# jacobwilliams/lbfgsb

Hardware: NVIDIA B200
Metric: lbfgsb_iterations_per_s (higher is better)
Workload: dtype f64

## Files before the change

### include/lbfgsb_b200.h

```cpp
#ifndef LBFGSB_B200_H
#define LBFGSB_B200_H

#include <stdint.h>

#ifdef __cplusplus
extern "C" {
#endif

#define LBFGSB_B200_MMAX 20

typedef struct lbfgsb_dev lbfgsb_dev_t;

int lbfgsb_b200_version(void);
const char* lbfgsb_b200_last_error(void);

void lbfgsb_setulb_f64(const int32_t* n, const int32_t* m, double* x, const double* l, const double* u,
                       const int32_t* nbd, double* f, double* g, const double* factr, const double* pgtol,
                       double* wa, int32_t* iwa, char* task, const int32_t* iprint, char* csave,
                       int32_t* lsave, int32_t* isave, double* dsave, const char* itfile, int32_t itfile_len);
void lbfgsb_setulb_f32(const int32_t* n, const int32_t* m, float* x, const float* l, const float* u,
                       const int32_t* nbd, float* f, float* g, const float* factr, const float* pgtol,
                       float* wa, int32_t* iwa, char* task, const int32_t* iprint, char* csave,
                       int32_t* lsave, int32_t* isave, float* dsave, const char* itfile, int32_t itfile_len);
void lbfgsb_host_release(int32_t* isave);
// ... 5 lines not shown
lbfgsb_dev_t* lbfgsb_dev_create_sharded(int64_t n_local, int64_t offset, int64_t n_global, int32_t m,
                                        int32_t real_kind, void* cuda_stream, void* nccl_comm,
                                        int32_t rank, int32_t world);
void lbfgsb_dev_destroy(lbfgsb_dev_t* h);
void lbfgsb_dev_set_iteration_file(lbfgsb_dev_t* h, const char* name);
void lbfgsb_setulb_dev_f64(lbfgsb_dev_t* h, double* x_dev, const double* l_dev, const double* u_dev,
                           const int32_t* nbd_dev, double* f, double* g_dev, const double* factr,
                           const double* pgtol, char* task, const int32_t* iprint, char* csave,
                           int32_t* lsave, int32_t* isave, double* dsave);
void lbfgsb_setulb_dev_f32(lbfgsb_dev_t* h, float* x_dev, const float* l_dev, const float* u_dev,
                           const int32_t* nbd_dev, float* f, float* g_dev, const float* factr,
                           const float* pgtol, char* task, const int32_t* iprint, char* csave,
                           int32_t* lsave, int32_t* isave, float* dsave);

typedef int (*lbfgsb_fg_dev_f64)(void* user, int64_t n, const double* x_dev, double* g_dev, double* f_out, void* cuda_stream);
typedef int (*lbfgsb_fg_dev_f32)(void* user, int64_t n, const float* x_dev, float* g_dev, float* f_out, void* cuda_stream);
int lbfgsb_minimize_dev_f64(lbfgsb_dev_t* h, double* x_dev, const double* l_dev, const double* u_dev, const int32_t* nbd_dev,
                            lbfgsb_fg_dev_f64 fg, void* user, double factr, double pgtol, int32_t max_iter, int32_t max_fg,
                            int32_t iprint, double* f, double* g_dev, char* task, char* csave, int32_t* lsave, int32_t* isave,
                            double* dsave);
int lbfgsb_minimize_dev_f32(lbfgsb_dev_t* h, float* x_dev, const float* l_dev, const float* u_dev, const int32_t* nbd_dev,
                            lbfgsb_fg_dev_f32 fg, void* user, float factr, float pgtol, int32_t max_iter, int32_t max_fg,
                            int32_t iprint, float* f, float* g_dev, char* task, char* csave, int32_t* lsave, int32_t* isave,
                            float* dsave);

typedef int (*lbfgsb_fg_enqueue_f64)(void* user, int64_t n, const double* x_dev, double* g_dev, double* f_dev, void* cuda_stream);
typedef int (*lbfgsb_fg_enqueue_f32)(void* user, int64_t n, const float* x_dev, float* g_dev, float* f_dev, void* cuda_stream);
int lbfgsb_minimize_graph_dev_f64(lbfgsb_dev_t* h, double* x_dev, const double* l_dev, const double* u_dev, const int32_t* nbd_dev,
                                  lbfgsb_fg_enqueue_f64 fg, void* user, double factr, double pgtol, int32_t max_iter, int32_t max_fg,
                                  double* f, double* g_dev, char* task, char* csave, int32_t* lsave, int32_t* isave, double* dsave);
int lbfgsb_minimize_graph_dev_f32(lbfgsb_dev_t* h, float* x_dev, const float* l_dev, const float* u_dev, const int32_t* nbd_dev,
                                  lbfgsb_fg_enqueue_f32 fg, void* user, float factr, float pgtol, int32_t max_iter, int32_t max_fg,
                                  float* f, float* g_dev, char* task, char* csave, int32_t* lsave, int32_t* isave, float* dsave);
int lbfgsb_dev_graph_stats(lbfgsb_dev_t* h, int64_t* graph_steps, int64_t* launches_per_step);

int lbfgsb_dev_checkpoint_write(lbfgsb_dev_t* h, const char* path);
int lbfgsb_dev_checkpoint_read(lbfgsb_dev_t* h, const char* path);

int lbfgsb_dev_nccl_unique_id(void* id128);
void* lbfgsb_dev_nccl_init(const void* id128, int32_t rank, int32_t world);
void lbfgsb_dev_nccl_destroy(void* comm);

int lbfgsb_dev_active_set_hash(lbfgsb_dev_t* h, uint64_t* hash, int64_t* count);
void* lbfgsb_dev_vector(lbfgsb_dev_t* h, int32_t which);
int lbfgsb_dev_vector_copy(lbfgsb_dev_t* h, int32_t which, void* dst_dev, int64_t bytes);
int lbfgsb_dev_exchange_mode(lbfgsb_dev_t* h);
int lbfgsb_dev_counters(lbfgsb_dev_t* h, int64_t* launches, int64_t* syncs);
void lbfgsb_dev_profile(lbfgsb_dev_t* h, int32_t enable);
int lbfgsb_dev_profile_read(lbfgsb_dev_t* h, int32_t cap, char* names , double* ms, double* bytes,
                            int64_t* calls);
void lbfgsb_dev_profile_reset(lbfgsb_dev_t* h);
void lbfgsb_dev_set_tie_limit(lbfgsb_dev_t* h, int64_t max_breakpoints);
int lbfgsb_dev_tie_stats(lbfgsb_dev_t* h, int64_t* replays, int64_t* not_replayed);

int lbfgsb_problem_rosenbrock_f64(int64_t n, const double* x_dev, double* g_dev, double* f_out, void* cuda_stream,
                                  int32_t first, int32_t last, double xl, double xr, void* scratch_dev);
int lbfgsb_problem_rosenbrock_f32(int64_t n, const float* x_dev, float* g_dev, float* f_out, void* cuda_stream,
                                  int32_t first, int32_t last, float xl, float xr, void* scratch_dev);
int64_t lbfgsb_problem_scratch_bytes(void);
int lbfgsb_problem_rosenbrock_halo_f64(int64_t n, const double* x_dev, double* g_dev, double* f_part_dev, void* cuda_stream,
                                       int32_t first, int32_t last, const double* halo_dev, void* scratch_dev);
typedef struct {
    const void* d_dev;
    void* gd_part_dev;
    void* pg_part_dev;
    int64_t n;
    int32_t grid, block, unroll, real_kind;
    int32_t vec, reserved;
} lbfgsb_trial_sums_t;
int lbfgsb_dev_trial_sums(lbfgsb_dev_t* h, lbfgsb_trial_sums_t* out);
void lbfgsb_dev_trial_sums_commit(lbfgsb_dev_t* h);
int lbfgsb_problem_fused_f64(lbfgsb_dev_t* h, int32_t kind, const double* x_dev, double* g_dev, const double* l_dev,
                             const double* u_dev, const int32_t* nbd_dev, double* f_out, uint64_t seed);
int lbfgsb_problem_sharded_f64(lbfgsb_dev_t* h, int32_t kind, const double* x_dev, double* g_dev, const double* l_dev,
                               const double* u_dev, const int32_t* nbd_dev, double* f_out, uint64_t seed);
int lbfgsb_problem_quadratic_halo_f64(int64_t n, const double* x_dev, double* g_dev, double* f_part_dev, void* cuda_stream,
                                      int64_t index_offset, uint64_t seed, const double* halo_dev, void* scratch_dev);

int lbfgsb_problem_quadratic_f64(int64_t n, const double* x_dev, double* g_dev, double* f_out, void* cuda_stream,
                                 int64_t index_offset, uint64_t seed, double xl, double xr, void* scratch_dev);
int lbfgsb_problem_quadratic_f32(int64_t n, const float* x_dev, float* g_dev, float* f_out, void* cuda_stream,
                                 int64_t index_offset, uint64_t seed, float xl, float xr, void* scratch_dev);

typedef struct lbfgsb_batch lbfgsb_batch_t;
lbfgsb_batch_t* lbfgsb_batch_create(int32_t nprob, int64_t n, int32_t m, int32_t real_kind, void* cuda_stream);
void lbfgsb_batch_destroy(lbfgsb_batch_t* h);
void lbfgsb_batch_setulb_dev_f64(lbfgsb_batch_t* h, double* x_dev, const double* l_dev, const double* u_dev, const int32_t* nbd_dev,
                                 double* f_dev, double* g_dev, const double* factr, const double* pgtol, char* task, char* csave,
                                 int32_t* lsave, int32_t* isave, double* dsave);
void lbfgsb_batch_setulb_dev_f32(lbfgsb_batch_t* h, float* x_dev, const float* l_dev, const float* u_dev, const int32_t* nbd_dev,
                                 float* f_dev, float* g_dev, const float* factr, const float* pgtol, char* task, char* csave,
                                 int32_t* lsave, int32_t* isave, float* dsave);
int lbfgsb_batch_counts(lbfgsb_batch_t* h, int32_t* n_fg, int32_t* n_newx, int32_t* n_done);
void* lbfgsb_batch_stream(lbfgsb_batch_t* h);
void* lbfgsb_batch_fg_mask(lbfgsb_batch_t* h);
int lbfgsb_batch_get_iwhere(lbfgsb_batch_t* h, int32_t* iwhere_host);
int lbfgsb_problem_rosenbrock_batch_f64(int32_t nprob, int64_t n, const double* x_dev, double* g_dev, double* f_dev,
                                        const int32_t* mask_dev, void* cuda_stream);
int lbfgsb_problem_rosenbrock_batch_f32(int32_t nprob, int64_t n, const float* x_dev, float* g_dev, float* f_dev,
                                        const int32_t* mask_dev, void* cuda_stream);

int lbfgsb_test_projgr_f64(int64_t n, const double* l, const double* u, const int32_t* nbd, const double* x,
                           const double* g, double* sbgnrm_out);
int lbfgsb_test_sum_f64(int64_t n, const double* a, const double* b, double* out);
int lbfgsb_test_sum_f32(int64_t n, const float* a, const float* b, float* out);
int lbfgsb_test_sort_f64(int64_t n, const double* t_dev, int32_t* order_out_dev, double* sorted_out_dev);
// ... 16 lines not shown
```

### lbfgsb_b200/__init__.py

```python
import ctypes as C
import os
import subprocess

import numpy as np

_HERE = os.path.dirname(os.path.abspath(__file__))
_ROOT = os.path.dirname(_HERE)
SO_PATH = os.path.join(_HERE, "liblbfgsb_b200.so")
_SOURCES = ["engine.cu", "common.cuh", "kernels_stream.cuh", "kernels_dense.cuh", "cauchy_walk.cuh", "kernels_tma.cuh",
            "tma_pipe.cuh", "cauchy_walk_dist.cuh", "batch.cuh", "host_print.h"]
NVCC_FLAGS = ["-gencode", "arch=compute_100a,code=sm_100a", "-lineinfo", "-O3", "-std=c++17",
              "-fmad=false", "-Xcompiler", "-fPIC", "-shared"]

_LIB = None


class LbfgsbB200Error(RuntimeError):
    pass


def _stale():
    if not os.path.exists(SO_PATH):
        return True
    t = os.path.getmtime(SO_PATH)
    deps = [os.path.join(_HERE, "csrc", s) for s in _SOURCES]
    deps += [os.path.join(_ROOT, "include", h) for h in ("lbfgsb_b200.h", "lbfgsb_b200_shape.h")]
    return any(os.path.exists(p) and os.path.getmtime(p) > t for p in deps)


def build(force=False, verbose=False):
    if not (force or _stale()):
        return SO_PATH
    nvcc = os.environ.get("NVCC", "/usr/local/cuda/bin/nvcc")
    cmd = [nvcc] + NVCC_FLAGS + (["-Xptxas", "-v"] if verbose else []) + \
          ["-o", SO_PATH, os.path.join(_HERE, "csrc", "engine.cu"), "-ldl"]
    subprocess.check_call(cmd)
    return SO_PATH


_REAL = {np.dtype(np.float64): ("f64", C.c_double), np.dtype(np.float32): ("f32", C.c_float)}


def lib():
    global _LIB
    if _LIB is None:
        if not os.path.exists(SO_PATH):
            raise LbfgsbB200Error(
                "lbfgsb_b200: %s is missing -- run `python -c 'import __graft_entry__ as g; g.build()'` "
                "(there is no CPU path)" % SO_PATH)
        L = C.CDLL(SO_PATH)
        L.lbfgsb_b200_last_error.restype = C.c_char_p
        L.lbfgsb_dev_create.restype = C.c_void_p
        L.lbfgsb_dev_create.argtypes = [C.c_int64, C.c_int32, C.c_int32, C.c_void_p]
        L.lbfgsb_dev_create_sharded.restype = C.c_void_p
        L.lbfgsb_dev_create_sharded.argtypes = [C.c_int64, C.c_int64, C.c_int64, C.c_int32, C.c_int32,
                                                C.c_void_p, C.c_void_p, C.c_int32, C.c_int32]
        L.lbfgsb_dev_destroy.argtypes = [C.c_void_p]
        L.lbfgsb_dev_set_iteration_file.argtypes = [C.c_void_p, C.c_char_p]
        L.lbfgsb_dev_checkpoint_write.argtypes = [C.c_void_p, C.c_char_p]
        L.lbfgsb_dev_checkpoint_read.argtypes = [C.c_void_p, C.c_char_p]
        L.lbfgsb_host_engine.restype = C.c_void_p
        L.lbfgsb_host_engine.argtypes = [C.c_void_p]
        L.lbfgsb_dev_vector.restype = C.c_void_p
        L.lbfgsb_dev_vector.argtypes = [C.c_void_p, C.c_int32]
        L.lbfgsb_dev_vector_copy.argtypes = [C.c_void_p, C.c_int32, C.c_void_p, C.c_int64]
        L.lbfgsb_dev_active_set_hash.argtypes = [C.c_void_p, C.c_void_p, C.c_void_p]
        L.lbfgsb_dev_counters.argtypes = [C.c_void_p, C.c_void_p, C.c_void_p]
        L.lbfgsb_dev_graph_stats.argtypes = [C.c_void_p, C.c_void_p, C.c_void_p]
        L.lbfgsb_problem_rosenbrock_halo_f64.argtypes = [C.c_int64, C.c_void_p, C.c_void_p, C.c_void_p, C.c_void_p, C.c_int32, C.c_int32,
                                                         C.c_void_p, C.c_void_p]
        L.lbfgsb_problem_quadratic_halo_f64.argtypes = [C.c_int64, C.c_void_p, C.c_void_p, C.c_void_p, C.c_void_p, C.c_int64, C.c_uint64,
                                                        C.c_void_p, C.c_void_p]
        L.lbfgsb_dev_profile.argtypes = [C.c_void_p, C.c_int32]
        L.lbfgsb_dev_profile_reset.argtypes = [C.c_void_p]
        L.lbfgsb_dev_set_tie_limit.argtypes = [C.c_void_p, C.c_int64]
        L.lbfgsb_dev_set_tie_limit.restype = None
        L.lbfgsb_dev_tie_stats.argtypes = [C.c_void_p, C.c_void_p, C.c_void_p]
        L.lbfgsb_dev_profile_read.argtypes = [C.c_void_p, C.c_int32, C.c_void_p, C.c_void_p, C.c_void_p, C.c_void_p]
        L.lbfgsb_dev_nccl_init.restype = C.c_void_p
        L.lbfgsb_dev_nccl_init.argtypes = [C.c_void_p, C.c_int32, C.c_int32]
        L.lbfgsb_dev_nccl_destroy.argtypes = [C.c_void_p]
        L.lbfgsb_problem_scratch_bytes.restype = C.c_int64
        for sfx, cr in (("f64", C.c_double), ("f32", C.c_float)):
            getattr(L, "lbfgsb_setulb_" + sfx).restype = None
            getattr(L, "lbfgsb_setulb_dev_" + sfx).restype = None
            getattr(L, "lbfgsb_problem_rosenbrock_" + sfx).argtypes = [
                C.c_int64, C.c_void_p, C.c_void_p, C.c_void_p, C.c_void_p, C.c_int32, C.c_int32, cr, cr, C.c_void_p]
            getattr(L, "lbfgsb_problem_quadratic_" + sfx).argtypes = [
                C.c_int64, C.c_void_p, C.c_void_p, C.c_void_p, C.c_void_p, C.c_int64, C.c_uint64, cr, cr, C.c_void_p]
        L.lbfgsb_problem_rosenbrock_halo_f64.argtypes = [C.c_int64, C.c_void_p, C.c_void_p, C.c_void_p, C.c_void_p, C.c_int32,
                                                         C.c_int32, C.c_void_p, C.c_void_p]
        L.lbfgsb_problem_quadratic_halo_f64.argtypes = [C.c_int64, C.c_void_p, C.c_void_p, C.c_void_p, C.c_void_p, C.c_int64,
                                                        C.c_uint64, C.c_void_p, C.c_void_p]
        for nm in ("lbfgsb_problem_fused_f64", "lbfgsb_problem_sharded_f64"):
            getattr(L, nm).argtypes = [C.c_void_p, C.c_int32, C.c_void_p, C.c_void_p, C.c_void_p, C.c_void_p, C.c_void_p,
                                       C.c_void_p, C.c_uint64]
        L.lbfgsb_dev_exchange_mode.argtypes = [C.c_void_p]
        L.lbfgsb_batch_create.restype = C.c_void_p
        L.lbfgsb_batch_create.argtypes = [C.c_int32, C.c_int64, C.c_int32, C.c_int32, C.c_void_p]
        L.lbfgsb_batch_destroy.argtypes = [C.c_void_p]
        L.lbfgsb_batch_counts.argtypes = [C.c_void_p, C.c_void_p, C.c_void_p, C.c_void_p]
        L.lbfgsb_batch_stream.restype = C.c_void_p
        L.lbfgsb_batch_stream.argtypes = [C.c_void_p]
        L.lbfgsb_batch_get_iwhere.restype = C.c_int
        L.lbfgsb_batch_get_iwhere.argtypes = [C.c_void_p, C.c_void_p]
        L.lbfgsb_batch_fg_mask.restype = C.c_void_p
        L.lbfgsb_batch_fg_mask.argtypes = [C.c_void_p]
        for sfx in ("f64", "f32"):
            getattr(L, "lbfgsb_batch_setulb_dev_" + sfx).restype = None
            getattr(L, "lbfgsb_batch_setulb_dev_" + sfx).argtypes = [C.c_void_p] * 14
            getattr(L, "lbfgsb_problem_rosenbrock_batch_" + sfx).argtypes = [C.c_int32, C.c_int64, C.c_void_p, C.c_void_p, C.c_void_p,
                                                                             C.c_void_p, C.c_void_p]
        _LIB = L
    return _LIB


def last_error():
    return lib().lbfgsb_b200_last_error().decode()


def _p(a):
    return a.ctypes.data_as(C.c_void_p)


def _check_task(task):
    s = bytes(task[:60]).decode(errors="replace")
    if s.startswith(("ERROR: CUDA", "ERROR: NO CUDA", "ERROR: INVALID LBFGSB", "ERROR: DEVICE POINTERS", "ERROR: SETULB CALLED")):
        raise LbfgsbB200Error(s.rstrip() + " -- " + last_error())


# ... 150 lines not shown
        if lib().lbfgsb_dev_checkpoint_write(C.c_void_p(self.h), path.encode()) != 0:
            raise LbfgsbB200Error("checkpoint write failed: " + last_error())

    def checkpoint_read(self, path):
        if lib().lbfgsb_dev_checkpoint_read(C.c_void_p(self.h), path.encode()) != 0:
            raise LbfgsbB200Error("checkpoint read failed: " + last_error())

    def active_set_hash(self):
        h, c = C.c_uint64(0), C.c_int64(0)
        if lib().lbfgsb_dev_active_set_hash(C.c_void_p(self.h), C.byref(h), C.byref(c)) != 0:
            raise LbfgsbB200Error(last_error())
        return h.value, c.value

    @staticmethod
    def _opt(t):
        return C.c_void_p(t.data_ptr()) if t is not None else C.c_void_p(0)

    def fused_fg(self, kind, x, g, l=None, u=None, nbd=None, seed=0):
        out = C.c_double(0.0)
        rc = lib().lbfgsb_problem_fused_f64(C.c_void_p(self.h), C.c_int32(kind), C.c_void_p(x.data_ptr()),
                                            C.c_void_p(g.data_ptr()), self._opt(l), self._opt(u), self._opt(nbd),
                                            C.byref(out), C.c_uint64(int(seed)))
        if rc != 0:
            raise LbfgsbB200Error("objective kernel failed (rc %d): %s" % (rc, last_error()))
        return out.value

    def sharded_fg(self, kind, x, g, l=None, u=None, nbd=None, seed=0):
        out = C.c_double(0.0)
        rc = lib().lbfgsb_problem_sharded_f64(C.c_void_p(self.h), C.c_int32(kind), C.c_void_p(x.data_ptr()),
                                              C.c_void_p(g.data_ptr()), self._opt(l), self._opt(u), self._opt(nbd),
                                              C.byref(out), C.c_uint64(int(seed)))
        if rc == 2:
            return None
        if rc != 0:
            raise LbfgsbB200Error("sharded objective failed: " + last_error())
        return out.value

    def exchange_mode(self):
        return int(lib().lbfgsb_dev_exchange_mode(C.c_void_p(self.h)))

    def counters(self):
        a, b = C.c_int64(0), C.c_int64(0)
        lib().lbfgsb_dev_counters(C.c_void_p(self.h), C.byref(a), C.byref(b))
        return a.value, b.value

    def set_tie_limit(self, max_breakpoints):
        lib().lbfgsb_dev_set_tie_limit(C.c_void_p(self.h), C.c_int64(int(max_breakpoints)))

    def tie_stats(self):
        a, b = C.c_int64(0), C.c_int64(0)
        lib().lbfgsb_dev_tie_stats(C.c_void_p(self.h), C.byref(a), C.byref(b))
        return a.value, b.value

    def profile(self, on=True):
        lib().lbfgsb_dev_profile(C.c_void_p(self.h), 1 if on else 0)

    def profile_reset(self):
        lib().lbfgsb_dev_profile_reset(C.c_void_p(self.h))

    def profile_read(self):
        cap = 64
        names = C.create_string_buffer(32 * cap)
        ms = (C.c_double * cap)()
        by = (C.c_double * cap)()
        calls = (C.c_int64 * cap)()
        k = lib().lbfgsb_dev_profile_read(C.c_void_p(self.h), cap, names, ms, by, calls)
        out = {}
        for i in range(k):
            nm = names.raw[32 * i:32 * (i + 1)].split(b"\0")[0].decode()
            out[nm] = {"ms": ms[i], "bytes": by[i], "calls": calls[i]}
        return out

    def vector(self, which, count=None, dtype=None):
        torch = self.torch
        n = self.n if count is None else count
        tdt = {np.dtype(np.float64): torch.float64, np.dtype(np.float32): torch.float32}[self.dtype]
        if which == 7:
            tdt = torch.int32
        out = torch.empty(n, dtype=tdt, device="cuda")
        if lib().lbfgsb_dev_vector_copy(C.c_void_p(self.h), which, C.c_void_p(out.data_ptr()),
                                        C.c_int64(out.numel() * out.element_size())) != 0:
            raise LbfgsbB200Error("lbfgsb_dev_vector_copy failed")
        return out

    def close(self):
        if self.h:
            lib().lbfgsb_dev_destroy(C.c_void_p(self.h))
            self.h = None

    def __del__(self):
        try:
            self.close()
        except Exception:
            pass


class RosenbrockDevice:

    def __init__(self, dtype, stream=None):
        import torch
        self.dtype = np.dtype(dtype)
        self.scratch = torch.empty(int(lib().lbfgsb_problem_scratch_bytes()), dtype=torch.uint8, device="cuda")
        sfx, self._cr = _REAL[self.dtype]
        self._fn = getattr(lib(), "lbfgsb_problem_rosenbrock_" + sfx)
        self._f = np.zeros(1, dtype=self.dtype)
        self.stream = stream
# ... 140 lines not shown
```

### lbfgsb_b200/csrc/common.cuh

```cuda
#pragma once
#include <cuda_runtime.h>
#include <stdint.h>
#include <float.h>
#include <math.h>

#include "../../include/lbfgsb_b200_shape.h"

typedef long long i64;

#define LB_MMAX 20
#define LB_KMAX (6 * LB_MMAX + 8)
#define LB_IMAX 8

enum {
    TK_START = 0, TK_FG_START = 1, TK_FG_LNSRCH = 2, TK_NEW_X = 3, TK_CONV_PG = 4, TK_CONV_F = 5,
    TK_ABNORMAL = 6, TK_RESTART = 7, TK_STOP = 8,
    TK_ERR_N = 10, TK_ERR_M = 11, TK_ERR_FACTR = 12, TK_ERR_NBD = 13, TK_ERR_INFEAS = 14
};
enum { PAUSE_NONE = 0, PAUSE_CLASSIFY = 1, PAUSE_WALK = 2, PAUSE_GCP_FREEV = 3, PAUSE_DELTA = 4, PAUSE_BACKTRACK = 5, PAUSE_LSINIT = 6 };
enum {
    CS_START = 0, CS_FG = 1, CS_CONV = 2, CS_WARN_ROUND = 3, CS_WARN_XTOL = 4, CS_WARN_STPMAX = 5,
    CS_WARN_STPMIN = 6, CS_ERR_STP_LT_MIN = 10, CS_ERR_STP_GT_MAX = 11, CS_ERR_G_GE_0 = 12,
    CS_ERR_FTOL = 13, CS_ERR_GTOL = 14, CS_ERR_XTOL = 15, CS_ERR_STPMIN = 16, CS_ERR_STPMAX = 17,
    CS_BLANK = 99
};
__host__ __device__ inline bool cs_is_warn(int c) { return c >= CS_WARN_ROUND && c <= CS_WARN_STPMIN; }
__host__ __device__ inline bool cs_is_err(int c) { return c >= CS_ERR_STP_LT_MIN && c <= CS_ERR_STPMAX; }

enum {
    EV_ITER_BEGIN = 1,
    EV_SUBGNORM0 = 2,
    EV_CAUCHY_SINGULAR = 3,
    EV_FORMK_FAIL = 4,
    EV_SUBSM_SINGULAR = 5,
    EV_BACKTRACK = 6,
    EV_ASCENT = 7,
    EV_LNSRCH_RESTART = 8,
    EV_SKIP = 9,
    EV_FORMT_FAIL = 10
};
#define LB_EVMAX 24

template <typename T> struct Real;
template <> struct Real<double> {
    static constexpr int VEC = LBFGSB_VEC_F64;
    static constexpr int UNROLL = LBFGSB_UNROLL_F64;
    typedef double2 vec_t;
    typedef int2 ivec_t;
    typedef unsigned long long key_t;
    __host__ __device__ static double eps() { return DBL_EPSILON; }
};
template <> struct Real<float> {
    static constexpr int VEC = LBFGSB_VEC_F32;
    static constexpr int UNROLL = LBFGSB_UNROLL_F32;
    typedef float2 vec_t;
    typedef int2 ivec_t;
    typedef unsigned int key_t;
    __host__ __device__ static float eps() { return FLT_EPSILON; }
};

template <typename T>
struct DevState {
    int go;
    int pause;
    int in_body;
    int restart;
    int need_walk;
    int cauchy_mode;
    int do_subspace, do_formk, do_delta, do_backtrack, do_update, do_step, do_restore;
    int fuse_uc;
    int classify_done;
    int lsinit_done;
    int spec_step;
    int step_done;
    int do_unstep;
    int lazy_gcp;
    int fuse_gf;
    int lazy_z;
    int p2p_timeout;
    int z_in_x;
    int save_z;
    int task, csave, info;
    int col, head, itail, iupdat, iter, nfgv, nskip, ifun, iback, iword;
    int updatd, prjctd, cnstnd, boxed, wrk, bnded;
    int brackt, stage;
    int m;
    int gstage;
    i64 n, nintol, nseg, nfree, nact, nenter, nleave, nbreak, nfreec, nbdd, errk;
    i64 ibkmin;
    i64 ibd;
    i64 walk_J;
    i64 walk_done;
    i64 walk_base;
    i64 walk_rcount;
    i64 walk_lcount;
    i64 walk_rem;
    i64 walk_cstart;
    i64 walk_fixn;
    int walk_closed, pad1;
    int tie_redo;
    int tie_round;
    i64 tie_limit;
    i64 tie_events;
    unsigned long long tie_key;
    i64 snap_base;
    int ev_n, ev_code[LB_EVMAX];
    T ev_a[LB_EVMAX], ev_b[LB_EVMAX];
    i64 n_el;
    T theta, fold, tol, dnorm, epsmch, gd, gdold, stp, stpmx, sbgnrm, dtd, xstep, f, rr, dr, ddum;
    T pgtol, factr, sbg_spec;
    T ls[13];
    T f1, f2, f2_org, dtm, tsum, bkmin;
    T dd_p, alpha;
    T walk_f1, walk_f2, walk_tlast, walk_tprev2;
    T sy[LB_MMAX * LB_MMAX], ss[LB_MMAX * LB_MMAX], wt[LB_MMAX * LB_MMAX];
    T wn[4 * LB_MMAX * LB_MMAX], wn1[4 * LB_MMAX * LB_MMAX];
    T p[2 * LB_MMAX], c[2 * LB_MMAX], v[2 * LB_MMAX], wv[2 * LB_MMAX], a[2 * LB_MMAX];
    T p0[2 * LB_MMAX];
    T walkA[2 * LB_MMAX], walkB[2 * LB_MMAX];
    T snapA[2 * LB_MMAX], snapB[2 * LB_MMAX];
    T snap_f1, snap_f2, snap_tlast, snap_tprev2;
};

template <typename T> __device__ inline void ev_push(DevState<T>* s, int code, T a = (T)0, T b = (T)0) {
    const int k = s->ev_n;
    if (k < LB_EVMAX) { s->ev_code[k] = code; s->ev_a[k] = a; s->ev_b[k] = b; s->ev_n = k + 1; }
}

template <typename T> __device__ __forceinline__ T shfl_xor_t(T v, int off);
template <> __device__ __forceinline__ double shfl_xor_t<double>(double v, int off) {
    return __shfl_xor_sync(0xffffffffu, v, off);
}
template <> __device__ __forceinline__ float shfl_xor_t<float>(float v, int off) {
    return __shfl_xor_sync(0xffffffffu, v, off);
}
template <> __device__ __forceinline__ i64 shfl_xor_t<i64>(i64 v, int off) {
    return __shfl_xor_sync(0xffffffffu, v, off);
}
template <> __device__ __forceinline__ int shfl_xor_t<int>(int v, int off) {
    return __shfl_xor_sync(0xffffffffu, v, off);
}

template <typename T> __device__ __forceinline__ T warp_sum(T v) {
#pragma unroll
    for (int off = 16; off >= 1; off >>= 1) v = v + shfl_xor_t<T>(v, off);
    return v;
}
template <typename T> __device__ __forceinline__ T warp_max(T v) {
#pragma unroll
    for (int off = 16; off >= 1; off >>= 1) { T o = shfl_xor_t<T>(v, off); v = o > v ? o : v; }
    return v;
}
template <typename T> __device__ __forceinline__ T warp_min(T v) {
#pragma unroll
    for (int off = 16; off >= 1; off >>= 1) { T o = shfl_xor_t<T>(v, off); v = o < v ? o : v; }
    return v;
}

template <typename T, int K>
__device__ __forceinline__ void block_sum_store(const T (&acc)[K], int kcount, T* smem, T* part) {
    const int lane = threadIdx.x & 31, w = threadIdx.x >> 5;
    constexpr int NW = LBFGSB_BLOCK / 32;
#pragma unroll
    for (int k = 0; k < K; ++k) {
        if (k < kcount) {
            T v = warp_sum<T>(acc[k]);
            if (lane == 0 && w < NW) smem[k * NW + w] = v;
        }
    }
    __syncthreads();
    for (int k = threadIdx.x; k < kcount; k += LBFGSB_BLOCK) {
        T s = smem[k * NW];
#pragma unroll
        for (int q = 1; q < NW; ++q) s = s + smem[k * NW + q];
// ... 186 lines not shown
            unsigned int q = *reinterpret_cast<const unsigned int*>(p + base);
#pragma unroll
            for (int v = 0; v < VEC; ++v) out[v] = (q >> (8 * v)) & 0xff;
        }
    } else {
#pragma unroll
        for (int v = 0; v < VEC; ++v) out[v] = (base + v < n) ? p[base + v] : 0;
    }
}
template <typename T>
__device__ __forceinline__ void stv(T* __restrict__ p, i64 base, i64 n, const T (&in)[Real<T>::VEC]) {
    constexpr int VEC = Real<T>::VEC;
    if (base + VEC <= n) {
        typename Real<T>::vec_t q;
        T* e = reinterpret_cast<T*>(&q);
#pragma unroll
        for (int v = 0; v < VEC; ++v) e[v] = in[v];
        *reinterpret_cast<typename Real<T>::vec_t*>(p + base) = q;
    } else {
#pragma unroll
        for (int v = 0; v < VEC; ++v) if (base + v < n) p[base + v] = in[v];
    }
}
template <typename T>
__device__ __forceinline__ void stvi(int* __restrict__ p, i64 base, i64 n, const int (&in)[Real<T>::VEC]) {
    constexpr int VEC = Real<T>::VEC;
    if (base + VEC <= n) {
        typename Real<T>::ivec_t q;
        int* e = reinterpret_cast<int*>(&q);
#pragma unroll
        for (int v = 0; v < VEC; ++v) e[v] = in[v];
        *reinterpret_cast<typename Real<T>::ivec_t*>(p + base) = q;
    } else {
#pragma unroll
        for (int v = 0; v < VEC; ++v) if (base + v < n) p[base + v] = in[v];
    }
}
template <typename T>
__device__ __forceinline__ void stvb(unsigned char* __restrict__ p, i64 base, i64 n,
                                     const int (&in)[Real<T>::VEC]) {
    constexpr int VEC = Real<T>::VEC;
    if (base + VEC <= n) {
        if (VEC == 2) {
            *reinterpret_cast<unsigned short*>(p + base) = (unsigned short)((in[0] & 0xff) | ((in[1] & 0xff) << 8));
        } else {
            unsigned int q = 0;
#pragma unroll
            for (int v = 0; v < VEC; ++v) q |= (unsigned int)(in[v] & 0xff) << (8 * v);
            *reinterpret_cast<unsigned int*>(p + base) = q;
        }
    } else {
#pragma unroll
        for (int v = 0; v < VEC; ++v) if (base + v < n) p[base + v] = (unsigned char)in[v];
    }
}

#define LB_FOR_TILES(T, n, base)                                                               \
    for (i64 _tl = blockIdx.x, _nt = ((n) + (i64)LBFGSB_BLOCK * Real<T>::VEC * Real<T>::UNROLL - 1) / \
                                     ((i64)LBFGSB_BLOCK * Real<T>::VEC * Real<T>::UNROLL);       \
         _tl < _nt; _tl += LBFGSB_GRID)                                                        \
        _Pragma("unroll") for (int _k = 0; _k < Real<T>::UNROLL; ++_k)                           \
            for (i64 base = _tl * ((i64)LBFGSB_BLOCK * Real<T>::VEC * Real<T>::UNROLL) +         \
                            (i64)_k * (LBFGSB_BLOCK * Real<T>::VEC) + (i64)threadIdx.x * Real<T>::VEC, \
                     _once = 1;                                                                \
                 _once && base < (n); _once = 0)

#define LB_FOR_TILES_NU(T, n, base)                                                            \
    for (i64 _tl = blockIdx.x, _nt = ((n) + (i64)LBFGSB_BLOCK * Real<T>::VEC * Real<T>::UNROLL - 1) / \
                                     ((i64)LBFGSB_BLOCK * Real<T>::VEC * Real<T>::UNROLL);       \
         _tl < _nt; _tl += LBFGSB_GRID)                                                        \
        _Pragma("unroll 1") for (int _k = 0; _k < Real<T>::UNROLL; ++_k)                         \
            for (i64 base = _tl * ((i64)LBFGSB_BLOCK * Real<T>::VEC * Real<T>::UNROLL) +         \
                            (i64)_k * (LBFGSB_BLOCK * Real<T>::VEC) + (i64)threadIdx.x * Real<T>::VEC, \
                     _once = 1;                                                                \
                 _once && base < (n); _once = 0)

namespace dense {

template <typename T> __device__ inline T ddot(int n, const T* dx, const T* dy) {
    T s = (T)0;
    for (int i = 0; i < n; ++i) s = s + dx[i] * dy[i];
    return s;
}
template <typename T> __device__ inline void daxpy(int n, T da, const T* dx, T* dy) {
    if (n <= 0 || da == (T)0) return;
    for (int i = 0; i < n; ++i) dy[i] = dy[i] + da * dx[i];
}

template <typename T> __device__ inline int dpofa(T* a, int lda, int n) {
    for (int j = 0; j < n; ++j) {
        T s = (T)0;
        for (int k = 0; k < j; ++k) {
            T t = a[k + j * lda] - ddot<T>(k, a + k * lda, a + j * lda);
            t = t / a[k + k * lda];
            a[k + j * lda] = t;
            s = s + t * t;
        }
        s = a[j + j * lda] - s;
        if (s <= (T)0) return j + 1;
        a[j + j * lda] = sqrt(s);
    }
    return 0;
}

template <typename T> __device__ inline int dtrsl(const T* t, int ldt, int n, T* b, int job) {
    for (int k = 0; k < n; ++k)
// ... 322 lines not shown
```

### lbfgsb_b200/csrc/engine.cu

```cuda
#include <cuda_runtime.h>
#include <dlfcn.h>
#include <stdarg.h>
#include <stdio.h>
#include <stdlib.h>
#include <string.h>

#include <mutex>
#include <string>
#include <unordered_set>
#include <vector>

#include "../../include/lbfgsb_b200.h"
#include "cauchy_walk.cuh"
#include "kernels_tma.cuh"
#include "cauchy_walk_dist.cuh"
#include "batch.cuh"
#include "host_print.h"
#include <algorithm>

static thread_local std::string g_last_error;
static void set_error(const char* fmt, ...) {
    char buf[512];
    va_list ap;
    va_start(ap, fmt);
// ... 4 lines not shown
#define CK(call)                                                                             \
    do {                                                                                     \
        cudaError_t _e = (call);                                                             \
        if (_e != cudaSuccess) {                                                             \
            set_error("CUDA error %s at %s:%d (%s)", cudaGetErrorString(_e), __FILE__, __LINE__, #call); \
            return false;                                                                    \
        }                                                                                    \
    } while (0)

typedef struct ncclComm* ncclComm_t;
typedef struct { char internal[128]; } ncclUniqueId;
struct NcclApi {
    int (*GetUniqueId)(ncclUniqueId*);
    int (*CommInitRank)(ncclComm_t*, int, ncclUniqueId, int);
    int (*CommDestroy)(ncclComm_t);
    int (*AllGather)(const void*, void*, size_t, int, ncclComm_t, cudaStream_t);
    int (*Send)(const void*, size_t, int, int, ncclComm_t, cudaStream_t);
    int (*Recv)(void*, size_t, int, int, ncclComm_t, cudaStream_t);
    int (*GroupStart)();
    int (*GroupEnd)();
    const char* (*GetErrorString)(int);
    bool ok;
};
static NcclApi* nccl_api() {
    static NcclApi api;
    static bool tried = false;
    if (!tried) {
        tried = true;
        api.ok = false;
        void* h = dlopen("libnccl.so.2", RTLD_NOW | RTLD_GLOBAL);
        if (!h) h = dlopen("libnccl.so", RTLD_NOW | RTLD_GLOBAL);
        if (h) {
            api.GetUniqueId = (int (*)(ncclUniqueId*))dlsym(h, "ncclGetUniqueId");
            api.CommInitRank = (int (*)(ncclComm_t*, int, ncclUniqueId, int))dlsym(h, "ncclCommInitRank");
            api.CommDestroy = (int (*)(ncclComm_t))dlsym(h, "ncclCommDestroy");
            api.AllGather = (int (*)(const void*, void*, size_t, int, ncclComm_t, cudaStream_t))dlsym(h, "ncclAllGather");
            api.GetErrorString = (const char* (*)(int))dlsym(h, "ncclGetErrorString");
            api.Send = (int (*)(const void*, size_t, int, int, ncclComm_t, cudaStream_t))dlsym(h, "ncclSend");
            api.Recv = (int (*)(void*, size_t, int, int, ncclComm_t, cudaStream_t))dlsym(h, "ncclRecv");
            api.GroupStart = (int (*)())dlsym(h, "ncclGroupStart");
            api.GroupEnd = (int (*)())dlsym(h, "ncclGroupEnd");
            api.ok = api.GetUniqueId && api.CommInitRank && api.CommDestroy && api.AllGather && api.Send && api.Recv &&
                     api.GroupStart && api.GroupEnd;
        }
    }
    return &api;
}

#define LB_TIE_DEVICE_MAX 16384

enum Fam {
    F_ERRCLB, F_ACTIVE, F_PROJGR, F_CLASSIFY, F_GCP_FREEV, F_FORMK_GRAM, F_FORMK_DELTA, F_CMPRLB_WV,
    F_SUBSM_STEP, F_BACKTRACK, F_LS_INIT, F_LS_STEP, F_LS_TRIAL, F_UPDATE, F_RESTORE, F_WALK_COMPACT,
    F_WALK_SORT, F_WALK_SCAN, F_WALK_FIX, F_SCALAR, F_HASH, F_UPDATE_CLASSIFY, F_FORMK_CMPRLB, F_SUBSM_LSINIT, F_COUNT
};
static const char* fam_name[F_COUNT] = {
    "errclb", "active", "projgr", "cauchy_classify", "gcp_freev", "formk_gram", "formk_delta", "cmprlb_wv",
    "subsm_step", "backtrack", "ls_init", "ls_step", "ls_trial", "update", "restore", "walk_compact",
    "walk_sort", "walk_scan", "walk_fix", "scalar", "hash", "update_classify", "formk_cmprlb", "subsm_lsinit"};

__global__ void __launch_bounds__(256) k_publish(const unsigned* src, unsigned* dst_host, int words, volatile unsigned long long* flag_host,
                                                 unsigned long long seq) {
    for (int q = threadIdx.x; q < words; q += blockDim.x) dst_host[q] = src[q];
    __threadfence_system();
    __syncthreads();
    if (threadIdx.x == 0) *flag_host = seq;
}

__global__ void __launch_bounds__(256) k_publish_g(const unsigned* src, unsigned* dst_host, int words, volatile unsigned long long* flag_host,
                                                   unsigned long long* counter) {
    for (int q = threadIdx.x; q < words; q += blockDim.x) dst_host[q] = src[q];
    __threadfence_system();
    __syncthreads();
    if (threadIdx.x == 0) { const unsigned long long v = *counter + 1; *counter = v; *flag_host = v; }
}

struct EngineBase {
    virtual ~EngineBase() {}
    int real_kind;
    lbprint::Ctx pr;
};

template <typename T>
struct Engine : EngineBase {
    i64 n = 0, n_global = 0, offset = 0;
    int m = 0, mt = 0;
    bool fused = false;
    cudaStream_t stream = 0;
    bool own_stream = false;
    Wk<T> w;
    WalkBuf<T> wb;
    DevState<T>* s_dev = nullptr;
    DevState<T>* s_host = nullptr;
    size_t header_bytes = 0;
    int* tile_counts = nullptr; i64* tile_offsets = nullptr; i64 ntiles = 0;
    int* rs_counts = nullptr;
    SortCtl* ctl_el = nullptr;
    SortCtl* ctl_host = nullptr;
    T* tmpAB = nullptr; T* tmpF = nullptr; unsigned long long* jmin = nullptr;
    T* fd_parts = nullptr; T* delta = nullptr; T* delta_all = nullptr; T* delta_sum = nullptr;
    std::vector<void*> allocs;
    int R = 1, rank = 0;
    ncclComm_t comm = nullptr;
    Red<T>* rec_local = nullptr; Red<T>* rec_all = nullptr;
    unsigned long long* samp_local = nullptr; unsigned long long* samp_all = nullptr; unsigned long long* spl_dev = nullptr;
    DwCtl* dctl = nullptr; i64* pos_all = nullptr; SortCtl* ctl_d = nullptr;
    RoundRec* rr_local = nullptr; RoundRec* rr_all = nullptr;
    WalkCarry<T>* carry_local = nullptr; WalkCarry<T>* carry_all = nullptr;
    struct DynBuf { void* p = nullptr; size_t cap = 0; };
    DynBuf dw_send, dw_recv, dw_k0, dw_k1, dw_v0, dw_v1;
    i64 launches = 0, syncs = 0, tie_replays = 0;
    bool profile = false;
    bool debug_launch = (getenv("LBFGSB_B200_DEBUG_LAUNCH") != nullptr);
    struct Ev { int fam; cudaEvent_t a, b; };
    std::vector<Ev> pending;
    std::vector<cudaEvent_t> pool;
    double fam_ms[F_COUNT]; i64 fam_calls[F_COUNT];
    bool x_changed = false, g_changed = false;
    bool walked_prev = false, walked_now = false, body_ran = false, bp_hint_ok = true, walk_gf_ok = true;
    bool started = false;

    bool p2p = false;
    P2PBuf<T>* p2p_local = nullptr;
    Peers peers, peers_delta;
    std::vector<void*> ipc_opened;
    bool trial_ready = false;
    unsigned long long site_seq = 0, delta_seq = 0, fg_seq = 0;
    T* fg_scratch = nullptr; T* fg_out = nullptr; T* fg_host = nullptr;
    int cur_slot = 0;
    bool site_pending = false;
    Dist<T> dist() {
        Dist<T> d; d.R = R; d.all = rec_all;
        d.p2p = p2p ? p2p_local : nullptr; d.slot = cur_slot; d.seq = site_seq; d.dseq = delta_seq;
        d.wait = site_pending ? 1 : 0; site_pending = false;
        return d;
    }
    bool setup_p2p() {
        if (const char* e = getenv("LBFGSB_B200_P2P")) { if (e[0] == '0') return true; }
        struct Pack { cudaIpcMemHandle_t hb, hd; int ok; int pad[3]; };
        Pack mine; memset(&mine, 0, sizeof mine);
        mine.ok = 1;
        if (cudaMalloc((void**)&p2p_local, sizeof(P2PBuf<T>)) != cudaSuccess) { p2p_local = nullptr; mine.ok = 0; cudaGetLastError(); }
        if (mine.ok) {
            allocs.push_back(p2p_local);
            cudaMemset(p2p_local, 0, sizeof(P2PBuf<T>));
            if (cudaIpcGetMemHandle(&mine.hb, p2p_local) != cudaSuccess || cudaIpcGetMemHandle(&mine.hd, delta_all) != cudaSuccess) {
                mine.ok = 0; cudaGetLastError();
            }
        }
        Pack* dsend = nullptr; Pack* drecv = nullptr;
        if (!dalloc(&dsend, sizeof(Pack)) || !dalloc(&drecv, sizeof(Pack) * R)) return false;
        CK(cudaMemcpy(dsend, &mine, sizeof mine, cudaMemcpyHostToDevice));
        if (!allgather(dsend, drecv, sizeof(Pack))) return false;
        std::vector<Pack> all(R);
        CK(cudaMemcpyAsync(all.data(), drecv, sizeof(Pack) * R, cudaMemcpyDeviceToHost, stream));
        CK(cudaStreamSynchronize(stream));
        bool ok = true;
        for (int q = 0; q < R; ++q) ok = ok && all[q].ok;
        memset(&peers, 0, sizeof peers); memset(&peers_delta, 0, sizeof peers_delta);
        int myok = ok ? 1 : 0;
        if (ok) {
            for (int q = 0; q < R && myok; ++q) {
                if (q == rank) { peers.p[q] = p2p_local; peers_delta.p[q] = delta_all; continue; }
                void *pb = nullptr, *pd = nullptr;
                if (cudaIpcOpenMemHandle(&pb, all[q].hb, cudaIpcMemLazyEnablePeerAccess) != cudaSuccess) { myok = 0; cudaGetLastError(); break; }
                ipc_opened.push_back(pb);
                if (cudaIpcOpenMemHandle(&pd, all[q].hd, cudaIpcMemLazyEnablePeerAccess) != cudaSuccess) { myok = 0; cudaGetLastError(); break; }
                ipc_opened.push_back(pd);
                peers.p[q] = pb; peers_delta.p[q] = pd;
            }
        }
        int* dflag = nullptr; int* dflags = nullptr;
        if (!dalloc(&dflag, sizeof(int)) || !dalloc(&dflags, sizeof(int) * R)) return false;
        CK(cudaMemcpy(dflag, &myok, sizeof(int), cudaMemcpyHostToDevice));
        if (!allgather(dflag, dflags, sizeof(int))) return false;
        std::vector<int> oks(R);
        CK(cudaMemcpyAsync(oks.data(), dflags, sizeof(int) * R, cudaMemcpyDeviceToHost, stream));
        CK(cudaStreamSynchronize(stream));
        p2p = true;
        for (int q = 0; q < R; ++q) p2p = p2p && oks[q];
        return true;
    }

    template <typename P> bool dalloc(P** p, size_t bytes) {
        void* q = nullptr;
        if (bytes == 0) bytes = 16;
        cudaError_t e = cudaMalloc(&q, bytes);
        if (e != cudaSuccess) { set_error("cudaMalloc(%zu) failed: %s", bytes, cudaGetErrorString(e)); return false; }
        allocs.push_back(q);
        *p = (P*)q;
        return true;
    }

    bool init(i64 n_, i64 off_, i64 ng_, int m_, cudaStream_t st, ncclComm_t cm, int rank_, int world_) {
        n = n_; offset = off_; n_global = ng_; m = m_; R = world_; rank = rank_; comm = cm;
        real_kind = (int)sizeof(T);
        mt = (m <= 5) ? 5 : (m <= 10 ? 10 : 20);
        fused = (mt == 5 ? fused_passes_ok<T, 5>() : (mt == 10 ? fused_passes_ok<T, 10>() : fused_passes_ok<T, 20>()));
        if (const char* e = getenv("LBFGSB_B200_NO_FUSION")) { if (e[0] == '1') fused = false; }
        fast = fused;
        if (const char* e = getenv("LBFGSB_B200_NO_FAST")) { if (e[0] == '1') fast = false; }
        if (const char* e = getenv("LBFGSB_B200_NO_TIMERS")) { if (e[0] == '1') timers = false; }
        if (const char* e = getenv("LBFGSB_B200_NO_SMALL_ROUNDS")) { if (e[0] == '1') { small_rounds = false; small_sort = false; } }
        if (const char* e = getenv("LBFGSB_B200_NO_BP_HINT")) { if (e[0] == '1') { bp_hint_ok = false; walk_gf_ok = false; } }
        if (!(mt == 5 ? set_smem_attrs<5>() : (mt == 10 ? set_smem_attrs<10>() : set_smem_attrs<20>()))) return false;
        for (int q = 0; q < F_COUNT; ++q) { fam_ms[q] = 0; fam_calls[q] = 0; }
        if (st) stream = st;
        else { CK(cudaStreamCreateWithFlags(&stream, cudaStreamNonBlocking)); own_stream = true; }
        memset(&w, 0, sizeof w);
        w.n = n; w.m = m; w.off = offset;
        w.ldw = (n + 31) / 32 * 32;
        const size_t vb = (size_t)w.ldw * sizeof(T);
        if (!dalloc(&w.ws, vb * m) || !dalloc(&w.wy, vb * m)) return false;
        if (!dalloc(&w.z, vb) || !dalloc(&w.r, vb) || !dalloc(&w.d, vb) || !dalloc(&w.t, vb) || !dalloc(&w.xp, vb) || !dalloc(&w.gold, vb)) return false;
        if (!dalloc(&w.iwhere, (size_t)w.ldw * 4) || !dalloc(&w.state, (size_t)w.ldw)) return false;
        if (!dalloc(&w.part, sizeof(T) * LB_KMAX * LBFGSB_GRID) || !dalloc(&w.ipart, sizeof(i64) * LB_IMAX * LBFGSB_GRID)) return false;
        if (!dalloc(&w.part2, sizeof(T) * LB_KMAX * LBFGSB_GRID) || !dalloc(&w.ipart2, sizeof(i64) * LB_IMAX * LBFGSB_GRID)) return false;
        if (!dalloc(&s_dev, sizeof(DevState<T>))) return false;
        CK(cudaMemsetAsync(s_dev, 0, sizeof(DevState<T>), stream));
        {
            i64 lim = (i64)1 << 28;
            if (R > 1) lim = (i64)1 << 26;
            if (const char* e = getenv("LBFGSB_B200_TIE_LIMIT")) lim = atoll(e);
            CK(cudaMemcpyAsync(&s_dev->tie_limit, &lim, sizeof lim, cudaMemcpyHostToDevice, stream));
        }
        CK(cudaMemsetAsync(w.ws, 0, vb * m, stream));
        CK(cudaMemsetAsync(w.wy, 0, vb * m, stream));
        w.s = s_dev;
        CK(cudaHostAlloc((void**)&s_host, sizeof(DevState<T>) + 64, cudaHostAllocMapped));
        memset(s_host, 0, sizeof(DevState<T>) + 64);
        pub_flag = (volatile unsigned long long*)((char*)s_host + ((sizeof(DevState<T>) + 7) / 8) * 8);
        if (const char* e = getenv("LBFGSB_B200_SYNC")) { if (e[0] == 'm') publish = false; }
        CK(cudaMallocHost((void**)&ctl_host, sizeof(SortCtl)));
        header_bytes = offsetof(DevState<T>, sy);
        const i64 tile = (i64)LBFGSB_BLOCK * Real<T>::VEC * Real<T>::UNROLL;
        ntiles = (n + tile - 1) / tile;
        if (!dalloc(&tile_counts, sizeof(int) * (size_t)(ntiles + 1)) || !dalloc(&tile_offsets, sizeof(i64) * (size_t)(ntiles + 1))) return false;
        if (!dalloc(&rs_counts, sizeof(int) * 256 * LB_RS_GRID)) return false;
        typedef typename Real<T>::key_t K;
        memset(&wb, 0, sizeof wb);
        if (!dalloc(&wb.k0, sizeof(K) * (size_t)w.ldw) || !dalloc(&wb.k1, sizeof(K) * (size_t)w.ldw)) return false;
        if (!dalloc(&wb.v0, 4 * (size_t)w.ldw) || !dalloc(&wb.v1, 4 * (size_t)w.ldw)) return false;
        if (!dalloc(&wb.ctl, sizeof(SortCtl)) || !dalloc(&ctl_el, sizeof(SortCtl))) return false;
        i64 cap = n < (i64)(1 << 22) ? n : (i64)(1 << 22);
        cap = (cap + LB_WB - 1) / LB_WB * LB_WB;
        wb.cap = cap;
        const size_t cb = (size_t)cap * sizeof(T);
        if (!dalloc(&wb.wj, cb * 2 * m) || !dalloc(&wb.vj, cb * 2 * m)) return false;
        if (!dalloc(&wb.delta, cb) || !dalloc(&wb.zeta, cb) || !dalloc(&wb.omega, cb) || !dalloc(&wb.g2, cb) ||
            !dalloc(&wb.g1, cb) || !dalloc(&wb.f1a, cb) || !dalloc(&wb.f2a, cb)) return false;
        const i64 nblk = cap / LB_WB;
        if (!dalloc(&wb.blkA, sizeof(T) * (size_t)nblk * 2 * LB_MMAX) || !dalloc(&wb.blkB, sizeof(T) * (size_t)nblk * 2 * LB_MMAX)) return false;
        if (!dalloc(&wb.blk_a, sizeof(T) * (size_t)nblk) || !dalloc(&wb.blk_b, sizeof(T) * (size_t)nblk) || !dalloc(&wb.blkH, sizeof(T) * (size_t)nblk)) return false;
        if (!dalloc(&tmpAB, sizeof(T) * 4 * LB_MMAX) || !dalloc(&tmpF, sizeof(T) * 2) || !dalloc(&jmin, 8)) return false;
        if (!dalloc(&fd_parts, sizeof(T) * (size_t)LB_FD_GRID * 6 * LB_MMAX * LB_MMAX) || !dalloc(&delta, sizeof(T) * 6 * LB_MMAX * LB_MMAX)) return false;
        CK(cudaMemsetAsync(delta, 0, sizeof(T) * 6 * LB_MMAX * LB_MMAX, stream));
        if (!dalloc(&rr_local, sizeof(RoundRec)) || !dalloc(&rr_all, sizeof(RoundRec) * (R > 1 ? R : 1))) return false;
        if (R > 1) {
            if (R > LB_MAXR) { set_error("at most %d ranks", LB_MAXR); return false; }
            if (!dalloc(&rec_local, sizeof(Red<T>)) || !dalloc(&rec_all, sizeof(Red<T>) * R)) return false;
            const size_t sb = sizeof(unsigned long long) * (2 * LB_DW_SAMPLES + 1);
            if (!dalloc(&samp_local, sb) || !dalloc(&samp_all, sb * R) || !dalloc(&spl_dev, 16 * LB_MAXR)) return false;
            if (!dalloc(&dctl, sizeof(DwCtl)) || !dalloc(&pos_all, sizeof(i64) * (LB_MAXR + 1) * R) || !dalloc(&ctl_d, sizeof(SortCtl))) return false;
            if (!dalloc(&carry_local, sizeof(WalkCarry<T>)) || !dalloc(&carry_all, sizeof(WalkCarry<T>) * R)) return false;
            if (!dalloc(&delta_all, sizeof(T) * 6 * LB_MMAX * LB_MMAX * R) || !dalloc(&delta_sum, sizeof(T) * 6 * LB_MMAX * LB_MMAX)) return false;
        }
        CK(cudaStreamSynchronize(stream));
        if (R > 1 && !setup_p2p()) return false;
// ... 74 lines not shown
            launches++;
            unsigned spins = 0;
            while (*pub_flag != pub_seq) {
                if ((++spins & 0x3fff) == 0) {
                    cudaError_t q = cudaStreamQuery(stream);
                    if (q != cudaSuccess && q != cudaErrorNotReady) { set_error("CUDA error %s while waiting for the state block", cudaGetErrorString(q)); return false; }
                    if (q == cudaSuccess && *pub_flag != pub_seq) { set_error("the state block was not published (internal error)"); return false; }
                }
            }
        } else {
            CK(cudaMemcpyAsync(s_host, s_dev, header_bytes, cudaMemcpyDeviceToHost, stream));
            CK(cudaStreamSynchronize(stream));
        }
        syncs++;
        if (profile && resolve) resolve_events();
        if (s_host->p2p_timeout) { set_error("a peer rank's reduction record did not arrive (sharded run over peer memory)"); return false; }
        return true;
    }
    bool site(const SiteSpec& sp) {
        if (R <= 1) return true;
        site_pending = true;
        if (p2p) {
            site_seq++; cur_slot = (int)(site_seq & 1ULL);
            k_rank_finish_p2p<T><<<1, LB_SCALAR_THREADS, 0, stream>>>(w, sp, peers, R, rank, cur_slot, site_seq);
            launches++;
            return true;
        }
        k_rank_finish<T><<<1, LB_SCALAR_THREADS, 0, stream>>>(w, sp, rec_local);
        launches++;
        int rc = nccl_api()->AllGather(rec_local, rec_all, sizeof(Red<T>), 0 , comm, stream);
        if (rc != 0) { set_error("ncclAllGather failed: %d", rc); return false; }
        return true;
    }
    bool site_m(const MSite& ms) {
        if (R <= 1) return true;
        site_pending = true;
        if (p2p) { site_seq++; cur_slot = (int)(site_seq & 1ULL); }
        k_rank_finish_m<T><<<1, LB_SCALAR_THREADS, 0, stream>>>(w, ms, rec_local, peers, R, rank, cur_slot, site_seq, p2p ? 1 : 0);
        launches++;
        if (!p2p) {
            int rc = nccl_api()->AllGather(rec_local, rec_all, sizeof(Red<T>), 0 , comm, stream);
            if (rc != 0) { set_error("ncclAllGather failed: %d", rc); return false; }
        }
        return true;
    }
#define LG LBFGSB_GRID, LBFGSB_BLOCK, 0, stream
#define LS 1, LB_SCALAR_THREADS, 0, stream
#define MTCALL(kern, smemfn, ...)                                                                          \
    do {                                                                                                   \
        if (mt == 5) kern<T, 5><<<LBFGSB_GRID, LB_TMA_THREADS, smemfn<T, 5>(), stream>>>(__VA_ARGS__);        \
        else if (mt == 10) kern<T, 10><<<LBFGSB_GRID, LB_TMA_THREADS, smemfn<T, 10>(), stream>>>(__VA_ARGS__); \
        else kern<T, 20><<<LBFGSB_GRID, LB_TMA_THREADS, smemfn<T, 20>(), stream>>>(__VA_ARGS__);              \
    } while (0)

    template <int MT> void launch_update_classify() {
        if constexpr (fused_passes_ok<T, MT>()) k_update_classify<T, MT><<<LBFGSB_GRID, LB_TMA_THREADS, smem_update_classify<T, MT>(), stream>>>(w);
    }
    template <int MT> void launch_formk_cmprlb() {
        if constexpr (fused_passes_ok<T, MT>()) k_formk_cmprlb<T, MT, 0><<<LBFGSB_GRID, LB_TMA_THREADS, smem_formk_cmprlb<T, MT>(), stream>>>(w);
    }
    template <int MT> void launch_formk_cmprlb_gf() {
        if constexpr (fused_passes_ok<T, MT>()) k_formk_cmprlb<T, MT, 1><<<LBFGSB_GRID, LB_TMA_THREADS, smem_formk_cmprlb<T, MT>(), stream>>>(w);
    }
    template <int MT> void launch_formk_cmprlb_gf2() {
        if constexpr (fused_passes_ok<T, MT>()) k_formk_cmprlb<T, MT, 2><<<LBFGSB_GRID, LB_TMA_THREADS, smem_formk_cmprlb<T, MT>(), stream>>>(w);
    }
    template <int MT> void launch_subsm_lsinit() {
        if constexpr (fused_passes_ok<T, MT>()) k_subsm_lsinit<T, MT, 0><<<LBFGSB_GRID, LB_TMA_THREADS, smem_subsm<T, MT>(), stream>>>(w);
    }
    template <int MT> void launch_subsm_dir() {
        if constexpr (fused_passes_ok<T, MT>()) k_subsm_lsinit<T, MT, 1><<<LBFGSB_GRID, LB_TMA_THREADS, smem_subsm<T, MT>(), stream>>>(w);
    }
#define MTFUSED(fn) do { if (mt == 5) fn<5>(); else if (mt == 10) fn<10>(); else fn<20>(); } while (0)

    template <int MT> bool set_smem_attrs() {
        CK(cudaFuncSetAttribute(k_update<T, MT>, cudaFuncAttributeMaxDynamicSharedMemorySize, (int)smem_update<T, MT>()));
        CK(cudaFuncSetAttribute(k_cauchy_classify<T, MT>, cudaFuncAttributeMaxDynamicSharedMemorySize, (int)smem_classify<T, MT>()));
        CK(cudaFuncSetAttribute(k_formk_gram<T, MT>, cudaFuncAttributeMaxDynamicSharedMemorySize, (int)smem_formk<T, MT>()));
        CK(cudaFuncSetAttribute(k_cmprlb_wv<T, MT>, cudaFuncAttributeMaxDynamicSharedMemorySize, (int)smem_cmprlb<T, MT>()));
        CK(cudaFuncSetAttribute(k_subsm_step<T, MT>, cudaFuncAttributeMaxDynamicSharedMemorySize, (int)smem_subsm<T, MT>()));
        if constexpr (fused_passes_ok<T, MT>()) {
            CK(cudaFuncSetAttribute(k_update_classify<T, MT>, cudaFuncAttributeMaxDynamicSharedMemorySize, (int)smem_update_classify<T, MT>()));
            CK(cudaFuncSetAttribute(k_formk_cmprlb<T, MT, 0>, cudaFuncAttributeMaxDynamicSharedMemorySize, (int)smem_formk_cmprlb<T, MT>()));
            CK(cudaFuncSetAttribute(k_formk_cmprlb<T, MT, 1>, cudaFuncAttributeMaxDynamicSharedMemorySize, (int)smem_formk_cmprlb<T, MT>()));
            CK(cudaFuncSetAttribute(k_formk_cmprlb<T, MT, 2>, cudaFuncAttributeMaxDynamicSharedMemorySize, (int)smem_formk_cmprlb<T, MT>()));
            CK(cudaFuncSetAttribute(k_subsm_lsinit<T, MT, 0>, cudaFuncAttributeMaxDynamicSharedMemorySize, (int)smem_subsm<T, MT>()));
            CK(cudaFuncSetAttribute(k_subsm_lsinit<T, MT, 1>, cudaFuncAttributeMaxDynamicSharedMemorySize, (int)smem_subsm<T, MT>()));
        }
        return true;
    }

    static unsigned long long key_of(T t) {
        typename Real<T>::key_t k;
        memcpy(&k, &t, sizeof k);
        return (unsigned long long)k;
    }
    int run_round(const BpRange& rg, bool first = false) {
        begin(F_WALK_COMPACT);
        if (first) k_bp_count<T, true><<<LG>>>(w, rg, tile_counts);
        else k_bp_count<T, false><<<LG>>>(w, rg, tile_counts);
        k_walk_round_local<T><<<1, 1024, 0, stream>>>(w, tile_counts, tile_offsets, ntiles, wb.ctl, rr_local);
        end(F_WALK_COMPACT, 2);
        if (R > 1 && !allgather(rr_local, rr_all, sizeof(RoundRec))) return -1;
        k_walk_round_begin<T><<<1, 32, 0, stream>>>(w, R > 1 ? rr_all : rr_local, R, n_global); launches++;
        if (!sync_state()) return -1;
        if (s_host->walk_closed) return 1;
        if (s_host->walk_rcount > 0) {
            begin(F_WALK_COMPACT); k_bp_write<T><<<LG>>>(w, rg, tile_counts, tile_offsets, wb.k0, wb.v0); end(F_WALK_COMPACT);
            begin(F_WALK_SORT); enqueue_sort(wb.k0, wb.k1, wb.v0, wb.v1, wb.ctl, s_host->walk_lcount); end(F_WALK_SORT, 0);
            if (R > 1) { if (!round_scan_sharded()) return -1; }
            else if (!round_scan_single(s_host->walk_lcount)) return -1;
            if (!sync_state()) return -1;
            if (s_host->walk_closed) return 1;
            if (s_host->tie_redo) return 2;
        }
        return 0;
    }
    int tie_replay(const BpRange& rg) {
        if (R > 1) return tie_replay_sharded(rg);
        const unsigned long long tk = s_host->tie_key;
        k_tie_restore<T><<<1, 32, 0, stream>>>(w); launches++;
        if (tk > 0) {
            BpRange ra = rg; ra.hi = tk - 1;
            if (!(ra.lo_valid && ra.hi <= ra.lo)) {
                const int st = run_round(ra);
                if (st < 0) return -1;
                if (st != 0) { set_error("heap replay: the round below the tie group did not pass (internal error)"); return -1; }
            }
        }
        begin(F_WALK_COMPACT);
        k_flag_count<T, 2><<<LG>>>(w, tile_counts);
        k_tile_scan<T><<<1, 1024, 0, stream>>>(w, 2, tile_counts, tile_offsets, ntiles, wb.ctl);
        k_flag_write<T, 2><<<LG>>>(w, tile_counts, tile_offsets, wb.k0, wb.v0);
        end(F_WALK_COMPACT, 3);
        if (s_host->nbreak <= LB_TIE_DEVICE_MAX) {
            begin(F_WALK_SORT); k_heap_replay<T><<<1, 1024, 0, stream>>>(w, wb); end(F_WALK_SORT);
        } else if (!heap_replay_on_host(tk)) return -1;
        if (!sync_state()) return -1;
        tie_replays++;
        if (s_host->walk_lcount <= 0) { set_error("heap replay: empty tie group (internal error)"); return -1; }
// ... 300 lines not shown
        k_dw_pack<T><<<LBFGSB_GRID, 256, 0, stream>>>(w, wb, send, rs); launches++;
        nccl_api()->GroupStart();
        for (int q = 0; q < R; ++q) {
            const i64 sc = cnt(rank, q), rc = cnt(q, rank);
            if (q == rank) {
                if (sc > 0) CK(cudaMemcpyAsync(recv + hc.roff[q] * rs, send + hc.pos[q] * rs, sizeof(T) * (size_t)sc * rs, cudaMemcpyDeviceToDevice, stream));
                continue;
            }
            if (sc > 0) nccl_api()->Send(send + hc.pos[q] * rs, sizeof(T) * (size_t)sc * rs, 0, q, comm, stream);
            if (rc > 0) nccl_api()->Recv(recv + hc.roff[q] * rs, sizeof(T) * (size_t)rc * rs, 0, q, comm, stream);
        }
        int grc = nccl_api()->GroupEnd();
        if (grc != 0) { set_error("nccl send/recv group failed: %d", grc); return false; }
        WalkBuf<T> wd = wb;
        wd.k0 = (K*)dw_k0.p; wd.k1 = (K*)dw_k1.p; wd.v0 = (int*)dw_v0.p; wd.v1 = (int*)dw_v1.p; wd.ctl = ctl_d;
        k_dw_keys<T><<<LBFGSB_GRID, 256, 0, stream>>>(recv, rs, nrecv, wd.k0, wd.v0, ctl_d); launches++;
        enqueue_sort(wd.k0, wd.k1, wd.v0, wd.v1, ctl_d, nrecv);
        for (int turn = 0; turn < R; ++turn) {
            if (turn == rank) {
                for (i64 start = 0; start < nrecv; start += wd.cap) {
                    const i64 len = (nrecv - start < wd.cap) ? (nrecv - start) : wd.cap;
                    const i64 nblk = (len + LB_WB - 1) / LB_WB;
                    CK(cudaMemsetAsync(jmin, 0xff, 8, stream));
                    k_dw_gather<T><<<(unsigned)nblk, LB_WB, 0, stream>>>(w, wd, recv, rs, start, len);
                    k_walk_scan_vec<T><<<1, 1024, 0, stream>>>(w, wd, nblk, tmpAB);
                    k_walk_dots<T><<<(unsigned)nblk, LB_WB, 0, stream>>>(w, wd, start, len);
                    k_walk_scan_f2<T><<<1, 32, 0, stream>>>(w, wd, nblk, tmpF);
                    k_walk_f2<T><<<(unsigned)nblk, LB_WB, 0, stream>>>(w, wd, start, len);
                    k_walk_scan_f1<T><<<1, 32, 0, stream>>>(w, wd, nblk, tmpF);
                    k_walk_test<T><<<(unsigned)nblk, LB_WB, 0, stream>>>(w, wd, start, len, jmin);
                    k_walk_chunk_end<T><<<1, 32, 0, stream>>>(w, wd, start, len, tmpAB, tmpF, jmin);
                    launches += 8;
                }
                k_dw_fixcount<T><<<LBFGSB_GRID, 256, 0, stream>>>(w, wd, R, dctl); launches++;
            }
            k_dw_turn_end<T><<<1, LB_WB, 0, stream>>>(w, wd, dctl, wd.cap, turn == rank ? 1 : 0, R, carry_local); launches++;
            if (!allgather(carry_local, carry_all, sizeof(WalkCarry<T>))) return false;
            k_dw_adopt<T><<<1, 32, 0, stream>>>(w, carry_all, turn, R, rank, dctl, n_global); launches++;
        }
        end(F_WALK_SCAN, 0);
        begin(F_WALK_FIX);
        k_dw_fix<T><<<LBFGSB_GRID, 256, 0, stream>>>(w, wb, dctl);
        end(F_WALK_FIX);
        return true;
    }

    bool enqueue_body(int from = PAUSE_NONE) {
        body_ran = true;
        for (;;) {
            bool gf = false;
            bool gf2 = false;
            if (from <= PAUSE_CLASSIFY) {
                phase(PH_CAUCHY);
                begin(F_CLASSIFY); MTCALL(k_cauchy_classify, smem_classify, w); end(F_CLASSIFY);
                if (!site(site_cauchy(mt))) return false;
                begin(F_SCALAR); s_cauchy<T><<<LS>>>(w, dist(), mt, fused ? 1 : 0); end(F_SCALAR);
            }
            if (from <= PAUSE_WALK) {
                if (s_host->cnstnd) {
                    if (from != PAUSE_WALK && !sync_state()) return false;
                    if (s_host->go && s_host->in_body && s_host->need_walk) {
                        walked_now = true;
                        if (!enqueue_walk_rounds()) return false;
                        if (fused && walk_gf_ok) { begin(F_SCALAR); s_walk_gf<T><<<LS>>>(w, 1); end(F_SCALAR); gf2 = true; }
                    }
                    gf = fused && s_host->go && s_host->in_body && s_host->fuse_gf;
                }
            }
            if (from <= PAUSE_GCP_FREEV) {
                phase(PH_SUBSPACE);
                if (!gf) {
                    begin(F_GCP_FREEV); k_gcp_freev<T><<<LG>>>(w); end(F_GCP_FREEV);
                    if (!site(site_freev())) return false;
                }
                begin(F_SCALAR); s_freev<T><<<LS>>>(w, dist(), n_global, 0); end(F_SCALAR);
                if (fused) {
                    begin(F_FORMK_CMPRLB);
                    if (gf) MTFUSED(launch_formk_cmprlb_gf);
                    else { if (gf2) { MTFUSED(launch_formk_cmprlb_gf2); launches++; } MTFUSED(launch_formk_cmprlb); }
                    end(F_FORMK_CMPRLB);
                }
                else { begin(F_FORMK_GRAM); MTCALL(k_formk_gram, smem_formk, w); end(F_FORMK_GRAM); }
                if (gf || gf2) {
                    if (!site(site_freev())) return false;
                    begin(F_SCALAR); s_freev<T><<<LS>>>(w, dist(), n_global, 1); end(F_SCALAR);
                }
            }
            if (from <= PAUSE_DELTA) {
                if (from == PAUSE_DELTA) phase(PH_SUBSPACE);
                begin(F_FORMK_DELTA);
                k_el_count<T><<<LG>>>(w, tile_counts);
                k_tile_scan<T><<<1, 1024, 0, stream>>>(w, 1, tile_counts, tile_offsets, ntiles, ctl_el);
                k_flag_write<T, 1><<<LG>>>(w, tile_counts, tile_offsets, wb.k0, wb.v0);
                k_formk_delta<T><<<fd_grid<T>(), 256, 0, stream>>>(w, wb.v0, ctl_el, fd_parts);
                k_formk_delta_final<T><<<(6 * LB_MMAX * LB_MMAX + 255) / 256, 256, 0, stream>>>(w, fd_parts, fd_grid<T>(), delta);
                end(F_FORMK_DELTA, 5);
                if (!site(site_formk(mt))) return false;
                if (R > 1) {
                    if (p2p) { delta_seq++; k_delta_push<T><<<1, 256, 0, stream>>>(w, delta, peers_delta, peers, R, rank, delta_seq); launches++; }
                    else if (!allgather(delta, delta_all, sizeof(T) * 6 * LB_MMAX * LB_MMAX)) return false;
                }
                begin(F_SCALAR); s_formk_dense<T><<<LS>>>(w, dist(), mt, R > 1 ? delta_all : delta, delta_sum); end(F_SCALAR);
                if (!fused) { begin(F_CMPRLB_WV); MTCALL(k_cmprlb_wv, smem_cmprlb, w); end(F_CMPRLB_WV); }
                if (!site(site_wv(mt))) return false;
                begin(F_SCALAR); s_subsm_dense<T><<<LS>>>(w, dist(), mt, fused ? 1 : 0); end(F_SCALAR);
                if (fused) { begin(F_SUBSM_LSINIT); MTFUSED(launch_subsm_lsinit); end(F_SUBSM_LSINIT); }
                else { begin(F_SUBSM_STEP); MTCALL(k_subsm_step, smem_subsm, w); end(F_SUBSM_STEP); }
                if (!site(site_subsm())) return false;
                begin(F_SCALAR); s_subsm_post<T><<<LS>>>(w, dist(), fused ? 1 : 0); end(F_SCALAR);
            }
            if (from <= PAUSE_BACKTRACK) {
                if (from == PAUSE_BACKTRACK) phase(PH_SUBSPACE);
                begin(F_BACKTRACK);
                if (fused) { MTFUSED(launch_subsm_dir); launches++; }
                k_bt_alpha<T><<<LG>>>(w);
                if (!site(site_bt())) return false;
                s_bt<T><<<LS>>>(w, dist(), offset);
                k_bt_apply<T><<<LG>>>(w);
                end(F_BACKTRACK, 3);
            }
            phase(PH_LNSRCH);
            begin(F_LS_INIT); k_ls_init<T><<<LG>>>(w); end(F_LS_INIT);
            if (!site(site_lsinit())) return false;
            begin(F_SCALAR); s_ls_init<T><<<LS>>>(w, dist()); end(F_SCALAR);
            begin(F_LS_STEP); k_ls_step<T><<<LG>>>(w); end(F_LS_STEP);
            phase(PH_END);
            if (!sync_state()) return false;
            if (s_host->do_step) x_changed = true;
            if (!s_host->restart) break;
            begin(F_SCALAR); s_restart_body<T><<<1, 32, 0, stream>>>(w); end(F_SCALAR);
            from = PAUSE_NONE;
        }
        return true;
    }

    bool fast = false;
    bool fast_newx(T f) {
        begin(F_SCALAR); f_head<T><<<1, 32, 0, stream>>>(w, f, 1); end(F_SCALAR);
        phase(PH_CAUCHY);
        begin(F_UPDATE_CLASSIFY); MTFUSED(launch_update_classify); end(F_UPDATE_CLASSIFY);
        if (!site_m(msite_ucf(mt))) return false;
        begin(F_SCALAR); f_ucf<T><<<LS>>>(w, dist(), mt); end(F_SCALAR);
        const size_t ev_ucf = pending.size();
        phase(PH_SUBSPACE);
        begin(F_FORMK_CMPRLB); MTFUSED(launch_formk_cmprlb_gf); end(F_FORMK_CMPRLB);
        if (!site_m(msite_mid(mt))) return false;
        begin(F_SCALAR); f_mid<T><<<LS>>>(w, dist(), mt, n_global); end(F_SCALAR);
        const size_t ev_mid = pending.size();
        begin(F_SUBSM_LSINIT); MTFUSED(launch_subsm_lsinit); end(F_SUBSM_LSINIT);
        if (!site_m(msite_tail())) return false;
        phase(PH_LNSRCH);
        begin(F_SCALAR); f_tail<T><<<LS>>>(w, dist()); end(F_SCALAR);
        phase(PH_END);
        if (!sync_state(false)) return false;
        if (profile) {
            const int ps = s_host->pause;
            if (ps == PAUSE_CLASSIFY || ps == PAUSE_WALK || ps == PAUSE_GCP_FREEV) drop_events_from(ev_ucf);
            else if (ps == PAUSE_DELTA || ps == PAUSE_LSINIT) drop_events_from(ev_mid);
            resolve_events();
        }
// ... 82 lines not shown
        marks.clear();
        walked_now = false; body_ran = false;
        if (s_host->gstage == 2) {
            if (s_host->pause != PAUSE_NONE) {
                const int from = s_host->pause;
                fast_pauses++;
                s_resume<T><<<1, 32, 0, stream>>>(w); launches++;
                if (!enqueue_body(from)) return false;
            } else if (s_host->restart) {
                s_restart_body<T><<<1, 32, 0, stream>>>(w); launches++;
                if (!enqueue_body()) return false;
            }
        } else {
            if (s_host->do_restore) {
                k_restore<T><<<LG>>>(w); launches++;
                CK(cudaStreamSynchronize(stream));
            }
            if (s_host->restart) {
                s_restart_body<T><<<1, 32, 0, stream>>>(w); launches++;
                if (!enqueue_body()) return false;
            }
        }
        resolve_phases();
        return check_launch();
    }

    bool check_launch() {
        cudaError_t e = cudaGetLastError();
        if (e != cudaSuccess) { set_error("kernel launch failed: %s", cudaGetErrorString(e)); return false; }
        return true;
    }

    bool call(int entry, int aux, T* x, const T* l, const T* u, const int* nbd, T* f, T* g, T factr, T pgtol) {
        w.x = x; w.l = l; w.u = u; w.nbd = nbd; w.g = g;
        w.bp_hint = (entry == 3 && walked_prev && bp_hint_ok) ? 1 : 0;
        walked_now = false; body_ran = false;
        x_changed = false; g_changed = false;
        for (auto& mk : marks) pool.push_back(mk.e);
        marks.clear();
        const bool ts_ready = trial_ready;
        trial_ready = false;
        if (entry == 0) {
            started = true;
            ph_time[0] = ph_time[1] = ph_time[2] = 0;
            int host_err = 0;
            if (factr < (T)0) host_err = TK_ERR_FACTR;
            s_start<T><<<1, 32, 0, stream>>>(w, factr, pgtol, host_err); launches++;
            begin(F_ERRCLB); k_errclb<T><<<LG>>>(w); end(F_ERRCLB);
            if (!site(site_errclb())) return false;
            s_errclb<T><<<LS>>>(w, dist(), offset); launches++;
            begin(F_ACTIVE); k_active<T><<<LG>>>(w); end(F_ACTIVE);
            if (!site(site_active())) return false;
            s_active<T><<<LS>>>(w, dist()); launches++;
            if (!sync_state()) return false;
            x_changed = true;
            return check_launch();
        }
        if (entry == 4) {
            if (aux) {
                CK(cudaMemcpyAsync(x, w.t, sizeof(T) * n, cudaMemcpyDeviceToDevice, stream));
                CK(cudaMemcpyAsync(g, w.gold, sizeof(T) * n, cudaMemcpyDeviceToDevice, stream));
                CK(cudaStreamSynchronize(stream));
                *f = s_host->fold;
                s_host->f = s_host->fold;
                x_changed = true; g_changed = true;
            }
            s_host->task = TK_STOP;
            return true;
        }
        if (entry == 5) {
            s_host->task = TK_FG_START;
            return true;
        }
        if (entry == 1) {
            s_call_begin<T><<<1, 32, 0, stream>>>(w, *f, entry); launches++;
            begin(F_PROJGR); k_projgr<T><<<LG>>>(w); end(F_PROJGR);
            if (!site(site_projgr())) return false;
            begin(F_SCALAR); s_fg_start<T><<<LS>>>(w, dist()); end(F_SCALAR);
            if (!enqueue_body()) return false;
        } else if (entry == 2) {
            phase(PH_LNSRCH);
            if (!ts_ready) { begin(F_LS_TRIAL); k_ls_trial<T><<<LG>>>(w); end(F_LS_TRIAL); }
            if (!site(site_lstrial())) return false;
            begin(F_SCALAR); s_ls_trial<T><<<LS>>>(w, dist(), 1, *f); end(F_SCALAR);
            phase(PH_END);
            if (!sync_state()) return false;
            if (s_host->do_restore) {
                begin(F_RESTORE); k_restore<T><<<LG>>>(w); end(F_RESTORE);
                CK(cudaStreamSynchronize(stream));
                if (profile) resolve_events();
                x_changed = true; g_changed = true;
            }
            if (!finish_step()) return false;
            if (s_host->restart) {
                begin(F_SCALAR); s_restart_body<T><<<1, 32, 0, stream>>>(w); end(F_SCALAR);
                if (!enqueue_body()) return false;
            }
        } else if (fast && s_host->cnstnd) {
            if (!fast_newx(*f)) return false;
        } else {
            s_call_begin<T><<<1, 32, 0, stream>>>(w, *f, entry); launches++;
            begin(F_SCALAR); s_newx_tests<T><<<1, 32, 0, stream>>>(w, fused ? 1 : 0); end(F_SCALAR);
            if (fused) { begin(F_UPDATE_CLASSIFY); MTFUSED(launch_update_classify); end(F_UPDATE_CLASSIFY); }
            begin(F_UPDATE); MTCALL(k_update, smem_update, w); end(F_UPDATE);
            if (!site(site_update(mt))) return false;
            begin(F_SCALAR); s_update_dense<T><<<LS>>>(w, dist(), mt); end(F_SCALAR);
            if (!enqueue_body()) return false;
        }
        *f = s_host->f;
        if (body_ran) walked_prev = walked_now;
        resolve_phases();
        return check_launch();
    }

    struct CkHeader { char magic[8]; i64 n, ldw, n_global, offset; int m, real_kind, R, rank; i64 state_bytes; };
    bool checkpoint_io(const char* path, bool write) {
        CK(cudaStreamSynchronize(stream));
        const std::string tmp = std::string(path) + ".tmp";
        FILE* fp = fopen(write ? tmp.c_str() : path, write ? "wb" : "rb");
        if (!fp) { set_error("cannot open checkpoint file %s", write ? tmp.c_str() : path); return false; }
        CkHeader hd; memset(&hd, 0, sizeof hd);
        memcpy(hd.magic, "LBB2CKP2", 8);
        hd.n = n; hd.ldw = w.ldw; hd.n_global = n_global; hd.offset = offset; hd.m = m; hd.real_kind = (int)sizeof(T); hd.R = R; hd.rank = rank;
        hd.state_bytes = (i64)sizeof(DevState<T>);
        bool ok = true;
        if (write) ok = fwrite(&hd, sizeof hd, 1, fp) == 1;
        else {
            CkHeader in;
            ok = fread(&in, sizeof in, 1, fp) == 1 && memcmp(in.magic, hd.magic, 8) == 0 && in.n == hd.n && in.ldw == hd.ldw &&
                 in.n_global == hd.n_global && in.offset == hd.offset && in.m == hd.m && in.real_kind == hd.real_kind &&
                 in.R == hd.R && in.rank == hd.rank && in.state_bytes == hd.state_bytes;
            if (!ok) set_error("checkpoint %s does not match this workspace (n, m, real kind or shard differ)", path);
        }
        i64 my_tie_limit = 0;
        if (ok && !write) ok = cudaMemcpy(&my_tie_limit, &s_dev->tie_limit, sizeof my_tie_limit, cudaMemcpyDeviceToHost) == cudaSuccess;
        const size_t CH = (size_t)64 << 20;
        void* stage = nullptr;
        if (ok && cudaMallocHost(&stage, CH) != cudaSuccess) { set_error("cudaMallocHost failed"); ok = false; }
        auto xfer = [&](void* dptr, size_t bytes) {
            for (size_t o = 0; ok && o < bytes; o += CH) {
                const size_t c = bytes - o < CH ? bytes - o : CH;
                if (write) {
                    ok = cudaMemcpy(stage, (char*)dptr + o, c, cudaMemcpyDeviceToHost) == cudaSuccess && fwrite(stage, 1, c, fp) == c;
                } else {
                    ok = fread(stage, 1, c, fp) == c && cudaMemcpy((char*)dptr + o, stage, c, cudaMemcpyHostToDevice) == cudaSuccess;
                }
            }
        };
        const size_t vb = (size_t)w.ldw * sizeof(T);
        xfer(s_dev, sizeof(DevState<T>));
        xfer(w.ws, vb * m); xfer(w.wy, vb * m);
        xfer(w.z, vb); xfer(w.r, vb); xfer(w.d, vb); xfer(w.t, vb); xfer(w.xp, vb); xfer(w.gold, vb);
        xfer(w.iwhere, (size_t)w.ldw * 4); xfer(w.state, (size_t)w.ldw);
        if (stage) cudaFreeHost(stage);
        if (ok && !write) ok = cudaMemcpy(&s_dev->tie_limit, &my_tie_limit, sizeof my_tie_limit, cudaMemcpyHostToDevice) == cudaSuccess;
        if (ok && !write) ok = cudaMemcpy(s_host, s_dev, header_bytes, cudaMemcpyDeviceToHost) == cudaSuccess;
        if (ok && !write) started = true;
        if (write && ok) ok = fflush(fp) == 0;
        if (fclose(fp) != 0) ok = false;
        if (write) {
            if (ok) ok = rename(tmp.c_str(), path) == 0;
            else remove(tmp.c_str());
        }
        if (!ok && g_last_error.empty()) set_error("checkpoint %s failed on %s", write ? "write" : "read", path);
        return ok;
    }

    bool active_hash(uint64_t* hash, i64* count) {
        begin(F_HASH); k_active_hash<T><<<LG>>>(w, offset); end(F_HASH);
        std::vector<i64> hp(2 * LBFGSB_GRID);
        CK(cudaMemcpyAsync(hp.data(), w.ipart, sizeof(i64) * 2 * LBFGSB_GRID, cudaMemcpyDeviceToHost, stream));
        CK(cudaStreamSynchronize(stream));
        uint64_t h = 0; i64 c = 0;
        for (int b = 0; b < LBFGSB_GRID; ++b) { h += (uint64_t)hp[b]; c += hp[LBFGSB_GRID + b]; }
        *hash = h; *count = c;
        return true;
    }
};

static void put60(char* s, const char* lit) {
    size_t k = strlen(lit);
    if (k > 60) k = 60;
    memcpy(s, lit, k);
    for (size_t i = k; i < 60; ++i) s[i] = ' ';
}
static bool pre60(const char* s, const char* lit) { return memcmp(s, lit, strlen(lit)) == 0; }
static bool eq60(const char* s, const char* lit) {
    size_t k = strlen(lit);
    if (memcmp(s, lit, k) != 0) return false;
    for (size_t i = k; i < 60; ++i) if (s[i] != ' ') return false;
    return true;
}
static const char* task_text(int code) {
    switch (code) {
        case TK_FG_START: return "FG_START";
        case TK_FG_LNSRCH: return "FG_LNSRCH";
        case TK_NEW_X: return "NEW_X";
        case TK_CONV_PG: return "CONVERGENCE: NORM_OF_PROJECTED_GRADIENT_<=_PGTOL";
        case TK_CONV_F: return "CONVERGENCE: REL_REDUCTION_OF_F_<=_FACTR*EPSMCH";
        case TK_ABNORMAL: return "ABNORMAL_TERMINATION_IN_LNSRCH";
        case TK_RESTART: return "RESTART_FROM_LNSRCH";
        case TK_ERR_N: return "ERROR: N <= 0";
        case TK_ERR_M: return "ERROR: M <= 0";
        case TK_ERR_FACTR: return "ERROR: FACTR < 0";
        case TK_ERR_NBD: return "ERROR: INVALID NBD";
        case TK_ERR_INFEAS: return "ERROR: NO FEASIBLE SOLUTION";
        default: return "START";
    }
}
static const char* csave_text(int code) {
// ... 260 lines not shown
        isave[18] = 0;
        if (*n <= 0) { put60(task, "ERROR: N <= 0"); if (*m <= 0) put60(task, "ERROR: M <= 0"); if (*factr < (T)0) put60(task, "ERROR: FACTR < 0"); return; }
        if (*m <= 0) { put60(task, "ERROR: M <= 0"); if (*factr < (T)0) put60(task, "ERROR: FACTR < 0"); return; }
        if (*m > LB_MMAX) { put60(task, "ERROR: M > 20 IS NOT SUPPORTED BY LBFGSB_B200"); return; }
        int ndev = 0;
        if (cudaGetDeviceCount(&ndev) != cudaSuccess || ndev == 0) {
            put60(task, "ERROR: NO CUDA DEVICE (LBFGSB_B200 HAS NO CPU PATH)");
            set_error("no CUDA device");
            return;
        }
        Engine<T>* e = new Engine<T>();
        if (!e->init(*n, 0, *n, *m, nullptr, nullptr, 0, 1)) { delete e; put60(task, "ERROR: CUDA FAILURE (see lbfgsb_b200_last_error)"); return; }
        if (itfile && itfile_len > 0) e->pr.itname = std::string(itfile, (size_t)itfile_len);
        p = new HostProblem();
        p->eng = e; p->n = *n; p->kind = (int)sizeof(T);
        const size_t vb = (size_t)(*n) * sizeof(T);
        if (cudaMalloc(&p->x, vb) || cudaMalloc(&p->l, vb) || cudaMalloc(&p->u, vb) || cudaMalloc(&p->g, vb) ||
            cudaMalloc((void**)&p->nbd, (size_t)(*n) * 4)) {
            set_error("cudaMalloc failed for the host twin's staging vectors");
            put60(task, "ERROR: CUDA FAILURE (see lbfgsb_b200_last_error)");
            delete e; delete p; return;
        }
        cudaMemcpyAsync(p->x, x, vb, cudaMemcpyHostToDevice, e->stream);
        cudaMemcpyAsync(p->l, l, vb, cudaMemcpyHostToDevice, e->stream);
        cudaMemcpyAsync(p->u, u, vb, cudaMemcpyHostToDevice, e->stream);
        cudaMemcpyAsync(p->nbd, nbd, (size_t)(*n) * 4, cudaMemcpyHostToDevice, e->stream);
        {
            std::lock_guard<std::mutex> lk(g_reg_mu);
            g_registry.insert(p);
        }
        uint64_t v = (uint64_t)(uintptr_t)p;
        isave[16] = (int32_t)(uint32_t)(v & 0xffffffffu); isave[17] = (int32_t)(uint32_t)(v >> 32); isave[18] = LB_MAGIC;
    } else {
        p = hp_from_isave(isave);
        if (!p || p->kind != (int)sizeof(T)) { put60(task, "ERROR: SETULB CALLED WITHOUT A VALID START (ISAVE ALTERED?)"); return; }
    }
    Engine<T>* e = (Engine<T>*)p->eng;
    const size_t vb = (size_t)p->n * sizeof(T);
    if (pre60(task, "FG")) cudaMemcpyAsync(p->g, g, vb, cudaMemcpyHostToDevice, e->stream);
    setulb_dev_impl<T>((lbfgsb_dev_t*)e, (T*)p->x, (const T*)p->l, (const T*)p->u, p->nbd, f, (T*)p->g, factr, pgtol,
                       task, iprint, csave, lsave, isave, dsave);
    if (e->x_changed) cudaMemcpyAsync(x, p->x, vb, cudaMemcpyDeviceToHost, e->stream);
    if (e->g_changed) cudaMemcpyAsync(g, p->g, vb, cudaMemcpyDeviceToHost, e->stream);
    if (e->x_changed || e->g_changed) cudaStreamSynchronize(e->stream);
    if (pre60(task, "CONV") || pre60(task, "ABNO") || pre60(task, "ERROR") || pre60(task, "STOP")) {
        hp_free(p);
        isave[18] = 0;
    }
}

template <typename T>
struct TrialSums {
    const T* d; const T* l; const T* u; const int* nbd;
    T* gd_part; T* pg_part;
};
template <typename T>
__device__ __forceinline__ void trial_sums_store(const TrialSums<T>& ts, T agd, T pg, T* sm) {
    T a[1]; a[0] = agd;
    __syncthreads();
    block_sum_store<T, 1>(a, 1, sm, ts.gd_part);
    __syncthreads();
    T r = block_max<T>(pg, sm);
    if (threadIdx.x == 0) ts.pg_part[blockIdx.x] = r;
}

template <typename T>
__global__ void __launch_bounds__(LBFGSB_BLOCK) k_rosenbrock(i64 n, const T* __restrict__ x, T* __restrict__ g,
                                                            T* part, int first, int last, T xl, T xr, const T* halo,
                                                            TrialSums<T> ts) {
    constexpr int VEC = Real<T>::VEC;
    __shared__ T sm[LBFGSB_BLOCK / 32];
    if (halo) { xl = halo[0]; xr = halo[1]; }
    T agd = (T)0, pgm = (T)0;
    T acc[1]; acc[0] = (T)0;
    LB_FOR_TILES(T, n, base) {
        T xv[VEC], gv[VEC];
        ldv<T>(x, base, n, xv);
        T xm = (base > 0) ? x[base - 1] : xl;
        T xp = (base + VEC < n) ? x[base + VEC] : xr;
#pragma unroll
        for (int v = 0; v < VEC; ++v) {
            const i64 i = base + v;
            if (i < n) {
                const T xi = xv[v];
                const T xprev = (v == 0) ? xm : xv[v - 1];
                const T xnext = (v == VEC - 1 || i + 1 >= n) ? ((i + 1 < n) ? ((v == VEC - 1) ? xp : xv[v + 1]) : xr) : xv[v + 1];
                const bool is_first = first && i == 0, is_last = last && i == n - 1;
                T t2 = xi - xprev * xprev;
                T t1 = xnext - xi * xi;
                if (is_first) {
                    gv[v] = (T)2 * (xi - (T)1) - (T)16 * xi * t1;
                    acc[0] = acc[0] + (T)0.25 * (xi - (T)1) * (xi - (T)1);
                } else {
                    acc[0] = acc[0] + t2 * t2;
                    gv[v] = is_last ? (T)8 * t2 : ((T)8 * t2 - (T)16 * xi * t1);
                }
            } else gv[v] = (T)0;
        }
        stv<T>(g, base, n, gv);
        if (ts.d) {
            T d[VEC], l[VEC], u[VEC]; int nb[VEC];
            ldv<T>(ts.d, base, n, d); ldv<T>(ts.l, base, n, l); ldv<T>(ts.u, base, n, u); ldvi<T>(ts.nbd, base, n, nb);
#pragma unroll
            for (int v = 0; v < VEC; ++v)
                if (base + v < n) {
                    agd = agd + gv[v] * d[v];
                    pgm = dense::tmax(pgm, projg_one<T>(xv[v], gv[v], l[v], u[v], nb[v]));
                }
        }
    }
    block_sum_store<T, 1>(acc, 1, sm, part);
    if (ts.d) trial_sums_store<T>(ts, agd, pgm, sm);
}
template <typename T>
__global__ void k_rosenbrock_final(const T* part, T* out) {
    T s = final_sum_warp<T>(part);
    if (threadIdx.x == 0) out[0] = (T)4 * s;
}
template <typename T>
static int rosenbrock_impl(i64 n, const T* x, T* g, T* f_out, void* st, int first, int last, T xl, T xr, void* scratch) {
    cudaStream_t s = (cudaStream_t)st;
    T* part = (T*)scratch;
    T* out = part + LBFGSB_GRID;
    k_rosenbrock<T><<<LBFGSB_GRID, LBFGSB_BLOCK, 0, s>>>(n, x, g, part, first, last, xl, xr, nullptr, TrialSums<T>{});
    k_rosenbrock_final<T><<<1, 32, 0, s>>>(part, out);
    if (cudaMemcpyAsync(f_out, out, sizeof(T), cudaMemcpyDeviceToHost, s) != cudaSuccess) return 1;
    if (cudaStreamSynchronize(s) != cudaSuccess) { set_error("rosenbrock kernel failed: %s", cudaGetErrorString(cudaGetLastError())); return 1; }
    return 0;
}

__host__ __device__ inline unsigned long long lb_mix64(unsigned long long v) {
    v += 0x9E3779B97F4A7C15ULL;
    v = (v ^ (v >> 30)) * 0xBF58476D1CE4E5B9ULL;
    v = (v ^ (v >> 27)) * 0x94D049BB133111EBULL;
    return v ^ (v >> 31);
}
template <typename T>
__device__ __forceinline__ void quad_coeff(unsigned long long gi, unsigned long long seedp, T& diag, T& b) {
    const double u1 = (double)(lb_mix64(2ULL * gi + 2ULL * seedp) >> 32) * (1.0 / 4294967296.0);
    const double u2 = (double)(lb_mix64(2ULL * gi + 1ULL + 2ULL * seedp) >> 32) * (1.0 / 4294967296.0);
    diag = (T)(2.0 + (0.1 + u1));
    b = (T)(2.0 * u2 - 1.0);
}
template <typename T>
__global__ void __launch_bounds__(LBFGSB_BLOCK) k_quadratic(i64 n, const T* __restrict__ x, T* __restrict__ g, T* part,
                                                           i64 off, unsigned long long seedp, T xl, T xr, const T* halo,
                                                           TrialSums<T> ts) {
    constexpr int VEC = Real<T>::VEC;
    __shared__ T sm[LBFGSB_BLOCK / 32];
    if (halo) { xl = halo[0]; xr = halo[1]; }
    T agd = (T)0, pgm = (T)0;
    T acc[1]; acc[0] = (T)0;
    LB_FOR_TILES(T, n, base) {
        T xv[VEC], gv[VEC];
        ldv<T>(x, base, n, xv);
        const T xm = (base > 0) ? x[base - 1] : xl;
        const T xp = (base + VEC < n) ? x[base + VEC] : xr;
#pragma unroll
        for (int v = 0; v < VEC; ++v) {
            const i64 i = base + v;
            gv[v] = (T)0;
            if (i < n) {
                const T xi = xv[v];
                const T xprev = (v == 0) ? xm : xv[v - 1];
                const T xnext = (i + 1 >= n) ? xr : ((v == VEC - 1) ? xp : xv[v + 1]);
                T diag, b;
                quad_coeff<T>((unsigned long long)(i + off), seedp, diag, b);
                const T ax = diag * xi - xprev - xnext;
                gv[v] = ax - b;
                acc[0] = acc[0] + ((T)0.5 * ax - b) * xi;
            }
        }
        stv<T>(g, base, n, gv);
        if (ts.d) {
            T d[VEC], l[VEC], u[VEC]; int nb[VEC];
            ldv<T>(ts.d, base, n, d); ldv<T>(ts.l, base, n, l); ldv<T>(ts.u, base, n, u); ldvi<T>(ts.nbd, base, n, nb);
#pragma unroll
            for (int v = 0; v < VEC; ++v)
                if (base + v < n) {
                    agd = agd + gv[v] * d[v];
                    pgm = dense::tmax(pgm, projg_one<T>(xv[v], gv[v], l[v], u[v], nb[v]));
                }
        }
    }
    block_sum_store<T, 1>(acc, 1, sm, part);
    if (ts.d) trial_sums_store<T>(ts, agd, pgm, sm);
}
template <typename T>
__global__ void k_sum_final(const T* part, T* out) {
    T s = final_sum_warp<T>(part);
    if (threadIdx.x == 0) out[0] = s;
}
template <typename T>
static int quadratic_impl(i64 n, const T* x, T* g, T* f_out, void* st, i64 off, unsigned long long seed, T xl, T xr, void* scratch) {
    cudaStream_t s = (cudaStream_t)st;
    T* part = (T*)scratch;
    T* out = part + LBFGSB_GRID;
    const unsigned long long seedp = seed * 0x9E3779B97F4A7C15ULL;
    k_quadratic<T><<<LBFGSB_GRID, LBFGSB_BLOCK, 0, s>>>(n, x, g, part, off, seedp, xl, xr, nullptr, TrialSums<T>{});
    k_sum_final<T><<<1, 32, 0, s>>>(part, out);
    if (cudaMemcpyAsync(f_out, out, sizeof(T), cudaMemcpyDeviceToHost, s) != cudaSuccess) return 1;
    if (cudaStreamSynchronize(s) != cudaSuccess) { set_error("quadratic kernel failed: %s", cudaGetErrorString(cudaGetLastError())); return 1; }
    return 0;
}

template <typename T>
__global__ void k_fg_halo_push(const T* x, i64 n, Peers peers, int R, int rank, int slot, unsigned long long seq) {
    if (threadIdx.x != 0) return;
    P2PBuf<T>* left = rank > 0 ? (P2PBuf<T>*)peers.p[rank - 1] : nullptr;
    P2PBuf<T>* right = rank < R - 1 ? (P2PBuf<T>*)peers.p[rank + 1] : nullptr;
    if (left) left->halo[slot][1] = x[0];
    if (right) right->halo[slot][0] = x[n - 1];
    __threadfence_system();
    if (left) *(volatile unsigned long long*)&left->hflag[slot][1] = seq;
    if (right) *(volatile unsigned long long*)&right->hflag[slot][0] = seq;
}
template <typename T>
__global__ void k_fg_halo_wait(Wk<T> w, P2PBuf<T>* mine, int R, int rank, int slot, unsigned long long seq, T* halo_out) {
    if (threadIdx.x != 0) return;
    const long long t0 = clock64();
    for (int side = 0; side < 2; ++side) {
        const bool need = side == 0 ? rank > 0 : rank < R - 1;
        T v = (T)0;
        if (need) {
            volatile unsigned long long* f = &mine->hflag[slot][side];
            while (*f != seq) { if (clock64() - t0 > LB_P2P_SPIN_LIMIT) { w.s->p2p_timeout = 1; break; } }
            __threadfence_system();
            v = *(volatile T*)&mine->halo[slot][side];
        }
// ... 72 lines not shown
        else if (op == 11) r = wdense::dtrsl<double>(a, m, col, b, 1);
        else if (op == 12) r = wdense::dtrsl<double>(a, m, col, b, 11);
        else if (op == 13) r = wdense::bmv<double>(m, a, b, col, c, c + 2 * m);
        else r = wdense::formt<double>(m, c, a, b, col, theta);
        if (threadIdx.x == 0) *info = r;
        return;
    }
    if (op == 15) {
        if (threadIdx.x == 0) {
            st->m = m; st->col = col; st->theta = theta; st->do_formk = 1; st->updatd = 0; st->do_delta = 0; st->iupdat = m + 1;
            st->restart = 0; st->in_body = 1; st->ev_n = 0;
            for (int q = 0; q < m * m; ++q) st->sy[q] = b[q];
        }
        __syncwarp();
        Red<double>* red = nullptr;
        w_formk_dense<double>(st, *red, m <= 5 ? 5 : (m <= 10 ? 10 : 20), (const double*)nullptr, c, a);
        if (threadIdx.x == 0) *info = st->restart ? 1 : 0;
        return;
    }
    if (threadIdx.x != 0) return;
    if (op == 0) *info = dense::dpofa<double>(a, m, col);
    else if (op == 1) *info = dense::dtrsl<double>(a, m, col, b, 1);
    else if (op == 2) *info = dense::dtrsl<double>(a, m, col, b, 11);
    else if (op == 3) *info = dense::bmv<double>(m, a, b, col, c, c + 2 * m);
    else if (op == 4) *info = dense::formt<double>(m, c, a, b, col, theta);
}
__global__ void k_test_dcsrch(double f, double g, double* stp, double stpmax, int* task, int* isave2, double* dsave13) {
    if (threadIdx.x != 0 || blockIdx.x != 0) return;
    dense::dcsrch<double>(f, g, *stp, 1.0e-3, 0.9, 0.1, 0.0, stpmax, *task, isave2[0], isave2[1], dsave13);
}
template <typename K>
__global__ void k_test_iota(int* v, i64 n) {
    for (i64 i = (i64)blockIdx.x * blockDim.x + threadIdx.x; i < n; i += (i64)gridDim.x * blockDim.x) v[i] = (int)i;
}
__global__ void k_test_heap_order(unsigned long long* k, int* v, i64 n, int* order_out) {
    if (threadIdx.x != 0 || blockIdx.x != 0) return;
    heap_build<unsigned long long>(k - 1, v - 1, n);
    for (i64 nleft = n; nleft > 0; --nleft) {
        unsigned long long out; int var;
        heap_pop<unsigned long long>(k - 1, v - 1, nleft, out, var);
        order_out[n - nleft] = var;
    }
}
__global__ void k_test_setctl(SortCtl* c, i64 n) { if (threadIdx.x == 0) { c->count = n; c->cur = 0; c->skip = 0; } }

extern "C" int lbfgsb_dev_trial_sums(lbfgsb_dev_t* h, lbfgsb_trial_sums_t* out);
extern "C" void lbfgsb_dev_trial_sums_commit(lbfgsb_dev_t* h);
template <typename T>
static TrialSums<T> trial_sums_of(Engine<T>* e, const T* l, const T* u, const int32_t* nbd) {
    TrialSums<T> ts; memset(&ts, 0, sizeof ts);
    lbfgsb_trial_sums_t pub;
    if (l && u && nbd && lbfgsb_dev_trial_sums((lbfgsb_dev_t*)e, &pub) == 0) {
        ts.d = (const T*)pub.d_dev; ts.l = l; ts.u = u; ts.nbd = nbd;
        ts.gd_part = (T*)pub.gd_part_dev; ts.pg_part = (T*)pub.pg_part_dev;
        lbfgsb_dev_trial_sums_commit((lbfgsb_dev_t*)e);
    }
    return ts;
}

struct BatchBase {
    virtual ~BatchBase() {}
    int real_kind;
};
template <typename T>
struct BatchEngine : BatchBase {
    BatchWk<T> bw;
    cudaStream_t stream = 0;
    bool own_stream = false;
    std::vector<void*> allocs;
    int* entry_dev = nullptr; int* entry_host = nullptr;
    char* hdr_host = nullptr;
    size_t header_bytes = 0;
    std::vector<char> started;
    int n_fg = 0, n_newx = 0, n_done = 0;
    i64 launches = 0;
    template <typename P> bool dalloc(P** p, size_t bytes) {
        void* q = nullptr;
        if (bytes == 0) bytes = 16;
        cudaError_t e = cudaMalloc(&q, bytes);
        if (e != cudaSuccess) { set_error("cudaMalloc(%zu) failed: %s", bytes, cudaGetErrorString(e)); return false; }
        allocs.push_back(q);
        *p = (P*)q;
        return true;
    }
    template <int MT> bool set_attr() {
        CK(cudaFuncSetAttribute(k_batch_setulb<T, MT>, cudaFuncAttributeMaxDynamicSharedMemorySize, (int)sizeof(BatchSm<T>)));
        return true;
    }
    bool init(int nprob, i64 n, int m, cudaStream_t st) {
        real_kind = (int)sizeof(T);
        memset(&bw, 0, sizeof bw);
        bw.nprob = nprob; bw.n = n; bw.m = m; bw.mt = (m <= 5) ? 5 : (m <= 10 ? 10 : 20);
        bw.ldw = (n + 31) / 32 * 32;
        if (st) stream = st;
        else { CK(cudaStreamCreateWithFlags(&stream, cudaStreamNonBlocking)); own_stream = true; }
        const size_t P = (size_t)nprob, vb = (size_t)bw.ldw * sizeof(T);
        if (!dalloc(&bw.ws, P * vb * m) || !dalloc(&bw.wy, P * vb * m)) return false;
        if (!dalloc(&bw.z, P * vb) || !dalloc(&bw.r, P * vb) || !dalloc(&bw.d, P * vb) || !dalloc(&bw.t, P * vb) || !dalloc(&bw.xp, P * vb) ||
            !dalloc(&bw.gold, P * vb) || !dalloc(&bw.bpt, P * vb)) return false;
        if (!dalloc(&bw.iwhere, P * bw.ldw * 4) || !dalloc(&bw.bpo, P * bw.ldw * 4) || !dalloc(&bw.state, P * bw.ldw)) return false;
        if (!dalloc(&bw.delta, P * sizeof(T) * 6 * LB_MMAX * LB_MMAX) || !dalloc(&bw.s, P * sizeof(DevState<T>))) return false;
        if (!dalloc(&entry_dev, P * sizeof(int)) || !dalloc(&bw.fgmask, P * sizeof(int))) return false;
        CK(cudaMemsetAsync(bw.fgmask, 0, P * sizeof(int), stream));
        CK(cudaMemsetAsync(bw.s, 0, P * sizeof(DevState<T>), stream));
        CK(cudaMemsetAsync(bw.ws, 0, P * vb * m, stream));
        CK(cudaMemsetAsync(bw.wy, 0, P * vb * m, stream));
// ... 273 lines not shown
    if (!b) return nullptr;
#define VSEL(E)                                                                                          \
    switch (which) { case 0: return E->w.z; case 1: return E->w.r; case 2: return E->w.d; case 3: return E->w.t; \
                     case 4: return E->w.xp; case 5: return E->w.ws; case 6: return E->w.wy; case 7: return E->w.iwhere; case 8: return E->w.gold; default: return nullptr; }
    if (b->real_kind == 8) { Engine<double>* e = (Engine<double>*)b; VSEL(e) }
    else { Engine<float>* e = (Engine<float>*)b; VSEL(e) }
}
int lbfgsb_dev_vector_copy(lbfgsb_dev_t* h, int32_t which, void* dst_dev, int64_t bytes) {
    void* src = lbfgsb_dev_vector(h, which);
    if (!src || !dst_dev || bytes < 0) return 1;
    EngineBase* b = (EngineBase*)h;
    const i64 ldw = (b->real_kind == 8) ? ((Engine<double>*)b)->w.ldw : ((Engine<float>*)b)->w.ldw;
    const i64 m = (b->real_kind == 8) ? ((Engine<double>*)b)->w.m : ((Engine<float>*)b)->w.m;
    const i64 cap = (which == 7) ? ldw * 4 : ((which == 5 || which == 6) ? m : 1) * ldw * (i64)b->real_kind;
    if (bytes > cap) { set_error("lbfgsb_dev_vector_copy: %lld bytes requested, vector %d holds %lld", (long long)bytes, (int)which, (long long)cap); return 1; }
    if (cudaDeviceSynchronize() != cudaSuccess) return 1;
    return cudaMemcpy(dst_dev, src, (size_t)bytes, cudaMemcpyDeviceToDevice) != cudaSuccess;
}
int lbfgsb_dev_exchange_mode(lbfgsb_dev_t* h) {
    EngineBase* b = (EngineBase*)h;
    if (!b) return -1;
    if (b->real_kind == 8) { Engine<double>* e = (Engine<double>*)b; return e->R <= 1 ? 0 : (e->p2p ? 2 : 1); }
    Engine<float>* e = (Engine<float>*)b; return e->R <= 1 ? 0 : (e->p2p ? 2 : 1);
}
int lbfgsb_dev_counters(lbfgsb_dev_t* h, int64_t* launches, int64_t* syncs) {
    EngineBase* b = (EngineBase*)h;
    if (!b) return 1;
    if (b->real_kind == 8) { *launches = ((Engine<double>*)b)->launches; *syncs = ((Engine<double>*)b)->syncs; }
    else { *launches = ((Engine<float>*)b)->launches; *syncs = ((Engine<float>*)b)->syncs; }
    return 0;
}
void lbfgsb_dev_profile(lbfgsb_dev_t* h, int32_t enable) {
    EngineBase* b = (EngineBase*)h;
    if (!b) return;
    if (b->real_kind == 8) ((Engine<double>*)b)->profile = enable != 0; else ((Engine<float>*)b)->profile = enable != 0;
}
void lbfgsb_dev_set_tie_limit(lbfgsb_dev_t* h, int64_t max_breakpoints) {
    EngineBase* b = (EngineBase*)h;
    if (!b) return;
    i64 lim = max_breakpoints < 0 ? 0 : max_breakpoints;
    if (b->real_kind == 8) { Engine<double>* e = (Engine<double>*)b; cudaStreamSynchronize(e->stream); cudaMemcpy(&e->s_dev->tie_limit, &lim, sizeof lim, cudaMemcpyHostToDevice); }
    else { Engine<float>* e = (Engine<float>*)b; cudaStreamSynchronize(e->stream); cudaMemcpy(&e->s_dev->tie_limit, &lim, sizeof lim, cudaMemcpyHostToDevice); }
}
int lbfgsb_dev_tie_stats(lbfgsb_dev_t* h, int64_t* replays, int64_t* not_replayed) {
    EngineBase* b = (EngineBase*)h;
    if (!b) return 1;
    i64 ev = 0;
    cudaError_t e;
    if (b->real_kind == 8) { Engine<double>* g = (Engine<double>*)b; cudaStreamSynchronize(g->stream); e = cudaMemcpy(&ev, &g->s_dev->tie_events, sizeof ev, cudaMemcpyDeviceToHost); *replays = g->tie_replays; }
    else { Engine<float>* g = (Engine<float>*)b; cudaStreamSynchronize(g->stream); e = cudaMemcpy(&ev, &g->s_dev->tie_events, sizeof ev, cudaMemcpyDeviceToHost); *replays = g->tie_replays; }
    *not_replayed = ev;
    return e != cudaSuccess;
}
void lbfgsb_dev_profile_reset(lbfgsb_dev_t* h) {
    EngineBase* b = (EngineBase*)h;
    if (!b) return;
    for (int q = 0; q < F_COUNT; ++q) {
        if (b->real_kind == 8) { ((Engine<double>*)b)->fam_ms[q] = 0; ((Engine<double>*)b)->fam_calls[q] = 0; }
        else { ((Engine<float>*)b)->fam_ms[q] = 0; ((Engine<float>*)b)->fam_calls[q] = 0; }
    }
}
int lbfgsb_dev_profile_read(lbfgsb_dev_t* h, int32_t cap, char* names, double* ms, double* bytes, int64_t* calls) {
    EngineBase* b = (EngineBase*)h;
    if (!b) return 0;
    int k = 0;
    for (int q = 0; q < F_COUNT && k < cap; ++q, ++k) {
        snprintf(names + 32 * k, 32, "%s", fam_name[q]);
        if (b->real_kind == 8) { ms[k] = ((Engine<double>*)b)->fam_ms[q]; calls[k] = ((Engine<double>*)b)->fam_calls[q]; }
        else { ms[k] = ((Engine<float>*)b)->fam_ms[q]; calls[k] = ((Engine<float>*)b)->fam_calls[q]; }
        bytes[k] = 0;
    }
    return k;
}

int64_t lbfgsb_problem_scratch_bytes(void) { return (int64_t)sizeof(double) * (LBFGSB_GRID + 8); }
int lbfgsb_problem_rosenbrock_f64(int64_t n, const double* x, double* g, double* f_out, void* st, int32_t first, int32_t last,
                                  double xl, double xr, void* scratch) {
    return rosenbrock_impl<double>(n, x, g, f_out, st, first, last, xl, xr, scratch);
}
int lbfgsb_problem_rosenbrock_f32(int64_t n, const float* x, float* g, float* f_out, void* st, int32_t first, int32_t last,
                                  float xl, float xr, void* scratch) {
    return rosenbrock_impl<float>(n, x, g, f_out, st, first, last, xl, xr, scratch);
}

int lbfgsb_problem_rosenbrock_halo_f64(int64_t n, const double* x, double* g, double* f_part_dev, void* st, int32_t first,
                                       int32_t last, const double* halo_dev, void* scratch) {
    return rosenbrock_halo_impl<double>(n, x, g, f_part_dev, st, first, last, halo_dev, scratch);
}
int lbfgsb_problem_quadratic_halo_f64(int64_t n, const double* x, double* g, double* f_part_dev, void* st, int64_t off,
                                      uint64_t seed, const double* halo_dev, void* scratch) {
    return quadratic_halo_impl<double>(n, x, g, f_part_dev, st, off, seed, halo_dev, scratch);
}
int lbfgsb_dev_trial_sums(lbfgsb_dev_t* h, lbfgsb_trial_sums_t* out) {
    EngineBase* b = (EngineBase*)h;
    if (!b || !out) return 1;
    memset(out, 0, sizeof *out);
    if (b->real_kind == 8) {
        Engine<double>* e = (Engine<double>*)b;
        out->d_dev = e->w.d; out->gd_part_dev = LB_SLOT(e->w.part, 0); out->pg_part_dev = LB_SLOT(e->w.part, 1); out->n = e->n;
    } else {
        Engine<float>* e = (Engine<float>*)b;
        out->d_dev = e->w.d; out->gd_part_dev = LB_SLOT(e->w.part, 0); out->pg_part_dev = LB_SLOT(e->w.part, 1); out->n = e->n;
    }
    out->grid = LBFGSB_GRID; out->block = LBFGSB_BLOCK; out->unroll = LBFGSB_UNROLL(b->real_kind); out->real_kind = b->real_kind;
    out->vec = LBFGSB_VEC(b->real_kind);
    return 0;
}
void lbfgsb_dev_trial_sums_commit(lbfgsb_dev_t* h) {
    EngineBase* b = (EngineBase*)h;
    if (!b) return;
    if (b->real_kind == 8) ((Engine<double>*)b)->trial_ready = true;
    else ((Engine<float>*)b)->trial_ready = true;
}
int lbfgsb_problem_fused_f64(lbfgsb_dev_t* hh, int32_t kind, const double* x, double* g, const double* l, const double* u,
                             const int32_t* nbd, double* f_out, uint64_t seed) {
    EngineBase* b = (EngineBase*)hh;
    if (!b || b->real_kind != 8) return 2;
    Engine<double>* e = (Engine<double>*)b;
    if (e->R > 1) return 2;
    typedef double T;
    if (!e->fg_scratch) {
        if (!e->dalloc(&e->fg_scratch, sizeof(T) * (LBFGSB_GRID + 8)) || !e->dalloc(&e->fg_out, sizeof(T) * 8)) return 1;
        if (cudaMallocHost((void**)&e->fg_host, sizeof(T) * 8) != cudaSuccess) return 1;
    }
    cudaStream_t st = e->stream;
    const TrialSums<T> ts = trial_sums_of<T>(e, l, u, nbd);
    if (kind == 0) {
        k_rosenbrock<T><<<LBFGSB_GRID, LBFGSB_BLOCK, 0, st>>>(e->n, x, g, e->fg_scratch, 1, 1, (T)0, (T)0, nullptr, ts);
        k_rosenbrock_final<T><<<1, 32, 0, st>>>(e->fg_scratch, e->fg_out);
    } else {
        const unsigned long long seedp = seed * 0x9E3779B97F4A7C15ULL;
        k_quadratic<T><<<LBFGSB_GRID, LBFGSB_BLOCK, 0, st>>>(e->n, x, g, e->fg_scratch, 0, seedp, (T)0, (T)0, nullptr, ts);
        k_sum_final<T><<<1, 32, 0, st>>>(e->fg_scratch, e->fg_out);
    }
    if (cudaMemcpyAsync(e->fg_host, e->fg_out, sizeof(T), cudaMemcpyDeviceToHost, st) != cudaSuccess) return 1;
    if (cudaStreamSynchronize(st) != cudaSuccess) { set_error("objective kernel failed: %s", cudaGetErrorString(cudaGetLastError())); return 1; }
    *f_out = e->fg_host[0];
    return 0;
}
int lbfgsb_problem_sharded_f64(lbfgsb_dev_t* hh, int32_t kind, const double* x, double* g, const double* l, const double* u,
                               const int32_t* nbd, double* f_out, uint64_t seed) {
    EngineBase* b = (EngineBase*)hh;
    if (!b || b->real_kind != 8) return 2;
    Engine<double>* e = (Engine<double>*)b;
    if (e->R <= 1 || !e->p2p) return 2;
    typedef double T;
    const TrialSums<T> ts = trial_sums_of<T>(e, l, u, nbd);
    if (!e->fg_scratch) {
        if (!e->dalloc(&e->fg_scratch, sizeof(T) * (LBFGSB_GRID + 8)) || !e->dalloc(&e->fg_out, sizeof(T) * 8)) return 1;
        if (cudaMallocHost((void**)&e->fg_host, sizeof(T) * 8) != cudaSuccess) return 1;
    }
    cudaStream_t st = e->stream;
    const unsigned long long seq = ++e->fg_seq;
    const int slot = (int)(seq & 1ULL);
    T* halo = e->fg_out + 2;
    T* fpart = e->fg_out + 4;
    k_fg_halo_push<T><<<1, 32, 0, st>>>(x, e->n, e->peers, e->R, e->rank, slot, seq);
    k_fg_halo_wait<T><<<1, 32, 0, st>>>(e->w, e->p2p_local, e->R, e->rank, slot, seq, halo);
    if (kind == 0) {
        k_rosenbrock<T><<<LBFGSB_GRID, LBFGSB_BLOCK, 0, st>>>(e->n, x, g, e->fg_scratch, e->rank == 0 ? 1 : 0, e->rank == e->R - 1 ? 1 : 0, (T)0, (T)0, halo, ts);
        k_rosenbrock_final<T><<<1, 32, 0, st>>>(e->fg_scratch, fpart);
    } else {
        const unsigned long long seedp = seed * 0x9E3779B97F4A7C15ULL;
        k_quadratic<T><<<LBFGSB_GRID, LBFGSB_BLOCK, 0, st>>>(e->n, x, g, e->fg_scratch, e->offset, seedp, (T)0, (T)0, halo, ts);
        k_sum_final<T><<<1, 32, 0, st>>>(e->fg_scratch, fpart);
    }
    k_fg_fsum_push<T><<<1, 32, 0, st>>>(fpart, e->peers, e->R, e->rank, slot, seq);
    k_fg_fsum_wait<T><<<1, 32, 0, st>>>(e->w, e->p2p_local, e->R, slot, seq, e->fg_out);
    if (cudaMemcpyAsync(e->fg_host, e->fg_out, sizeof(T), cudaMemcpyDeviceToHost, st) != cudaSuccess) return 1;
    if (cudaStreamSynchronize(st) != cudaSuccess) { set_error("sharded objective failed: %s", cudaGetErrorString(cudaGetLastError())); return 1; }
    *f_out = e->fg_host[0];
    return 0;
}
int lbfgsb_problem_quadratic_f64(int64_t n, const double* x, double* g, double* f_out, void* st, int64_t off, uint64_t seed,
                                 double xl, double xr, void* scratch) {
    return quadratic_impl<double>(n, x, g, f_out, st, off, seed, xl, xr, scratch);
}
int lbfgsb_problem_quadratic_f32(int64_t n, const float* x, float* g, float* f_out, void* st, int64_t off, uint64_t seed,
                                 float xl, float xr, void* scratch) {
    return quadratic_impl<float>(n, x, g, f_out, st, off, seed, xl, xr, scratch);
}

int lbfgsb_test_projgr_f64(int64_t n, const double* l, const double* u, const int32_t* nbd, const double* x, const double* g,
                           double* out) {
    Wk<double> w; memset(&w, 0, sizeof w);
    DevState<double>* s = nullptr; double* part = nullptr;
    if (cudaMalloc(&s, sizeof(DevState<double>)) || cudaMalloc(&part, sizeof(double) * (LBFGSB_GRID + 1))) return 1;
    int one = 1;
    cudaMemcpy(&s->go, &one, sizeof(int), cudaMemcpyHostToDevice);
    w.n = n; w.l = l; w.u = u; w.nbd = nbd; w.x = (double*)x; w.g = (double*)g; w.part = part; w.s = s;
    k_projgr<double><<<LBFGSB_GRID, LBFGSB_BLOCK>>>(w);
    std::vector<double> hp(LBFGSB_GRID);
    cudaError_t e = cudaMemcpy(hp.data(), part, sizeof(double) * LBFGSB_GRID, cudaMemcpyDeviceToHost);
    double r = 0; for (double v : hp) r = v > r ? v : r;
    *out = r;
    cudaFree(s); cudaFree(part);
    return e != cudaSuccess;
}
int lbfgsb_test_sum_f64(int64_t n, const double* a, const double* b, double* out) { return test_sum_impl<double>(n, a, b, out); }
int lbfgsb_test_sum_f32(int64_t n, const float* a, const float* b, float* out) { return test_sum_impl<float>(n, a, b, out); }

int lbfgsb_test_sort_f64(int64_t n, const double* t, int32_t* order_out, double* sorted_out) {
    typedef unsigned long long K;
    K *k0, *k1; int *v0, *v1, *cnt; SortCtl* ctl;
    if (cudaMalloc(&k0, 8 * n) || cudaMalloc(&k1, 8 * n) || cudaMalloc(&v0, 4 * n) || cudaMalloc(&v1, 4 * n) ||
        cudaMalloc(&cnt, 4 * 256 * LB_RS_GRID) || cudaMalloc(&ctl, sizeof(SortCtl))) return 1;
    cudaMemcpy(k0, t, 8 * n, cudaMemcpyDeviceToDevice);
    k_test_iota<K><<<256, 256>>>(v0, n);
    k_test_setctl<<<1, 32>>>(ctl, n);
    for (int pass = 0; pass < 8; ++pass) {
        k_rs_hist<K><<<LB_RS_GRID, 256>>>(k0, k1, ctl, pass * 8, cnt);
        k_rs_scan<<<1, 1024>>>(cnt, ctl, LB_RS_GRID);
        k_rs_scatter<K><<<LB_RS_GRID, 256>>>(k0, k1, v0, v1, ctl, pass * 8, cnt);
        k_rs_flip<<<1, 32>>>(ctl);
    }
    SortCtl hc;
    cudaMemcpy(&hc, ctl, sizeof hc, cudaMemcpyDeviceToHost);
// ... 141 lines not shown
```

### lbfgsb_b200/csrc/kernels_stream.cuh

```cuda
#pragma once
#include "common.cuh"

template <typename T>
struct Wk {
    i64 n, ldw;
    i64 off;
    int m;
    T *ws, *wy;
    T *z, *r, *d, *t, *xp;
    T* gold;
    int* iwhere;
    unsigned char* state;
    T* part;
    i64* ipart;
    T* part2;
    i64* ipart2;
    DevState<T>* s;
    T* x; const T* l; const T* u; const int* nbd; T* g;
    int bp_hint;
};

#define LB_SLOT(part, k) ((part) + (i64)(k) * LBFGSB_GRID)
#define LB_INF(T) ((T)INFINITY)
#define LB_I64MAX 0x7fffffffffffffffLL

template <typename T>
__global__ void __launch_bounds__(LBFGSB_BLOCK) k_errclb(Wk<T> w) {
    constexpr int VEC = Real<T>::VEC;
    i64 k6 = -1, k7 = -1;
    LB_FOR_TILES(T, w.n, base) {
        T l[VEC], u[VEC]; int nb[VEC];
        ldv<T>(w.l, base, w.n, l); ldv<T>(w.u, base, w.n, u); ldvi<T>(w.nbd, base, w.n, nb);
#pragma unroll
        for (int v = 0; v < VEC; ++v) {
            i64 i = base + v;
            if (i < w.n) {
                if (nb[v] < 0 || nb[v] > 3) k6 = i;
                if (nb[v] == 2 && l[v] > u[v]) k7 = i;
            }
        }
    }
    i64 m6 = k6, m7 = k7;
#pragma unroll
    for (int off = 16; off >= 1; off >>= 1) {
        i64 o6 = shfl_xor_t<i64>(m6, off), o7 = shfl_xor_t<i64>(m7, off);
        m6 = o6 > m6 ? o6 : m6; m7 = o7 > m7 ? o7 : m7;
    }
    __shared__ i64 s6[LBFGSB_BLOCK / 32], s7[LBFGSB_BLOCK / 32];
    if ((threadIdx.x & 31) == 0) { s6[threadIdx.x >> 5] = m6; s7[threadIdx.x >> 5] = m7; }
    __syncthreads();
    if (threadIdx.x == 0) {
        for (int q = 1; q < LBFGSB_BLOCK / 32; ++q) { m6 = s6[q] > m6 ? s6[q] : m6; m7 = s7[q] > m7 ? s7[q] : m7; }
        LB_SLOT(w.ipart, 0)[blockIdx.x] = m6;
        LB_SLOT(w.ipart, 1)[blockIdx.x] = m7;
    }
}

template <typename T>
__global__ void __launch_bounds__(LBFGSB_BLOCK) k_active(Wk<T> w) {
    constexpr int VEC = Real<T>::VEC;
    if (!w.s->go) return;
    __shared__ i64 smi[LBFGSB_BLOCK / 32];
    i64 nbdd = 0, prj = 0, cns = 0, nbx = 0;
    LB_FOR_TILES(T, w.n, base) {
        T x[VEC], l[VEC], u[VEC]; int nb[VEC], iw[VEC], st[VEC];
        ldv<T>(w.x, base, w.n, x); ldv<T>(w.l, base, w.n, l); ldv<T>(w.u, base, w.n, u);
        ldvi<T>(w.nbd, base, w.n, nb);
#pragma unroll
        for (int v = 0; v < VEC; ++v) {
            iw[v] = 0; st[v] = 3;
            if (base + v < w.n) {
                if (nb[v] > 0) {
                    if (nb[v] <= 2 && x[v] <= l[v]) {
                        if (x[v] < l[v]) { prj = 1; x[v] = l[v]; }
                        nbdd++;
                    } else if (nb[v] >= 2 && x[v] >= u[v]) {
                        if (x[v] > u[v]) { prj = 1; x[v] = u[v]; }
                        nbdd++;
                    }
                }
                if (nb[v] != 2) nbx = 1;
                if (nb[v] == 0) iw[v] = -1;
                else {
                    cns = 1;
                    iw[v] = (nb[v] == 2 && u[v] - l[v] <= (T)0) ? 3 : 0;
                }
            }
        }
        stv<T>(w.x, base, w.n, x);
        stvi<T>(w.iwhere, base, w.n, iw);
        stvb<T>(w.state, base, w.n, st);
    }
    i64 r0 = block_isum(nbdd, smi), r1 = block_isum(prj, smi), r2 = block_isum(cns, smi), r3 = block_isum(nbx, smi);
    if (threadIdx.x == 0) {
        LB_SLOT(w.ipart, 0)[blockIdx.x] = r0; LB_SLOT(w.ipart, 1)[blockIdx.x] = r1;
        LB_SLOT(w.ipart, 2)[blockIdx.x] = r2; LB_SLOT(w.ipart, 3)[blockIdx.x] = r3;
    }
}

template <typename T>
__device__ __forceinline__ T projg_one(T x, T g, T l, T u, int nb) {
    T gi = g;
    if (nb != 0) {
        if (gi < (T)0) { if (nb >= 2) gi = dense::tmax(x - u, gi); }
        else           { if (nb <= 2) gi = dense::tmin(x - l, gi); }
    }
    return fabs(gi);
}

template <typename T>
__global__ void __launch_bounds__(LBFGSB_BLOCK) k_projgr(Wk<T> w) {
    constexpr int VEC = Real<T>::VEC;
    if (!w.s->go) return;
    __shared__ T sm[LBFGSB_BLOCK / 32];
    T acc = (T)0;
    LB_FOR_TILES(T, w.n, base) {
        T x[VEC], l[VEC], u[VEC], g[VEC]; int nb[VEC];
        ldv<T>(w.x, base, w.n, x); ldv<T>(w.g, base, w.n, g); ldv<T>(w.l, base, w.n, l);
        ldv<T>(w.u, base, w.n, u); ldvi<T>(w.nbd, base, w.n, nb);
#pragma unroll
        for (int v = 0; v < VEC; ++v)
            if (base + v < w.n) acc = dense::tmax(acc, projg_one<T>(x[v], g[v], l[v], u[v], nb[v]));
    }
    T r = block_max<T>(acc, sm);
    if (threadIdx.x == 0) LB_SLOT(w.part, 0)[blockIdx.x] = r;
}

template <typename T>
__device__ __forceinline__ T cauchy_dir(int iw, T g) { return (iw == 0 || iw == -1) ? -g : (T)0; }

template <typename T>
__global__ void __launch_bounds__(LBFGSB_BLOCK) k_gcp_freev(Wk<T> w) {
    constexpr int VEC = Real<T>::VEC;
    const DevState<T>* s = w.s;
    if (!s->go || !s->in_body || s->cauchy_mode == 1 || s->fuse_gf) return;
    const i64 n = w.n;
    const T tsum = s->tsum;
    const bool axpy = (s->cauchy_mode == 0) && (tsum != (T)0);
    const bool lazy = (s->cauchy_mode == 0) && s->lazy_gcp;
    const bool cnt = (s->iter > 0 && s->cnstnd);
    __shared__ i64 smi[LBFGSB_BLOCK / 32];
    i64 nfr = 0, nen = 0, nle = 0;
    LB_FOR_TILES(T, n, base) {
        int iw[VEC], st[VEC];
        ldvi<T>(w.iwhere, base, n, iw); ldvb<T>(w.state, base, n, st);
        if (lazy) {
            T z[VEC];
            ldv<T>(w.x, base, n, z);
            if (axpy) {
                T g[VEC];
                ldv<T>(w.g, base, n, g);
#pragma unroll
// ... 232 lines not shown
```

### lbfgsb_b200/csrc/kernels_tma.cuh

```cuda
#pragma once
#include "kernels_stream.cuh"
#include "tma_pipe.cuh"

template <typename T, int MT> struct SubT { static constexpr int v = (sizeof(T) * MT <= 80) ? 256 : 128; };

template <typename T> struct SpecializeFullHistory { static constexpr bool value = sizeof(T) == 4; };
template <bool B> struct BoolC { static constexpr bool value = B; };

#define LB_DYN_STAGES(dyn) (dyn)

template <typename T>
__device__ __forceinline__ void pipe_add_w(PipeSrc* ps, const Wk<T>& w, int head0, int count, unsigned slot) {
    int pj = head0;
    for (int j = 0; j < count; ++j) {
        pipe_add(ps, w.wy + (i64)pj * w.ldw, (int)sizeof(T), slot);
        pipe_add(ps, w.ws + (i64)pj * w.ldw, (int)sizeof(T), slot);
        pj = (pj + 1 == w.m) ? 0 : pj + 1;
    }
}

template <typename T, int MT>
__global__ void __launch_bounds__(LB_TMA_THREADS, 1) k_update(Wk<T> w) {
    constexpr int VEC = Real<T>::VEC;
    constexpr int SUBT = SubT<T, MT>::v;
    typedef PipeGeom<T, SUBT> G;
    extern __shared__ __align__(128) char dyn[];
    __shared__ unsigned long long full[2 * LB_PIPE_STAGES];
    __shared__ PipeSrc ps;
    __shared__ T sm[(2 * MT + 1) * (LBFGSB_BLOCK / 32)];
    const DevState<T>* s = w.s;
    if (!s->go || !s->do_update || s->fuse_uc) return;
    const i64 n = w.n;
    const int col = s->col, m = s->m, head0 = s->head - 1, itail0 = s->itail - 1;
    const T stp = s->stp;
    if (threadIdx.x == 0) {
        pipe_begin(&ps);
        pipe_add(&ps, w.g, sizeof(T), G::REAL_SLOT);
        pipe_add(&ps, w.gold, sizeof(T), G::REAL_SLOT);
        pipe_add(&ps, w.d, sizeof(T), G::REAL_SLOT);
        pipe_add_w<T>(&ps, w, head0, col - 1, G::REAL_SLOT);
        pipe_end(&ps);
    }
    T acc[2 * MT + 1];
#pragma unroll
    for (int k = 0; k < 2 * MT + 1; ++k) acc[k] = (T)0;
    T* wsn = w.ws + (i64)itail0 * w.ldw;
    T* wyn = w.wy + (i64)itail0 * w.ldw;
    (void)m;
    tma_pass<T, SUBT>(n, &ps, LB_DYN_STAGES(dyn), full, [&](i64 base, const char* sb, int lt) {
        T g[VEC], r[VEC], d[VEC];
        lds_real<T>(sb, 0 * G::REAL_SLOT, lt, g);
        lds_real<T>(sb, 1 * G::REAL_SLOT, lt, r);
        lds_real<T>(sb, 2 * G::REAL_SLOT, lt, d);
#pragma unroll
        for (int v = 0; v < VEC; ++v) {
            r[v] = g[v] - r[v];
            if (stp != (T)1) d[v] = stp * d[v];
            if (base + v < n) acc[0] = acc[0] + r[v] * r[v];
        }
#pragma unroll
        for (int j = 0; j < MT; ++j) {
            if (j < col - 1) {
// ... 17 lines not shown

template <typename T>
struct CauchyScan {
    T bk; i64 ibk, nbr, nfc, bnd;
    __device__ __forceinline__ void init() { bk = LB_INF(T); ibk = LB_I64MAX; nbr = 0; nfc = 0; bnd = 1; }
};
template <typename T>
__device__ __forceinline__ void cauchy_classify_one(T x, T l, T u, T g, int nb, int& iw, T& d, bool& mv, T& d2acc,
                                                    CauchyScan<T>& cs, i64 gidx, T& tbp) {
    tbp = (T)-1;
    const T neggi = -g;
    T tl = (T)0, tu = (T)0;
    if (iw != 3 && iw != -1) {
        if (nb <= 2) tl = x - l;
        if (nb >= 2) tu = u - x;
        const bool xlower = nb <= 2 && tl <= (T)0;
        const bool xupper = nb >= 2 && tu <= (T)0;
        iw = 0;
        if (xlower) { if (neggi <= (T)0) iw = 1; }
        else if (xupper) { if (neggi >= (T)0) iw = 2; }
        else { if (fabs(neggi) <= (T)0) iw = -3; }
    }
    if (iw == 0 || iw == -1) {
        mv = true;
        d = neggi;
        d2acc = d2acc + neggi * neggi;
        T tb; bool hasb = false;
        if (nb <= 2 && nb != 0 && neggi < (T)0) { tb = tl / (-neggi); hasb = true; }
        else if (nb >= 2 && neggi > (T)0) { tb = tu / neggi; hasb = true; }
        if (hasb) {
            tbp = tb;
            cs.nbr++;
            if (tb < cs.bk) { cs.bk = tb; cs.ibk = gidx; }
        } else {
            cs.nfc++;
            if (fabs(neggi) > (T)0) cs.bnd = 0;
        }
    }
}
template <typename T, int MT>
__device__ __forceinline__ void cauchy_scan_store(const Wk<T>& w, CauchyScan<T>& cs, T* smv, i64* smi) {
    block_argmin<T>(cs.bk, cs.ibk, smv, smi);
    i64 r1 = block_isum(cs.nbr, smi), r2 = block_isum(cs.nfc, smi);
    i64 r3 = -block_isum(cs.bnd ? 0 : 1, smi);
    if (threadIdx.x == 0) {
        LB_SLOT(w.part2, 2 * MT + 1)[blockIdx.x] = cs.bk;
        LB_SLOT(w.ipart2, 0)[blockIdx.x] = cs.ibk;
        LB_SLOT(w.ipart2, 1)[blockIdx.x] = r1;
        LB_SLOT(w.ipart2, 2)[blockIdx.x] = r2;
        LB_SLOT(w.ipart2, 3)[blockIdx.x] = (r3 < 0) ? 0 : 1;
    }
}

template <typename T, int MT>
__global__ void __launch_bounds__(LB_TMA_THREADS, 1) k_cauchy_classify(Wk<T> w) {
    constexpr int VEC = Real<T>::VEC;
    constexpr int SUBT = SubT<T, MT>::v;
    typedef PipeGeom<T, SUBT> G;
    extern __shared__ __align__(128) char dyn[];
    __shared__ unsigned long long full[2 * LB_PIPE_STAGES];
    __shared__ PipeSrc ps;
    __shared__ T sm[(2 * MT + 1) * (LBFGSB_BLOCK / 32)];
    __shared__ T smv[LBFGSB_BLOCK / 32];
    __shared__ i64 smi[LBFGSB_BLOCK / 32];
    const DevState<T>* s = w.s;
    if (!s->go || !s->in_body || s->classify_done) return;
    const int mode = s->cauchy_mode;
    const i64 n = w.n;
    if (mode != 0) {
        if (threadIdx.x >= LBFGSB_BLOCK) return;
        LB_FOR_TILES(T, n, base) {
            T x[VEC];
            ldv<T>(w.x, base, n, x);
            stv<T>(w.z, base, n, x);
        }
        return;
    }
    const int col = s->col, head0 = s->head - 1;
    constexpr unsigned OX = 0, OG = G::REAL_SLOT, OL = 2 * G::REAL_SLOT, OU = 3 * G::REAL_SLOT, ONB = 4 * G::REAL_SLOT,
                       OIW = ONB + G::INT_SLOT, OW = OIW + G::INT_SLOT;
    if (threadIdx.x == 0) {
        pipe_begin(&ps);
        pipe_add(&ps, w.x, sizeof(T), G::REAL_SLOT);
        pipe_add(&ps, w.g, sizeof(T), G::REAL_SLOT);
        pipe_add(&ps, w.l, sizeof(T), G::REAL_SLOT);
        pipe_add(&ps, w.u, sizeof(T), G::REAL_SLOT);
        pipe_add(&ps, w.nbd, 4, G::INT_SLOT);
        pipe_add(&ps, w.iwhere, 4, G::INT_SLOT);
        pipe_add_w<T>(&ps, w, head0, col, G::REAL_SLOT);
        pipe_end(&ps);
    }
    T acc[2 * MT + 1];
#pragma unroll
    for (int k = 0; k < 2 * MT + 1; ++k) acc[k] = (T)0;
    CauchyScan<T> cs; cs.init();
    tma_pass<T, SUBT>(n, &ps, LB_DYN_STAGES(dyn), full, [&](i64 base, const char* sb, int lt) {
        T x[VEC], l[VEC], u[VEC], g[VEC], d[VEC];
        int nb[VEC], iw[VEC];
        lds_real<T>(sb, OX, lt, x); lds_real<T>(sb, OG, lt, g); lds_real<T>(sb, OL, lt, l); lds_real<T>(sb, OU, lt, u);
        lds_int<T>(sb, ONB, lt, nb); lds_int<T>(sb, OIW, lt, iw);
        bool mv[VEC]; T tk[VEC];
#pragma unroll
        for (int v = 0; v < VEC; ++v) {
            mv[v] = false; d[v] = (T)0; tk[v] = (T)-1;
            if (base + v < n) cauchy_classify_one<T>(x[v], l[v], u[v], g[v], nb[v], iw[v], d[v], mv[v], acc[2 * MT], cs, base + v + w.off, tk[v]);
        }
        if (w.bp_hint) { stv<T>(w.r, base, n, tk); stv<T>(w.z, base, n, x); }
        stvi<T>(w.iwhere, base, n, iw);
#pragma unroll
        for (int j = 0; j < MT; ++j) {
            if (j < col) {
                T wy[VEC], wsv[VEC];
                lds_real<T>(sb, OW + (2 * j) * G::REAL_SLOT, lt, wy);
                lds_real<T>(sb, OW + (2 * j + 1) * G::REAL_SLOT, lt, wsv);
#pragma unroll
                for (int v = 0; v < VEC; ++v)
                    if (mv[v]) {
                        acc[j] = acc[j] + wy[v] * d[v];
                        acc[MT + j] = acc[MT + j] + wsv[v] * d[v];
                    }
            }
        }
    });
    block_sum_store<T, 2 * MT + 1>(acc, 2 * MT + 1, sm, w.part2);
    cauchy_scan_store<T, MT>(w, cs, smv, smi);
}
template <typename T, int MT> constexpr unsigned smem_classify() { return pipe_smem_bytes<T, SubT<T, MT>::v>(4 + 2 * MT, 2, 0); }

template <typename T, int MT>
__global__ void __launch_bounds__(LB_TMA_THREADS, 1) k_formk_gram(Wk<T> w) {
    constexpr int VEC = Real<T>::VEC;
    constexpr int SUBT = SubT<T, MT>::v;
    typedef PipeGeom<T, SUBT> G;
    extern __shared__ __align__(128) char dyn[];
    __shared__ unsigned long long full[2 * LB_PIPE_STAGES];
    __shared__ PipeSrc ps;
    __shared__ T sm[4 * MT * (LBFGSB_BLOCK / 32)];
    const DevState<T>* s = w.s;
    if (!s->go || !s->in_body || !s->do_formk || !s->updatd) return;
    const i64 n = w.n;
    const int col = s->col, head0 = s->head - 1;
    if (threadIdx.x == 0) {
        pipe_begin(&ps);
        pipe_add_w<T>(&ps, w, head0, col, G::REAL_SLOT);
        pipe_add(&ps, w.state, 1, G::BYTE_SLOT);
        pipe_end(&ps);
    }
    const unsigned ost = 2u * (unsigned)col * G::REAL_SLOT;
    const unsigned olast = 2u * (unsigned)(col - 1) * G::REAL_SLOT;
    T acc[4 * MT];
#pragma unroll
    for (int k = 0; k < 4 * MT; ++k) acc[k] = (T)0;
    tma_pass<T, SUBT>(n, &ps, LB_DYN_STAGES(dyn), full, [&](i64 base, const char* sb, int lt) {
        int st[VEC];
        lds_byte<T>(sb, ost, lt, st);
        T wyl[VEC], wsl[VEC];
        lds_real<T>(sb, olast, lt, wyl);
        lds_real<T>(sb, olast + G::REAL_SLOT, lt, wsl);
#pragma unroll
        for (int j = 0; j < MT; ++j) {
            if (j < col) {
                T wy[VEC], wsv[VEC];
                lds_real<T>(sb, (2 * j) * G::REAL_SLOT, lt, wy);
                lds_real<T>(sb, (2 * j + 1) * G::REAL_SLOT, lt, wsv);
#pragma unroll
                for (int v = 0; v < VEC; ++v) {
                    if (base + v < n) {
                        if (st[v] & 1) {
                            acc[j] = acc[j] + wyl[v] * wy[v];
                            acc[3 * MT + j] = acc[3 * MT + j] + wsv[v] * wyl[v];
                        } else {
                            acc[MT + j] = acc[MT + j] + wsl[v] * wsv[v];
                            acc[2 * MT + j] = acc[2 * MT + j] + wsl[v] * wy[v];
                        }
                    }
                }
            }
        }
    });
    block_sum_store<T, 4 * MT>(acc, 4 * MT, sm, w.part);
// ... 26 lines not shown
        pipe_end(&ps);
    }
    const unsigned ost = OW + 2u * (unsigned)col * G::REAL_SLOT;
    T a1[MT], a2[MT], acc[2 * MT];
#pragma unroll
    for (int j = 0; j < MT; ++j) {
        a1[j] = (j < col) ? s->a[j] : (T)0;
        a2[j] = (j < col) ? theta * s->a[col + j] : (T)0;
        acc[j] = (T)0; acc[MT + j] = (T)0;
    }
    tma_pass<T, SUBT>(n, &ps, LB_DYN_STAGES(dyn), full, [&](i64 base, const char* sb, int lt) {
        int st[VEC];
        lds_byte<T>(sb, ost, lt, st);
        bool fr[VEC]; bool any = false;
#pragma unroll
        for (int v = 0; v < VEC; ++v) { fr[v] = (base + v < n) && (st[v] & 1); any |= fr[v]; }
        if (!any) return;
        T z[VEC], x[VEC], g[VEC], r[VEC];
        lds_real<T>(sb, OG, lt, g); lds_real<T>(sb, OZ, lt, z); lds_real<T>(sb, OX, lt, x);
#pragma unroll
        for (int v = 0; v < VEC; ++v) r[v] = uc ? -g[v] : (-theta * (z[v] - x[v]) - g[v]);
        if (!uc) {
#pragma unroll
            for (int j = 0; j < MT; ++j) {
                if (j < col) {
                    T wy[VEC], wsv[VEC];
                    lds_real<T>(sb, OW + (2 * j) * G::REAL_SLOT, lt, wy);
                    lds_real<T>(sb, OW + (2 * j + 1) * G::REAL_SLOT, lt, wsv);
#pragma unroll
                    for (int v = 0; v < VEC; ++v) r[v] = r[v] + wy[v] * a1[j] + wsv[v] * a2[j];
                }
            }
        }
#pragma unroll
        for (int j = 0; j < MT; ++j) {
            if (j < col) {
                T wy[VEC], wsv[VEC];
                lds_real<T>(sb, OW + (2 * j) * G::REAL_SLOT, lt, wy);
                lds_real<T>(sb, OW + (2 * j + 1) * G::REAL_SLOT, lt, wsv);
#pragma unroll
                for (int v = 0; v < VEC; ++v)
                    if (fr[v]) {
                        acc[j] = acc[j] + wy[v] * r[v];
                        acc[MT + j] = acc[MT + j] + wsv[v] * r[v];
                    }
            }
        }
        stv<T>(w.r, base, n, r);
    });
    block_sum_store<T, 2 * MT>(acc, 2 * MT, sm, w.part2);
}
template <typename T, int MT> constexpr unsigned smem_cmprlb() { return pipe_smem_bytes<T, SubT<T, MT>::v>(3 + 2 * MT, 0, 1); }

template <typename T, int MT>
__global__ void __launch_bounds__(LB_TMA_THREADS, 1) k_subsm_step(Wk<T> w) {
    constexpr int VEC = Real<T>::VEC;
    constexpr int SUBT = SubT<T, MT>::v;
    typedef PipeGeom<T, SUBT> G;
    extern __shared__ __align__(128) char dyn[];
    __shared__ unsigned long long full[2 * LB_PIPE_STAGES];
    __shared__ PipeSrc ps;
    __shared__ T sm[LBFGSB_BLOCK / 32];
    __shared__ i64 smi[LBFGSB_BLOCK / 32];
    const DevState<T>* s = w.s;
    if (!s->go || !s->in_body || !s->do_subspace) return;
    const i64 n = w.n;
    const int col = s->col, head0 = s->head - 1;
    const T theta = s->theta, rtheta = (T)1 / theta;
    constexpr unsigned OZ = 0, OX = G::REAL_SLOT, OG = 2 * G::REAL_SLOT, OR = 3 * G::REAL_SLOT, OL = 4 * G::REAL_SLOT,
                       OU = 5 * G::REAL_SLOT, OW = 6 * G::REAL_SLOT;
    if (threadIdx.x == 0) {
        pipe_begin(&ps);
        pipe_add(&ps, w.z, sizeof(T), G::REAL_SLOT);
        pipe_add(&ps, w.x, sizeof(T), G::REAL_SLOT);
        pipe_add(&ps, w.g, sizeof(T), G::REAL_SLOT);
        pipe_add(&ps, w.r, sizeof(T), G::REAL_SLOT);
        pipe_add(&ps, w.l, sizeof(T), G::REAL_SLOT);
        pipe_add(&ps, w.u, sizeof(T), G::REAL_SLOT);
        pipe_add_w<T>(&ps, w, head0, col, G::REAL_SLOT);
        pipe_add(&ps, w.nbd, 4, G::INT_SLOT);
        pipe_add(&ps, w.state, 1, G::BYTE_SLOT);
        pipe_end(&ps);
    }
    const unsigned onb = OW + 2u * (unsigned)col * G::REAL_SLOT, ost = onb + G::INT_SLOT;
    T wv1[MT], wv2[MT];
#pragma unroll
    for (int j = 0; j < MT; ++j) { wv1[j] = (j < col) ? s->wv[j] : (T)0; wv2[j] = (j < col) ? s->wv[col + j] : (T)0; }
    T acc[1]; acc[0] = (T)0;
    i64 iwd = 0;
    tma_pass<T, SUBT>(n, &ps, LB_DYN_STAGES(dyn), full, [&](i64 base, const char* sb, int lt) {
        int st[VEC];
        lds_byte<T>(sb, ost, lt, st);
        bool fr[VEC]; bool any = false;
#pragma unroll
        for (int v = 0; v < VEC; ++v) { fr[v] = (base + v < n) && (st[v] & 1); any |= fr[v]; }
        T z[VEC], x[VEC], g[VEC];
        lds_real<T>(sb, OZ, lt, z); lds_real<T>(sb, OX, lt, x); lds_real<T>(sb, OG, lt, g);
        stv<T>(w.xp, base, n, z);
        if (any) {
            T dk[VEC], l[VEC], u[VEC]; int nb[VEC];
            lds_real<T>(sb, OR, lt, dk); lds_real<T>(sb, OL, lt, l); lds_real<T>(sb, OU, lt, u);
            lds_int<T>(sb, onb, lt, nb);
#pragma unroll
            for (int j = 0; j < MT; ++j) {
                if (j < col) {
                    T wy[VEC], wsv[VEC];
                    lds_real<T>(sb, OW + (2 * j) * G::REAL_SLOT, lt, wy);
                    lds_real<T>(sb, OW + (2 * j + 1) * G::REAL_SLOT, lt, wsv);
#pragma unroll
                    for (int v = 0; v < VEC; ++v) dk[v] = dk[v] + wy[v] * wv1[j] / theta + wsv[v] * wv2[j];
                }
            }
#pragma unroll
            for (int v = 0; v < VEC; ++v) {
                dk[v] = rtheta * dk[v];
                if (fr[v]) {
                    T xk = z[v];
                    if (nb[v] != 0) {
                        if (nb[v] == 1) { z[v] = dense::tmax(l[v], xk + dk[v]); if (z[v] == l[v]) iwd = 1; }
                        else if (nb[v] == 2) {
                            xk = dense::tmax(l[v], xk + dk[v]);
                            z[v] = dense::tmin(u[v], xk);
                            if (z[v] == l[v] || z[v] == u[v]) iwd = 1;
                        } else if (nb[v] == 3) { z[v] = dense::tmin(u[v], xk + dk[v]); if (z[v] == u[v]) iwd = 1; }
                    } else z[v] = xk + dk[v];
                }
            }
            stv<T>(w.r, base, n, dk);
            stv<T>(w.z, base, n, z);
        }
#pragma unroll
        for (int v = 0; v < VEC; ++v)
            if (base + v < n) acc[0] = acc[0] + (z[v] - x[v]) * g[v];
    });
    block_sum_store<T, 1>(acc, 1, sm, w.part);
    i64 r0 = block_isum(iwd, smi);
    if (threadIdx.x == 0) LB_SLOT(w.ipart, 0)[blockIdx.x] = r0;
}
template <typename T, int MT> constexpr unsigned smem_subsm() { return pipe_smem_bytes<T, SubT<T, MT>::v>(6 + 2 * MT, 1, 1); }

template <typename T, int MT> constexpr bool fused_passes_ok() { return sizeof(T) * MT <= 80; }

template <typename T, int MT>
__global__ void __launch_bounds__(LB_TMA_THREADS, 1) k_update_classify(Wk<T> w) {
    constexpr int VEC = Real<T>::VEC;
    constexpr int SUBT = SubT<T, MT>::v;
    typedef PipeGeom<T, SUBT> G;
    extern __shared__ __align__(128) char dyn[];
    __shared__ unsigned long long full[2 * LB_PIPE_STAGES];
    __shared__ PipeSrc ps;
    __shared__ T sm[(2 * MT + 1) * (LBFGSB_BLOCK / 32)];
    __shared__ T smv[LBFGSB_BLOCK / 32];
    __shared__ i64 smi[LBFGSB_BLOCK / 32];
    const DevState<T>* s = w.s;
    if (!s->go || !s->do_update || !s->fuse_uc) return;
    const i64 n = w.n;
    const int col = s->col, head0 = s->head - 1, itail0 = s->itail - 1;
    const T stp = s->stp;
    constexpr unsigned OG = 0, OR = G::REAL_SLOT, OD = 2 * G::REAL_SLOT, OX = 3 * G::REAL_SLOT, OL = 4 * G::REAL_SLOT,
                       OU = 5 * G::REAL_SLOT, ONB = 6 * G::REAL_SLOT, OIW = ONB + G::INT_SLOT, OW = OIW + G::INT_SLOT;
    if (threadIdx.x == 0) {
        pipe_begin(&ps);
        pipe_add(&ps, w.g, sizeof(T), G::REAL_SLOT);
        pipe_add(&ps, w.gold, sizeof(T), G::REAL_SLOT);
        pipe_add(&ps, w.d, sizeof(T), G::REAL_SLOT);
        pipe_add(&ps, w.x, sizeof(T), G::REAL_SLOT);
        pipe_add(&ps, w.l, sizeof(T), G::REAL_SLOT);
        pipe_add(&ps, w.u, sizeof(T), G::REAL_SLOT);
        pipe_add(&ps, w.nbd, 4, G::INT_SLOT);
        pipe_add(&ps, w.iwhere, 4, G::INT_SLOT);
        pipe_add_w<T>(&ps, w, head0, col - 1, G::REAL_SLOT);
        pipe_end(&ps);
    }
    T au[2 * MT + 1], ac[2 * MT + 1];
#pragma unroll
    for (int k = 0; k < 2 * MT + 1; ++k) { au[k] = (T)0; ac[k] = (T)0; }
    CauchyScan<T> cs; cs.init();
    T* wsn = w.ws + (i64)itail0 * w.ldw;
    T* wyn = w.wy + (i64)itail0 * w.ldw;
    auto pass = [&](auto full_c) {
    constexpr bool FULLC = decltype(full_c)::value;
    tma_pass<T, SUBT>(n, &ps, LB_DYN_STAGES(dyn), full, [&](i64 base, const char* sb, int lt) {
        T g[VEC], y[VEC], sn[VEC];
        lds_real<T>(sb, OG, lt, g);
        lds_real<T>(sb, OR, lt, y);
        lds_real<T>(sb, OD, lt, sn);
#pragma unroll
        for (int v = 0; v < VEC; ++v) {
            y[v] = g[v] - y[v];
            if (stp != (T)1) sn[v] = stp * sn[v];
            if (base + v < n) au[0] = au[0] + y[v] * y[v];
        }
        stv<T>(wsn, base, n, sn);
        stv<T>(wyn, base, n, y);
        T x[VEC], l[VEC], u[VEC], dc[VEC];
        int nb[VEC], iw[VEC];
        lds_real<T>(sb, OX, lt, x); lds_real<T>(sb, OL, lt, l); lds_real<T>(sb, OU, lt, u);
        lds_int<T>(sb, ONB, lt, nb); lds_int<T>(sb, OIW, lt, iw);
        bool mv[VEC]; T tk[VEC];
#pragma unroll
        for (int v = 0; v < VEC; ++v) {
            mv[v] = false; dc[v] = (T)0; tk[v] = (T)-1;
            if (base + v < n) cauchy_classify_one<T>(x[v], l[v], u[v], g[v], nb[v], iw[v], dc[v], mv[v], ac[2 * MT], cs, base + v + w.off, tk[v]);
        }
        if (w.bp_hint) { stv<T>(w.r, base, n, tk); stv<T>(w.z, base, n, x); }
        stvi<T>(w.iwhere, base, n, iw);
#pragma unroll
        for (int j = 0; j < MT; ++j) {
            if (FULLC ? (j < MT - 1) : (j < col - 1)) {
                T wy[VEC], wsv[VEC];
                lds_real<T>(sb, OW + (2 * j) * G::REAL_SLOT, lt, wy);
                lds_real<T>(sb, OW + (2 * j + 1) * G::REAL_SLOT, lt, wsv);
#pragma unroll
                for (int v = 0; v < VEC; ++v) {
                    if (base + v < n) {
                        au[1 + j] = au[1 + j] + sn[v] * wy[v];
                        au[1 + MT + j] = au[1 + MT + j] + wsv[v] * sn[v];
                    }
                    if (mv[v]) {
                        ac[j] = ac[j] + wy[v] * dc[v];
                        ac[MT + j] = ac[MT + j] + wsv[v] * dc[v];
                    }
                }
            } else if (FULLC ? (j == MT - 1) : (j == col - 1)) {
#pragma unroll
                for (int v = 0; v < VEC; ++v)
                    if (mv[v]) {
                        ac[j] = ac[j] + y[v] * dc[v];
                        ac[MT + j] = ac[MT + j] + sn[v] * dc[v];
                    }
            }
        }
    });
    };
    if constexpr (SpecializeFullHistory<T>::value) { if (col == MT) pass(BoolC<true>{}); else pass(BoolC<false>{}); }
    else pass(BoolC<false>{});
    block_sum_store<T, 2 * MT + 1>(au, 2 * MT + 1, sm, w.part);
    block_sum_store<T, 2 * MT + 1>(ac, 2 * MT + 1, sm, w.part2);
    cauchy_scan_store<T, MT>(w, cs, smv, smi);
}
template <typename T, int MT> constexpr unsigned smem_update_classify() { return pipe_smem_bytes<T, SubT<T, MT>::v>(6 + 2 * (MT - 1), 2, 0); }

template <typename T, int MT, int GF>
__global__ void __launch_bounds__(LB_TMA_THREADS, 1) k_formk_cmprlb(Wk<T> w) {
    constexpr int VEC = Real<T>::VEC;
    constexpr int SUBT = SubT<T, MT>::v;
    typedef PipeGeom<T, SUBT> G;
    extern __shared__ __align__(128) char dyn[];
    __shared__ unsigned long long full[2 * LB_PIPE_STAGES];
    __shared__ PipeSrc ps;
    __shared__ T sm[4 * MT * (LBFGSB_BLOCK / 32)];
    __shared__ T coef[2 * MT];
    __shared__ i64 smi[LBFGSB_BLOCK / 32];
    const DevState<T>* s = w.s;
    if (!s->go || s->pause || !s->in_body || !s->do_subspace) return;
    constexpr bool gf = GF != 0;
    if (s->fuse_gf != GF) return;
    const bool gram = s->do_formk && s->updatd;
    const i64 n = w.n;
    const int col = s->col, head0 = s->head - 1;
    const T theta = s->theta;
    const bool uc = (!s->cnstnd && col > 0);
    const T tsum = s->tsum;
    const bool axpy = tsum != (T)0;
    const bool cnt = (s->iter > 0 && s->cnstnd);
    constexpr unsigned OG = 0, OX = G::REAL_SLOT, OZ = 2 * G::REAL_SLOT;
    constexpr unsigned OW = (GF == 1 ? 2u : 3u) * G::REAL_SLOT;
    if (threadIdx.x == 0) {
        pipe_begin(&ps);
        pipe_add(&ps, w.g, sizeof(T), G::REAL_SLOT);
        pipe_add(&ps, w.x, sizeof(T), G::REAL_SLOT);
        if (GF != 1) pipe_add(&ps, w.z, sizeof(T), G::REAL_SLOT);
        pipe_add_w<T>(&ps, w, head0, col, G::REAL_SLOT);
        pipe_add(&ps, w.state, 1, G::BYTE_SLOT);
        if (gf) pipe_add(&ps, w.iwhere, 4, G::INT_SLOT);
        pipe_end(&ps);
    }
    if (threadIdx.x < 2 * MT) {
        const int j = threadIdx.x % MT;
        coef[threadIdx.x] = (j < col) ? ((threadIdx.x < MT) ? s->a[j] : theta * s->a[col + j]) : (T)0;
    }
    T af[4 * MT], aw[2 * MT];
#pragma unroll
    for (int k = 0; k < 4 * MT; ++k) af[k] = (T)0;
#pragma unroll
    for (int k = 0; k < 2 * MT; ++k) aw[k] = (T)0;
    int nfr = 0, nen = 0, nle = 0;
    auto pass = [&](auto full_c) {
    constexpr bool FULLC = decltype(full_c)::value;
    const int colv = FULLC ? MT : col;
    const bool gramv = FULLC ? true : gram, ucv = FULLC ? false : uc;
    const unsigned ost = OW + 2u * (unsigned)colv * G::REAL_SLOT;
    const unsigned oiw = ost + G::BYTE_SLOT;
    const unsigned olast = OW + 2u * (unsigned)(colv - 1) * G::REAL_SLOT;
// ... 74 lines not shown
                            else { af[2 * MT + j] = af[2 * MT + j] + py; af[MT + j] = af[MT + j] + psv; }
                        }
                    }
                    if (!ucv) {
#pragma unroll
                        for (int v = 0; v < VEC; ++v) r[v] = r[v] + wy[v] * a1 + wsv[v] * a2;
                    }
                }
            }
        }
        if (!any) return;
        {
            T wyn[VEC], wsn[VEC];
            if (PREF) { lds_real_v<T>(sb, OW, lt, wyn); lds_real_v<T>(sb, OW + G::REAL_SLOT, lt, wsn); }
#pragma unroll
            for (int j = 0; j < MT; ++j) {
                if (j < col) {
                    T wy[VEC], wsv[VEC];
                    if (PREF) {
#pragma unroll
                        for (int v = 0; v < VEC; ++v) { wy[v] = wyn[v]; wsv[v] = wsn[v]; }
                        if (j + 1 < MT) {
                            lds_real_v<T>(sb, OW + (2 * j + 2) * G::REAL_SLOT, lt, wyn);
                            lds_real_v<T>(sb, OW + (2 * j + 3) * G::REAL_SLOT, lt, wsn);
                        }
                    } else {
                        lds_real<T>(sb, OW + (2 * j) * G::REAL_SLOT, lt, wy);
                        lds_real<T>(sb, OW + (2 * j + 1) * G::REAL_SLOT, lt, wsv);
                    }
#pragma unroll
                    for (int v = 0; v < VEC; ++v) {
                        const T py = wy[v] * r[v], psv = wsv[v] * r[v];
                        if (fr[v]) { aw[j] = aw[j] + py; aw[MT + j] = aw[MT + j] + psv; }
                    }
                }
            }
        }
        stv<T>(w.r, base, n, r);
    });
    };
    pass(BoolC<false>{});
    if (gram) block_sum_store<T, 4 * MT>(af, 4 * MT, sm, w.part);
    block_sum_store<T, 2 * MT>(aw, 2 * MT, sm, w.part2);
    if (gf) {
        i64 r0 = block_isum((i64)nfr, smi), r1 = block_isum((i64)nen, smi), r2 = block_isum((i64)nle, smi);
        if (threadIdx.x == 0) {
            LB_SLOT(w.ipart, 0)[blockIdx.x] = r0; LB_SLOT(w.ipart, 1)[blockIdx.x] = r1;
            LB_SLOT(w.ipart, 2)[blockIdx.x] = r2;
        }
    }
}
template <typename T, int MT> constexpr unsigned smem_formk_cmprlb() { return pipe_smem_bytes<T, SubT<T, MT>::v>(3 + 2 * MT, 1, 1); }

template <typename T, int MT, int PASS>
__global__ void __launch_bounds__(LB_TMA_THREADS, 1) k_subsm_lsinit(Wk<T> w) {
    constexpr int VEC = Real<T>::VEC;
    constexpr int SUBT = SubT<T, MT>::v;
    typedef PipeGeom<T, SUBT> G;
    extern __shared__ __align__(128) char dyn[];
    __shared__ unsigned long long full[2 * LB_PIPE_STAGES];
    __shared__ PipeSrc ps;
    __shared__ T sm[2 * (LBFGSB_BLOCK / 32)];
    __shared__ T smm[LBFGSB_BLOCK / 32];
    __shared__ i64 smi[LBFGSB_BLOCK / 32];
    const DevState<T>* s = w.s;
    if (!s->go || s->pause || !s->in_body || !s->do_subspace) return;
    const bool spec = s->spec_step != 0;
    if (PASS == 1 && !(spec && s->do_backtrack)) return;
    const i64 n = w.n;
    const int col = s->col, head0 = s->head - 1;
    const T theta = s->theta, rtheta = (T)1 / theta;
    const bool bounds = (s->cnstnd && s->iter != 0);
    const bool lz = s->lazy_z != 0;
    const T tsum = s->tsum;
    const bool axpy = tsum != (T)0;
    constexpr unsigned OX = 0, OG = G::REAL_SLOT, OL = 2 * G::REAL_SLOT, OU = 3 * G::REAL_SLOT, OR = 4 * G::REAL_SLOT,
                       OZ = 5 * G::REAL_SLOT;
    const unsigned OW = (lz ? 5u : 6u) * G::REAL_SLOT;
    if (threadIdx.x == 0) {
        pipe_begin(&ps);
        pipe_add(&ps, PASS == 1 ? w.t : w.x, sizeof(T), G::REAL_SLOT);
        pipe_add(&ps, w.g, sizeof(T), G::REAL_SLOT);
        pipe_add(&ps, w.l, sizeof(T), G::REAL_SLOT);
        pipe_add(&ps, w.u, sizeof(T), G::REAL_SLOT);
        pipe_add(&ps, w.r, sizeof(T), G::REAL_SLOT);
        if (!lz) pipe_add(&ps, w.z, sizeof(T), G::REAL_SLOT);
        pipe_add_w<T>(&ps, w, head0, col, G::REAL_SLOT);
        pipe_add(&ps, w.nbd, 4, G::INT_SLOT);
        pipe_add(&ps, w.state, 1, G::BYTE_SLOT);
        pipe_end(&ps);
    }
    T wv1[MT], wv2[MT];
#pragma unroll
    for (int j = 0; j < MT; ++j) { wv1[j] = (j < col) ? s->wv[j] : (T)0; wv2[j] = (j < col) ? s->wv[col + j] : (T)0; }
    T acc[2]; acc[0] = (T)0; acc[1] = (T)0;
    T smx = LB_INF(T);
    i64 iwd = 0;
    auto pass = [&](auto full_c) {
    constexpr bool FULLC = decltype(full_c)::value;
    const unsigned onb = OW + 2u * (unsigned)(FULLC ? MT : col) * G::REAL_SLOT, ost = onb + G::INT_SLOT;
    tma_pass<T, SUBT>(n, &ps, LB_DYN_STAGES(dyn), full, [&](i64 base, const char* sb, int lt) {
        int st[VEC];
        lds_byte<T>(sb, ost, lt, st);
        bool fr[VEC]; bool any = false;
#pragma unroll
        for (int v = 0; v < VEC; ++v) { fr[v] = (base + v < n) && (st[v] & 1); any |= fr[v]; }
        if (PASS == 1 && !any && !lz) return;
        T z[VEC], x[VEC], g[VEC];
        lds_real<T>(sb, OX, lt, x); lds_real<T>(sb, OG, lt, g);
        if (lz) {
#pragma unroll
            for (int v = 0; v < VEC; ++v) z[v] = axpy ? (x[v] + tsum * ((st[v] & 4) ? -g[v] : (T)0)) : x[v];
        } else lds_real<T>(sb, OZ, lt, z);
        T dk[VEC];
        if (any) {
            lds_real<T>(sb, OR, lt, dk);
#pragma unroll
            for (int j = 0; j < MT; ++j) {
                if (FULLC || j < col) {
                    T wy[VEC], wsv[VEC];
                    lds_real<T>(sb, OW + (2 * j) * G::REAL_SLOT, lt, wy);
                    lds_real<T>(sb, OW + (2 * j + 1) * G::REAL_SLOT, lt, wsv);
#pragma unroll
                    for (int v = 0; v < VEC; ++v) dk[v] = dk[v] + wy[v] * wv1[j] / theta + wsv[v] * wv2[j];
                }
            }
#pragma unroll
            for (int v = 0; v < VEC; ++v) dk[v] = rtheta * dk[v];
        }
        if (PASS == 1) {
            if (any) stv<T>(w.r, base, n, dk);
            if (lz) stv<T>(w.z, base, n, z);
            return;
        }
        T l[VEC], u[VEC]; int nb[VEC];
        lds_real<T>(sb, OL, lt, l); lds_real<T>(sb, OU, lt, u);
        lds_int<T>(sb, onb, lt, nb);
        if (!spec) stv<T>(w.xp, base, n, z);
        if (any) {
#pragma unroll
            for (int v = 0; v < VEC; ++v) {
                if (fr[v]) {
                    T xk = z[v];
                    if (nb[v] != 0) {
                        if (nb[v] == 1) { z[v] = dense::tmax(l[v], xk + dk[v]); if (z[v] == l[v]) iwd = 1; }
                        else if (nb[v] == 2) {
                            xk = dense::tmax(l[v], xk + dk[v]);
                            z[v] = dense::tmin(u[v], xk);
                            if (z[v] == l[v] || z[v] == u[v]) iwd = 1;
                        } else if (nb[v] == 3) { z[v] = dense::tmin(u[v], xk + dk[v]); if (z[v] == u[v]) iwd = 1; }
                    } else z[v] = xk + dk[v];
                }
            }
            if (!spec) {
                stv<T>(w.r, base, n, dk);
                stv<T>(w.z, base, n, z);
            }
        } else if (!spec && lz) stv<T>(w.z, base, n, z);
        T d[VEC];
#pragma unroll
        for (int v = 0; v < VEC; ++v) {
            d[v] = z[v] - x[v];
            if (base + v < n) { acc[0] = acc[0] + d[v] * d[v]; acc[1] = acc[1] + d[v] * g[v]; }
        }
        stv<T>(w.d, base, n, d); stv<T>(w.t, base, n, x); stv<T>(w.gold, base, n, g);
        if (spec) stv<T>(w.x, base, n, z);
        if (bounds) {
#pragma unroll
            for (int v = 0; v < VEC; ++v) {
                if (base + v < n && nb[v] != 0) {
                    const T a1 = d[v];
                    if (a1 < (T)0 && nb[v] <= 2) {
                        const T a2 = l[v] - x[v];
                        const T cand = (a2 >= (T)0) ? (T)0 : a2 / a1;
                        smx = dense::tmin(smx, cand);
                    } else if (a1 > (T)0 && nb[v] >= 2) {
                        const T a2 = u[v] - x[v];
                        const T cand = (a2 <= (T)0) ? (T)0 : a2 / a1;
                        smx = dense::tmin(smx, cand);
                    }
                }
            }
        }
    });
    };
    if constexpr (SpecializeFullHistory<T>::value && PASS == 0) { if (col == MT) pass(BoolC<true>{}); else pass(BoolC<false>{}); }
    else pass(BoolC<false>{});
    if (PASS == 1) return;
    T ddp[1]; ddp[0] = acc[1];
    block_sum_store<T, 1>(ddp, 1, sm, w.part);
// ... 7 lines not shown
```

Before: 93.93.

## Compress per-variable bounds into byte class indices with a shared lookup table

Adds a pass after the active-set setup that finds the distinct (l, u, nbd) combinations and, if there are no more than 64, writes a one-byte class index per variable plus a small table in device state. The classify, subspace step, update-classify and lsinit kernels, and the Rosenbrock trial sums, get compact variants that stream the byte index instead of two f64 bound arrays and an int32 nbd array. This is meant to cut per-iteration memory traffic in these bandwidth-bound passes. In exchange it adds three setup kernels, doubles the template instantiations, and changes the checkpoint format.

```diff
diff --git a/include/lbfgsb_b200.h b/include/lbfgsb_b200.h
--- a/include/lbfgsb_b200.h
+++ b/include/lbfgsb_b200.h
@@ -81,6 +81,7 @@
 void lbfgsb_dev_profile_reset(lbfgsb_dev_t* h);
 void lbfgsb_dev_set_tie_limit(lbfgsb_dev_t* h, int64_t max_breakpoints);
 int lbfgsb_dev_tie_stats(lbfgsb_dev_t* h, int64_t* replays, int64_t* not_replayed);
+int lbfgsb_dev_bound_classes(lbfgsb_dev_t* h, int32_t* count);
 
 int lbfgsb_problem_rosenbrock_f64(int64_t n, const double* x_dev, double* g_dev, double* f_out, void* cuda_stream,
                                   int32_t first, int32_t last, double xl, double xr, void* scratch_dev);
diff --git a/lbfgsb_b200/__init__.py b/lbfgsb_b200/__init__.py
--- a/lbfgsb_b200/__init__.py
+++ b/lbfgsb_b200/__init__.py
@@ -76,6 +76,7 @@
         L.lbfgsb_dev_set_tie_limit.argtypes = [C.c_void_p, C.c_int64]
         L.lbfgsb_dev_set_tie_limit.restype = None
         L.lbfgsb_dev_tie_stats.argtypes = [C.c_void_p, C.c_void_p, C.c_void_p]
+        L.lbfgsb_dev_bound_classes.argtypes = [C.c_void_p, C.c_void_p]
         L.lbfgsb_dev_profile_read.argtypes = [C.c_void_p, C.c_int32, C.c_void_p, C.c_void_p, C.c_void_p, C.c_void_p]
         L.lbfgsb_dev_nccl_init.restype = C.c_void_p
         L.lbfgsb_dev_nccl_init.argtypes = [C.c_void_p, C.c_int32, C.c_int32]
@@ -332,6 +333,12 @@
         lib().lbfgsb_dev_tie_stats(C.c_void_p(self.h), C.byref(a), C.byref(b))
         return a.value, b.value
 
+    def bound_classes(self):
+        c = C.c_int32(0)
+        if lib().lbfgsb_dev_bound_classes(C.c_void_p(self.h), C.byref(c)) != 0:
+            raise RuntimeError(last_error())
+        return c.value
+
     def profile(self, on=True):
         lib().lbfgsb_dev_profile(C.c_void_p(self.h), 1 if on else 0)
 
diff --git a/lbfgsb_b200/csrc/common.cuh b/lbfgsb_b200/csrc/common.cuh
--- a/lbfgsb_b200/csrc/common.cuh
+++ b/lbfgsb_b200/csrc/common.cuh
@@ -9,6 +9,7 @@
 typedef long long i64;
 
 #define LB_MMAX 20
+#define LB_NCLS 64
 #define LB_KMAX (6 * LB_MMAX + 8)
 #define LB_IMAX 8
 
@@ -81,6 +82,7 @@
     int z_in_x;
     int save_z;
     int task, csave, info;
+    int nbcls;
     int col, head, itail, iupdat, iter, nfgv, nskip, ifun, iback, iword;
     int updatd, prjctd, cnstnd, boxed, wrk, bnded;
     int brackt, stage;
@@ -120,6 +122,7 @@
     T walkA[2 * LB_MMAX], walkB[2 * LB_MMAX];
     T snapA[2 * LB_MMAX], snapB[2 * LB_MMAX];
     T snap_f1, snap_f2, snap_tlast, snap_tprev2;
+    typename Real<T>::vec_t bcls_tab[LB_NCLS];
 };
 
 template <typename T> __device__ inline void ev_push(DevState<T>* s, int code, T a = (T)0, T b = (T)0) {
@@ -412,6 +415,32 @@
     } else {
 #pragma unroll
         for (int v = 0; v < VEC; ++v) if (base + v < n) p[base + v] = (unsigned char)in[v];
+    }
+}
+
+template <typename T>
+__host__ __device__ __forceinline__ void bound_key(T l, T u, int nb, typename Real<T>::key_t& kl, typename Real<T>::key_t& ku) {
+    typename Real<T>::key_t bl, bu;
+    memcpy(&bl, &l, sizeof bl); memcpy(&bu, &u, sizeof bu);
+    kl = (nb == 1 || nb == 2) ? bl : 0;
+    ku = (nb == 2 || nb == 3) ? bu : 0;
+}
+template <typename T>
+__device__ __forceinline__ void class_bounds(int c, const typename Real<T>::vec_t* tab, T& l, T& u, int& nb) {
+    const typename Real<T>::vec_t q = tab[c & (LB_NCLS - 1)];
+    l = q.x; u = q.y; nb = c >> 6;
+}
+template <typename T>
+__device__ __forceinline__ void ld_bounds(const T* l, const T* u, const int* nbd, const unsigned char* cls,
+                                          const typename Real<T>::vec_t* tab, i64 base, i64 n, T (&lo)[Real<T>::VEC],
+                                          T (&hi)[Real<T>::VEC], int (&nb)[Real<T>::VEC]) {
+    if (cls) {
+        int c[Real<T>::VEC];
+        ldvb<T>(cls, base, n, c);
+#pragma unroll
+        for (int v = 0; v < Real<T>::VEC; ++v) class_bounds<T>(c[v], tab, lo[v], hi[v], nb[v]);
+    } else {
+        ldv<T>(l, base, n, lo); ldv<T>(u, base, n, hi); ldvi<T>(nbd, base, n, nb);
     }
 }
 
diff --git a/lbfgsb_b200/csrc/engine.cu b/lbfgsb_b200/csrc/engine.cu
--- a/lbfgsb_b200/csrc/engine.cu
+++ b/lbfgsb_b200/csrc/engine.cu
@@ -80,12 +80,12 @@
 enum Fam {
     F_ERRCLB, F_ACTIVE, F_PROJGR, F_CLASSIFY, F_GCP_FREEV, F_FORMK_GRAM, F_FORMK_DELTA, F_CMPRLB_WV,
     F_SUBSM_STEP, F_BACKTRACK, F_LS_INIT, F_LS_STEP, F_LS_TRIAL, F_UPDATE, F_RESTORE, F_WALK_COMPACT,
-    F_WALK_SORT, F_WALK_SCAN, F_WALK_FIX, F_SCALAR, F_HASH, F_UPDATE_CLASSIFY, F_FORMK_CMPRLB, F_SUBSM_LSINIT, F_COUNT
+    F_WALK_SORT, F_WALK_SCAN, F_WALK_FIX, F_SCALAR, F_HASH, F_UPDATE_CLASSIFY, F_FORMK_CMPRLB, F_SUBSM_LSINIT, F_BCLS, F_COUNT
 };
 static const char* fam_name[F_COUNT] = {
     "errclb", "active", "projgr", "cauchy_classify", "gcp_freev", "formk_gram", "formk_delta", "cmprlb_wv",
     "subsm_step", "backtrack", "ls_init", "ls_step", "ls_trial", "update", "restore", "walk_compact",
-    "walk_sort", "walk_scan", "walk_fix", "scalar", "hash", "update_classify", "formk_cmprlb", "subsm_lsinit"};
+    "walk_sort", "walk_scan", "walk_fix", "scalar", "hash", "update_classify", "formk_cmprlb", "subsm_lsinit", "bound_classes"};
 
 __global__ void __launch_bounds__(256) k_publish(const unsigned* src, unsigned* dst_host, int words, volatile unsigned long long* flag_host,
                                                  unsigned long long seq) {
@@ -147,6 +147,8 @@
     bool x_changed = false, g_changed = false;
     bool walked_prev = false, walked_now = false, body_ran = false, bp_hint_ok = true, walk_gf_ok = true;
     bool started = false;
+    bool classes_ok = true, compact = false;
+    typename Real<T>::key_t* bcls_blk = nullptr; int* bcls_blkn = nullptr;
 
     bool p2p = false;
     P2PBuf<T>* p2p_local = nullptr;
@@ -231,6 +233,7 @@
         if (const char* e = getenv("LBFGSB_B200_NO_TIMERS")) { if (e[0] == '1') timers = false; }
         if (const char* e = getenv("LBFGSB_B200_NO_SMALL_ROUNDS")) { if (e[0] == '1') { small_rounds = false; small_sort = false; } }
         if (const char* e = getenv("LBFGSB_B200_NO_BP_HINT")) { if (e[0] == '1') { bp_hint_ok = false; walk_gf_ok = false; } }
+        if (const char* e = getenv("LBFGSB_B200_NO_BOUND_CLASSES")) { if (e[0] == '1') classes_ok = false; }
         if (!(mt == 5 ? set_smem_attrs<5>() : (mt == 10 ? set_smem_attrs<10>() : set_smem_attrs<20>()))) return false;
         for (int q = 0; q < F_COUNT; ++q) { fam_ms[q] = 0; fam_calls[q] = 0; }
         if (st) stream = st;
@@ -241,7 +244,8 @@
         const size_t vb = (size_t)w.ldw * sizeof(T);
         if (!dalloc(&w.ws, vb * m) || !dalloc(&w.wy, vb * m)) return false;
         if (!dalloc(&w.z, vb) || !dalloc(&w.r, vb) || !dalloc(&w.d, vb) || !dalloc(&w.t, vb) || !dalloc(&w.xp, vb) || !dalloc(&w.gold, vb)) return false;
-        if (!dalloc(&w.iwhere, (size_t)w.ldw * 4) || !dalloc(&w.state, (size_t)w.ldw)) return false;
+        if (!dalloc(&w.iwhere, (size_t)w.ldw * 4) || !dalloc(&w.state, (size_t)w.ldw) || !dalloc(&w.bcls, (size_t)w.ldw)) return false;
+        if (!dalloc(&bcls_blk, sizeof(*bcls_blk) * 2 * LB_NCLS * LBFGSB_GRID) || !dalloc(&bcls_blkn, sizeof(int) * LBFGSB_GRID)) return false;
         if (!dalloc(&w.part, sizeof(T) * LB_KMAX * LBFGSB_GRID) || !dalloc(&w.ipart, sizeof(i64) * LB_IMAX * LBFGSB_GRID)) return false;
         if (!dalloc(&w.part2, sizeof(T) * LB_KMAX * LBFGSB_GRID) || !dalloc(&w.ipart2, sizeof(i64) * LB_IMAX * LBFGSB_GRID)) return false;
         if (!dalloc(&s_dev, sizeof(DevState<T>))) return false;
@@ -422,9 +426,20 @@
         else if (mt == 10) kern<T, 10><<<LBFGSB_GRID, LB_TMA_THREADS, smemfn<T, 10>(), stream>>>(__VA_ARGS__); \
         else kern<T, 20><<<LBFGSB_GRID, LB_TMA_THREADS, smemfn<T, 20>(), stream>>>(__VA_ARGS__);              \
     } while (0)
+    template <int MT> void launch_classify() {
+        if (compact) k_cauchy_classify<T, MT, true><<<LBFGSB_GRID, LB_TMA_THREADS, smem_classify<T, MT, true>(), stream>>>(w);
+        else k_cauchy_classify<T, MT, false><<<LBFGSB_GRID, LB_TMA_THREADS, smem_classify<T, MT, false>(), stream>>>(w);
+    }
+    template <int MT> void launch_subsm_step() {
+        if (compact) k_subsm_step<T, MT, true><<<LBFGSB_GRID, LB_TMA_THREADS, smem_subsm<T, MT, true>(), stream>>>(w);
+        else k_subsm_step<T, MT, false><<<LBFGSB_GRID, LB_TMA_THREADS, smem_subsm<T, MT, false>(), stream>>>(w);
+    }
 
     template <int MT> void launch_update_classify() {
-        if constexpr (fused_passes_ok<T, MT>()) k_update_classify<T, MT><<<LBFGSB_GRID, LB_TMA_THREADS, smem_update_classify<T, MT>(), stream>>>(w);
+        if constexpr (fused_passes_ok<T, MT>()) {
+            if (compact) k_update_classify<T, MT, true><<<LBFGSB_GRID, LB_TMA_THREADS, smem_update_classify<T, MT, true>(), stream>>>(w);
+            else k_update_classify<T, MT, false><<<LBFGSB_GRID, LB_TMA_THREADS, smem_update_classify<T, MT, false>(), stream>>>(w);
+        }
     }
     template <int MT> void launch_formk_cmprlb() {
         if constexpr (fused_passes_ok<T, MT>()) k_formk_cmprlb<T, MT, 0><<<LBFGSB_GRID, LB_TMA_THREADS, smem_formk_cmprlb<T, MT>(), stream>>>(w);
@@ -435,27 +450,32 @@
     template <int MT> void launch_formk_cmprlb_gf2() {
         if constexpr (fused_passes_ok<T, MT>()) k_formk_cmprlb<T, MT, 2><<<LBFGSB_GRID, LB_TMA_THREADS, smem_formk_cmprlb<T, MT>(), stream>>>(w);
     }
-    template <int MT> void launch_subsm_lsinit() {
-        if constexpr (fused_passes_ok<T, MT>()) k_subsm_lsinit<T, MT, 0><<<LBFGSB_GRID, LB_TMA_THREADS, smem_subsm<T, MT>(), stream>>>(w);
-    }
-    template <int MT> void launch_subsm_dir() {
-        if constexpr (fused_passes_ok<T, MT>()) k_subsm_lsinit<T, MT, 1><<<LBFGSB_GRID, LB_TMA_THREADS, smem_subsm<T, MT>(), stream>>>(w);
-    }
+    template <int MT, int PASS> void launch_subsm_pass() {
+        if constexpr (fused_passes_ok<T, MT>()) {
+            if (compact) k_subsm_lsinit<T, MT, PASS, true><<<LBFGSB_GRID, LB_TMA_THREADS, smem_subsm<T, MT, true>(), stream>>>(w);
+            else k_subsm_lsinit<T, MT, PASS, false><<<LBFGSB_GRID, LB_TMA_THREADS, smem_subsm<T, MT, false>(), stream>>>(w);
+        }
+    }
+    template <int MT> void launch_subsm_lsinit() { launch_subsm_pass<MT, 0>(); }
+    template <int MT> void launch_subsm_dir() { launch_subsm_pass<MT, 1>(); }
 #define MTFUSED(fn) do { if (mt == 5) fn<5>(); else if (mt == 10) fn<10>(); else fn<20>(); } while (0)
 
     template <int MT> bool set_smem_attrs() {
         CK(cudaFuncSetAttribute(k_update<T, MT>, cudaFuncAttributeMaxDynamicSharedMemorySize, (int)smem_update<T, MT>()));
-        CK(cudaFuncSetAttribute(k_cauchy_classify<T, MT>, cudaFuncAttributeMaxDynamicSharedMemorySize, (int)smem_classify<T, MT>()));
         CK(cudaFuncSetAttribute(k_formk_gram<T, MT>, cudaFuncAttributeMaxDynamicSharedMemorySize, (int)smem_formk<T, MT>()));
         CK(cudaFuncSetAttribute(k_cmprlb_wv<T, MT>, cudaFuncAttributeMaxDynamicSharedMemorySize, (int)smem_cmprlb<T, MT>()));
-        CK(cudaFuncSetAttribute(k_subsm_step<T, MT>, cudaFuncAttributeMaxDynamicSharedMemorySize, (int)smem_subsm<T, MT>()));
+        return set_smem_attrs_cb<MT, false>() && set_smem_attrs_cb<MT, true>();
+    }
+    template <int MT, bool CB> bool set_smem_attrs_cb() {
+        CK(cudaFuncSetAttribute(k_cauchy_classify<T, MT, CB>, cudaFuncAttributeMaxDynamicSharedMemorySize, (int)smem_classify<T, MT, CB>()));
+        CK(cudaFuncSetAttribute(k_subsm_step<T, MT, CB>, cudaFuncAttributeMaxDynamicSharedMemorySize, (int)smem_subsm<T, MT, CB>()));
         if constexpr (fused_passes_ok<T, MT>()) {
-            CK(cudaFuncSetAttribute(k_update_classify<T, MT>, cudaFuncAttributeMaxDynamicSharedMemorySize, (int)smem_update_classify<T, MT>()));
+            CK(cudaFuncSetAttribute(k_update_classify<T, MT, CB>, cudaFuncAttributeMaxDynamicSharedMemorySize, (int)smem_update_classify<T, MT, CB>()));
             CK(cudaFuncSetAttribute(k_formk_cmprlb<T, MT, 0>, cudaFuncAttributeMaxDynamicSharedMemorySize, (int)smem_formk_cmprlb<T, MT>()));
             CK(cudaFuncSetAttribute(k_formk_cmprlb<T, MT, 1>, cudaFuncAttributeMaxDynamicSharedMemorySize, (int)smem_formk_cmprlb<T, MT>()));
             CK(cudaFuncSetAttribute(k_formk_cmprlb<T, MT, 2>, cudaFuncAttributeMaxDynamicSharedMemorySize, (int)smem_formk_cmprlb<T, MT>()));
-            CK(cudaFuncSetAttribute(k_subsm_lsinit<T, MT, 0>, cudaFuncAttributeMaxDynamicSharedMemorySize, (int)smem_subsm<T, MT>()));
-            CK(cudaFuncSetAttribute(k_subsm_lsinit<T, MT, 1>, cudaFuncAttributeMaxDynamicSharedMemorySize, (int)smem_subsm<T, MT>()));
+            CK(cudaFuncSetAttribute(k_subsm_lsinit<T, MT, 0, CB>, cudaFuncAttributeMaxDynamicSharedMemorySize, (int)smem_subsm<T, MT, CB>()));
+            CK(cudaFuncSetAttribute(k_subsm_lsinit<T, MT, 1, CB>, cudaFuncAttributeMaxDynamicSharedMemorySize, (int)smem_subsm<T, MT, CB>()));
         }
         return true;
     }
@@ -862,7 +882,7 @@
             bool gf2 = false;
             if (from <= PAUSE_CLASSIFY) {
                 phase(PH_CAUCHY);
-                begin(F_CLASSIFY); MTCALL(k_cauchy_classify, smem_classify, w); end(F_CLASSIFY);
+                begin(F_CLASSIFY); MTFUSED(launch_classify); end(F_CLASSIFY);
                 if (!site(site_cauchy(mt))) return false;
                 begin(F_SCALAR); s_cauchy<T><<<LS>>>(w, dist(), mt, fused ? 1 : 0); end(F_SCALAR);
             }
@@ -915,7 +935,7 @@
                 if (!site(site_wv(mt))) return false;
                 begin(F_SCALAR); s_subsm_dense<T><<<LS>>>(w, dist(), mt, fused ? 1 : 0); end(F_SCALAR);
                 if (fused) { begin(F_SUBSM_LSINIT); MTFUSED(launch_subsm_lsinit); end(F_SUBSM_LSINIT); }
-                else { begin(F_SUBSM_STEP); MTCALL(k_subsm_step, smem_subsm, w); end(F_SUBSM_STEP); }
+                else { begin(F_SUBSM_STEP); MTFUSED(launch_subsm_step); end(F_SUBSM_STEP); }
                 if (!site(site_subsm())) return false;
                 begin(F_SCALAR); s_subsm_post<T><<<LS>>>(w, dist(), fused ? 1 : 0); end(F_SCALAR);
             }
@@ -1104,7 +1124,15 @@
             begin(F_ACTIVE); k_active<T><<<LG>>>(w); end(F_ACTIVE);
             if (!site(site_active())) return false;
             s_active<T><<<LS>>>(w, dist()); launches++;
+            if (classes_ok) {
+                begin(F_BCLS);
+                k_bcls_collect<T><<<LG>>>(w, bcls_blk, bcls_blkn);
+                k_bcls_merge<T><<<1, 32, 0, stream>>>(w, bcls_blk, bcls_blkn);
+                k_bcls_write<T><<<LG>>>(w);
+                end(F_BCLS, 3);
+            }
             if (!sync_state()) return false;
+            compact = classes_ok && s_host->nbcls > 0;
             x_changed = true;
             return check_launch();
         }
@@ -1172,7 +1200,7 @@
         FILE* fp = fopen(write ? tmp.c_str() : path, write ? "wb" : "rb");
         if (!fp) { set_error("cannot open checkpoint file %s", write ? tmp.c_str() : path); return false; }
         CkHeader hd; memset(&hd, 0, sizeof hd);
-        memcpy(hd.magic, "LBB2CKP2", 8);
+        memcpy(hd.magic, "LBB2CKP3", 8);
         hd.n = n; hd.ldw = w.ldw; hd.n_global = n_global; hd.offset = offset; hd.m = m; hd.real_kind = (int)sizeof(T); hd.R = R; hd.rank = rank;
         hd.state_bytes = (i64)sizeof(DevState<T>);
         bool ok = true;
@@ -1203,11 +1231,11 @@
         xfer(s_dev, sizeof(DevState<T>));
         xfer(w.ws, vb * m); xfer(w.wy, vb * m);
         xfer(w.z, vb); xfer(w.r, vb); xfer(w.d, vb); xfer(w.t, vb); xfer(w.xp, vb); xfer(w.gold, vb);
-        xfer(w.iwhere, (size_t)w.ldw * 4); xfer(w.state, (size_t)w.ldw);
+        xfer(w.iwhere, (size_t)w.ldw * 4); xfer(w.state, (size_t)w.ldw); xfer(w.bcls, (size_t)w.ldw);
         if (stage) cudaFreeHost(stage);
         if (ok && !write) ok = cudaMemcpy(&s_dev->tie_limit, &my_tie_limit, sizeof my_tie_limit, cudaMemcpyHostToDevice) == cudaSuccess;
         if (ok && !write) ok = cudaMemcpy(s_host, s_dev, header_bytes, cudaMemcpyDeviceToHost) == cudaSuccess;
-        if (ok && !write) started = true;
+        if (ok && !write) { started = true; compact = classes_ok && s_host->nbcls > 0; }
         if (write && ok) ok = fflush(fp) == 0;
         if (fclose(fp) != 0) ok = false;
         if (write) {
@@ -1574,6 +1602,7 @@
 template <typename T>
 struct TrialSums {
     const T* d; const T* l; const T* u; const int* nbd;
+    const unsigned char* bcls; const typename Real<T>::vec_t* btab;
     T* gd_part; T* pg_part;
 };
 template <typename T>
@@ -1586,7 +1615,7 @@
     if (threadIdx.x == 0) ts.pg_part[blockIdx.x] = r;
 }
 
-template <typename T>
+template <typename T, bool CB = false>
 __global__ void __launch_bounds__(LBFGSB_BLOCK) k_rosenbrock(i64 n, const T* __restrict__ x, T* __restrict__ g,
                                                             T* part, int first, int last, T xl, T xr, const T* halo,
                                                             TrialSums<T> ts) {
@@ -1622,7 +1651,7 @@
         stv<T>(g, base, n, gv);
         if (ts.d) {
             T d[VEC], l[VEC], u[VEC]; int nb[VEC];
-            ldv<T>(ts.d, base, n, d); ldv<T>(ts.l, base, n, l); ldv<T>(ts.u, base, n, u); ldvi<T>(ts.nbd, base, n, nb);
+            ldv<T>(ts.d, base, n, d); ld_bounds<T>(ts.l, ts.u, ts.nbd, CB ? ts.bcls : nullptr, ts.btab, base, n, l, u, nb);
 #pragma unroll
             for (int v = 0; v < VEC; ++v)
                 if (base + v < n) {
@@ -1664,7 +1693,7 @@
     diag = (T)(2.0 + (0.1 + u1));
     b = (T)(2.0 * u2 - 1.0);
 }
-template <typename T>
+template <typename T, bool CB = false>
 __global__ void __launch_bounds__(LBFGSB_BLOCK) k_quadratic(i64 n, const T* __restrict__ x, T* __restrict__ g, T* part,
                                                            i64 off, unsigned long long seedp, T xl, T xr, const T* halo,
                                                            TrialSums<T> ts) {
@@ -1696,7 +1725,7 @@
         stv<T>(g, base, n, gv);
         if (ts.d) {
             T d[VEC], l[VEC], u[VEC]; int nb[VEC];
-            ldv<T>(ts.d, base, n, d); ldv<T>(ts.l, base, n, l); ldv<T>(ts.u, base, n, u); ldvi<T>(ts.nbd, base, n, nb);
+            ldv<T>(ts.d, base, n, d); ld_bounds<T>(ts.l, ts.u, ts.nbd, CB ? ts.bcls : nullptr, ts.btab, base, n, l, u, nb);
 #pragma unroll
             for (int v = 0; v < VEC; ++v)
                 if (base + v < n) {
@@ -1875,6 +1904,7 @@
     lbfgsb_trial_sums_t pub;
     if (l && u && nbd && lbfgsb_dev_trial_sums((lbfgsb_dev_t*)e, &pub) == 0) {
         ts.d = (const T*)pub.d_dev; ts.l = l; ts.u = u; ts.nbd = nbd;
+        if (e->compact) { ts.bcls = e->w.bcls; ts.btab = e->s_dev->bcls_tab; }
         ts.gd_part = (T*)pub.gd_part_dev; ts.pg_part = (T*)pub.pg_part_dev;
         lbfgsb_dev_trial_sums_commit((lbfgsb_dev_t*)e);
     }
@@ -2254,6 +2284,13 @@
     *not_replayed = ev;
     return e != cudaSuccess;
 }
+int lbfgsb_dev_bound_classes(lbfgsb_dev_t* h, int32_t* count) {
+    EngineBase* b = (EngineBase*)h;
+    if (!b || !count) return 1;
+    if (b->real_kind == 8) { Engine<double>* e = (Engine<double>*)b; *count = e->compact ? e->s_host->nbcls : -1; }
+    else { Engine<float>* e = (Engine<float>*)b; *count = e->compact ? e->s_host->nbcls : -1; }
+    return 0;
+}
 void lbfgsb_dev_profile_reset(lbfgsb_dev_t* h) {
     EngineBase* b = (EngineBase*)h;
     if (!b) return;
@@ -2328,11 +2365,13 @@
     cudaStream_t st = e->stream;
     const TrialSums<T> ts = trial_sums_of<T>(e, l, u, nbd);
     if (kind == 0) {
-        k_rosenbrock<T><<<LBFGSB_GRID, LBFGSB_BLOCK, 0, st>>>(e->n, x, g, e->fg_scratch, 1, 1, (T)0, (T)0, nullptr, ts);
+        if (ts.bcls) k_rosenbrock<T, true><<<LBFGSB_GRID, LBFGSB_BLOCK, 0, st>>>(e->n, x, g, e->fg_scratch, 1, 1, (T)0, (T)0, nullptr, ts);
+        else k_rosenbrock<T><<<LBFGSB_GRID, LBFGSB_BLOCK, 0, st>>>(e->n, x, g, e->fg_scratch, 1, 1, (T)0, (T)0, nullptr, ts);
         k_rosenbrock_final<T><<<1, 32, 0, st>>>(e->fg_scratch, e->fg_out);
     } else {
         const unsigned long long seedp = seed * 0x9E3779B97F4A7C15ULL;
-        k_quadratic<T><<<LBFGSB_GRID, LBFGSB_BLOCK, 0, st>>>(e->n, x, g, e->fg_scratch, 0, seedp, (T)0, (T)0, nullptr, ts);
+        if (ts.bcls) k_quadratic<T, true><<<LBFGSB_GRID, LBFGSB_BLOCK, 0, st>>>(e->n, x, g, e->fg_scratch, 0, seedp, (T)0, (T)0, nullptr, ts);
+        else k_quadratic<T><<<LBFGSB_GRID, LBFGSB_BLOCK, 0, st>>>(e->n, x, g, e->fg_scratch, 0, seedp, (T)0, (T)0, nullptr, ts);
         k_sum_final<T><<<1, 32, 0, st>>>(e->fg_scratch, e->fg_out);
     }
     if (cudaMemcpyAsync(e->fg_host, e->fg_out, sizeof(T), cudaMemcpyDeviceToHost, st) != cudaSuccess) return 1;
@@ -2360,11 +2399,14 @@
     k_fg_halo_push<T><<<1, 32, 0, st>>>(x, e->n, e->peers, e->R, e->rank, slot, seq);
     k_fg_halo_wait<T><<<1, 32, 0, st>>>(e->w, e->p2p_local, e->R, e->rank, slot, seq, halo);
     if (kind == 0) {
-        k_rosenbrock<T><<<LBFGSB_GRID, LBFGSB_BLOCK, 0, st>>>(e->n, x, g, e->fg_scratch, e->rank == 0 ? 1 : 0, e->rank == e->R - 1 ? 1 : 0, (T)0, (T)0, halo, ts);
+        const int first = e->rank == 0 ? 1 : 0, last = e->rank == e->R - 1 ? 1 : 0;
+        if (ts.bcls) k_rosenbrock<T, true><<<LBFGSB_GRID, LBFGSB_BLOCK, 0, st>>>(e->n, x, g, e->fg_scratch, first, last, (T)0, (T)0, halo, ts);
+        else k_rosenbrock<T><<<LBFGSB_GRID, LBFGSB_BLOCK, 0, st>>>(e->n, x, g, e->fg_scratch, first, last, (T)0, (T)0, halo, ts);
         k_rosenbrock_final<T><<<1, 32, 0, st>>>(e->fg_scratch, fpart);
     } else {
         const unsigned long long seedp = seed * 0x9E3779B97F4A7C15ULL;
-        k_quadratic<T><<<LBFGSB_GRID, LBFGSB_BLOCK, 0, st>>>(e->n, x, g, e->fg_scratch, e->offset, seedp, (T)0, (T)0, halo, ts);
+        if (ts.bcls) k_quadratic<T, true><<<LBFGSB_GRID, LBFGSB_BLOCK, 0, st>>>(e->n, x, g, e->fg_scratch, e->offset, seedp, (T)0, (T)0, halo, ts);
+        else k_quadratic<T><<<LBFGSB_GRID, LBFGSB_BLOCK, 0, st>>>(e->n, x, g, e->fg_scratch, e->offset, seedp, (T)0, (T)0, halo, ts);
         k_sum_final<T><<<1, 32, 0, st>>>(e->fg_scratch, fpart);
     }
     k_fg_fsum_push<T><<<1, 32, 0, st>>>(fpart, e->peers, e->R, e->rank, slot, seq);
diff --git a/lbfgsb_b200/csrc/kernels_stream.cuh b/lbfgsb_b200/csrc/kernels_stream.cuh
--- a/lbfgsb_b200/csrc/kernels_stream.cuh
+++ b/lbfgsb_b200/csrc/kernels_stream.cuh
@@ -10,6 +10,7 @@
     T *z, *r, *d, *t, *xp;
     T* gold;
     int* iwhere;
+    unsigned char* bcls;
     unsigned char* state;
     T* part;
     i64* ipart;
@@ -98,6 +99,137 @@
     }
 }
 
+#define LB_BC_PER 4
+template <typename T>
+__global__ void __launch_bounds__(LBFGSB_BLOCK) k_bcls_collect(Wk<T> w, typename Real<T>::key_t* blk_tab, int* blk_n) {
+    typedef typename Real<T>::key_t K;
+    constexpr int STEP = LBFGSB_BLOCK * LB_BC_PER;
+    if (w.s->task != TK_FG_START) return;
+    __shared__ K tl[LB_NCLS], tu[LB_NCLS], cl[STEP], cu[STEP];
+    __shared__ unsigned miss[STEP / 32];
+    __shared__ int cnt, ovf;
+    const int tid = threadIdx.x, lane = tid & 31;
+    const i64 n = w.n;
+    const i64 chunk = ((n + LBFGSB_GRID - 1) / LBFGSB_GRID + STEP - 1) / STEP * STEP;
+    const i64 lo = (i64)blockIdx.x * chunk, hi = (lo + chunk < n) ? lo + chunk : n;
+    if (tid == 0) { cnt = 0; ovf = 0; }
+    __syncthreads();
+    int hint = 0;
+    for (i64 s0 = lo; s0 < hi; s0 += STEP) {
+        const int c = cnt;
+#pragma unroll
+        for (int p = 0; p < LB_BC_PER; ++p) {
+            const i64 i = s0 + p * LBFGSB_BLOCK + tid;
+            bool mis = false;
+            if (i < hi) {
+                K kl, ku;
+                bound_key<T>(w.l[i], w.u[i], w.nbd[i], kl, ku);
+                bool found = hint < c && tl[hint] == kl && tu[hint] == ku;
+                for (int k = 0; k < c && !found; ++k)
+                    if (tl[k] == kl && tu[k] == ku) { found = true; hint = k; }
+                cl[p * LBFGSB_BLOCK + tid] = kl; cu[p * LBFGSB_BLOCK + tid] = ku;
+                mis = !found;
+            }
+            const unsigned b = __ballot_sync(0xffffffffu, mis);
+            if (lane == 0) miss[(p * LBFGSB_BLOCK + tid) / 32] = b;
+        }
+        __syncthreads();
+        if (tid < 32) {
+            for (int q = 0; q < STEP / 32 && !ovf; ++q) {
+                unsigned b = miss[q];
+                while (b && !ovf) {
+                    const int e = q * 32 + __ffs(b) - 1;
+                    b &= b - 1;
+                    const K kl = cl[e], ku = cu[e];
+                    const int cc = cnt;
+                    const bool hit = (lane < cc && tl[lane] == kl && tu[lane] == ku) ||
+                                     (lane + 32 < cc && tl[lane + 32] == kl && tu[lane + 32] == ku);
+                    if (__ballot_sync(0xffffffffu, hit) == 0u && lane == 0) {
+                        if (cc == LB_NCLS) ovf = 1;
+                        else { tl[cc] = kl; tu[cc] = ku; cnt = cc + 1; }
+                    }
+                    __syncwarp();
+                }
+            }
+        }
+        __syncthreads();
+        if (ovf) break;
+    }
+    const int c = cnt;
+    for (int k = tid; k < c; k += LBFGSB_BLOCK) {
+        blk_tab[((i64)blockIdx.x * LB_NCLS + k) * 2] = tl[k];
+        blk_tab[((i64)blockIdx.x * LB_NCLS + k) * 2 + 1] = tu[k];
+    }
+    if (tid == 0) blk_n[blockIdx.x] = ovf ? -1 : c;
+}
+template <typename T>
+__global__ void k_bcls_merge(Wk<T> w, const typename Real<T>::key_t* blk_tab, const int* blk_n) {
+    typedef typename Real<T>::key_t K;
+    DevState<T>* s = w.s;
+    __shared__ K tl[LB_NCLS], tu[LB_NCLS];
+    const int lane = threadIdx.x;
+    if (s->task != TK_FG_START) { if (lane == 0) s->nbcls = 0; return; }
+    int cnt = 0;
+    bool ovf = false;
+    for (int b = 0; b < LBFGSB_GRID && !ovf; ++b) {
+        const int nb = blk_n[b];
+        if (nb < 0) { ovf = true; break; }
+        for (int k0 = 0; k0 < nb && !ovf; k0 += 32) {
+            const int k = k0 + lane;
+            K kl = 0, ku = 0;
+            bool miss = false;
+            if (k < nb) {
+                kl = blk_tab[((i64)b * LB_NCLS + k) * 2]; ku = blk_tab[((i64)b * LB_NCLS + k) * 2 + 1];
+                miss = true;
+                for (int j = 0; j < cnt; ++j) if (tl[j] == kl && tu[j] == ku) { miss = false; break; }
+            }
+            unsigned bal = __ballot_sync(0xffffffffu, miss);
+            const int add = __popc(bal);
+            if (cnt + add > LB_NCLS) { ovf = true; break; }
+            if (miss) { const int at = cnt + __popc(bal & ((1u << lane) - 1u)); tl[at] = kl; tu[at] = ku; }
+            cnt += add;
+            __syncwarp();
+        }
+    }
+    if (lane == 0) s->nbcls = ovf ? 0 : cnt;
+    if (!ovf)
+        for (int k = lane; k < cnt; k += 32) {
+            T l, u;
+            memcpy(&l, &tl[k], sizeof l); memcpy(&u, &tu[k], sizeof u);
+            s->bcls_tab[k].x = l; s->bcls_tab[k].y = u;
+        }
+}
+template <typename T>
+__global__ void __launch_bounds__(LBFGSB_BLOCK) k_bcls_write(Wk<T> w) {
+    typedef typename Real<T>::key_t K;
+    constexpr int VEC = Real<T>::VEC;
+    const DevState<T>* s = w.s;
+    const int c = s->nbcls;
+    if (s->task != TK_FG_START || c <= 0) return;
+    __shared__ K tl[LB_NCLS], tu[LB_NCLS];
+    for (int k = threadIdx.x; k < c; k += LBFGSB_BLOCK) {
+        memcpy(&tl[k], &s->bcls_tab[k].x, sizeof(K)); memcpy(&tu[k], &s->bcls_tab[k].y, sizeof(K));
+    }
+    __syncthreads();
+    int hint = 0;
+    LB_FOR_TILES(T, w.n, base) {
+        T l[VEC], u[VEC]; int nb[VEC], b[VEC];
+        ldv<T>(w.l, base, w.n, l); ldv<T>(w.u, base, w.n, u); ldvi<T>(w.nbd, base, w.n, nb);
+#pragma unroll
+        for (int v = 0; v < VEC; ++v) {
+            b[v] = 0;
+            if (base + v < w.n) {
+                K kl, ku;
+                bound_key<T>(l[v], u[v], nb[v], kl, ku);
+                if (!(tl[hint] == kl && tu[hint] == ku))
+                    for (int k = 0; k < c; ++k) if (tl[k] == kl && tu[k] == ku) { hint = k; break; }
+                b[v] = (nb[v] << 6) | hint;
+            }
+        }
+        stvb<T>(w.bcls, base, w.n, b);
+    }
+}
+
 template <typename T>
 __device__ __forceinline__ T projg_one(T x, T g, T l, T u, int nb) {
     T gi = g;
diff --git a/lbfgsb_b200/csrc/kernels_tma.cuh b/lbfgsb_b200/csrc/kernels_tma.cuh
--- a/lbfgsb_b200/csrc/kernels_tma.cuh
+++ b/lbfgsb_b200/csrc/kernels_tma.cuh
@@ -8,6 +8,26 @@
 template <bool B> struct BoolC { static constexpr bool value = B; };
 
 #define LB_DYN_STAGES(dyn) (dyn)
+
+template <typename T, bool CB>
+__device__ __forceinline__ void lds_bounds(const char* sb, unsigned ol, unsigned ou, unsigned onb, int lt,
+                                           const typename Real<T>::vec_t* btab, T (&l)[Real<T>::VEC], T (&u)[Real<T>::VEC],
+                                           int (&nb)[Real<T>::VEC]) {
+    if constexpr (CB) {
+        int c[Real<T>::VEC];
+        lds_byte<T>(sb, onb, lt, c);
+#pragma unroll
+        for (int v = 0; v < Real<T>::VEC; ++v) class_bounds<T>(c[v], btab, l[v], u[v], nb[v]);
+    } else {
+        lds_real<T>(sb, ol, lt, l); lds_real<T>(sb, ou, lt, u); lds_int<T>(sb, onb, lt, nb);
+    }
+}
+template <typename T, bool CB>
+__device__ __forceinline__ void btab_load(typename Real<T>::vec_t* btab, const DevState<T>* s) {
+    if constexpr (CB)
+        for (int k = threadIdx.x; k < s->nbcls; k += blockDim.x) btab[k] = s->bcls_tab[k];
+}
+#define LB_BTAB(T, CB) __shared__ typename Real<T>::vec_t btab[(CB) ? LB_NCLS : 1]
 
 template <typename T>
 __device__ __forceinline__ void pipe_add_w(PipeSrc* ps, const Wk<T>& w, int head0, int count, unsigned slot) {
@@ -131,7 +151,7 @@
     }
 }
 
-template <typename T, int MT>
+template <typename T, int MT, bool CB>
 __global__ void __launch_bounds__(LB_TMA_THREADS, 1) k_cauchy_classify(Wk<T> w) {
     constexpr int VEC = Real<T>::VEC;
     constexpr int SUBT = SubT<T, MT>::v;
@@ -156,15 +176,20 @@
         return;
     }
     const int col = s->col, head0 = s->head - 1;
-    constexpr unsigned OX = 0, OG = G::REAL_SLOT, OL = 2 * G::REAL_SLOT, OU = 3 * G::REAL_SLOT, ONB = 4 * G::REAL_SLOT,
-                       OIW = ONB + G::INT_SLOT, OW = OIW + G::INT_SLOT;
+    LB_BTAB(T, CB);
+    btab_load<T, CB>(btab, s);
+    constexpr unsigned OX = 0, OG = G::REAL_SLOT, OL = 2 * G::REAL_SLOT, OU = 3 * G::REAL_SLOT,
+                       ONB = (CB ? 2 : 4) * G::REAL_SLOT, OIW = ONB + (CB ? G::BYTE_SLOT : G::INT_SLOT), OW = OIW + G::INT_SLOT;
     if (threadIdx.x == 0) {
         pipe_begin(&ps);
         pipe_add(&ps, w.x, sizeof(T), G::REAL_SLOT);
         pipe_add(&ps, w.g, sizeof(T), G::REAL_SLOT);
-        pipe_add(&ps, w.l, sizeof(T), G::REAL_SLOT);
-        pipe_add(&ps, w.u, sizeof(T), G::REAL_SLOT);
-        pipe_add(&ps, w.nbd, 4, G::INT_SLOT);
+        if (CB) pipe_add(&ps, w.bcls, 1, G::BYTE_SLOT);
+        else {
+            pipe_add(&ps, w.l, sizeof(T), G::REAL_SLOT);
+            pipe_add(&ps, w.u, sizeof(T), G::REAL_SLOT);
+            pipe_add(&ps, w.nbd, 4, G::INT_SLOT);
+        }
         pipe_add(&ps, w.iwhere, 4, G::INT_SLOT);
         pipe_add_w<T>(&ps, w, head0, col, G::REAL_SLOT);
         pipe_end(&ps);
@@ -176,8 +201,8 @@
     tma_pass<T, SUBT>(n, &ps, LB_DYN_STAGES(dyn), full, [&](i64 base, const char* sb, int lt) {
         T x[VEC], l[VEC], u[VEC], g[VEC], d[VEC];
         int nb[VEC], iw[VEC];
-        lds_real<T>(sb, OX, lt, x); lds_real<T>(sb, OG, lt, g); lds_real<T>(sb, OL, lt, l); lds_real<T>(sb, OU, lt, u);
-        lds_int<T>(sb, ONB, lt, nb); lds_int<T>(sb, OIW, lt, iw);
+        lds_real<T>(sb, OX, lt, x); lds_real<T>(sb, OG, lt, g);
+        lds_bounds<T, CB>(sb, OL, OU, ONB, lt, btab, l, u, nb); lds_int<T>(sb, OIW, lt, iw);
         bool mv[VEC]; T tk[VEC];
 #pragma unroll
         for (int v = 0; v < VEC; ++v) {
@@ -204,7 +229,9 @@
     block_sum_store<T, 2 * MT + 1>(acc, 2 * MT + 1, sm, w.part2);
     cauchy_scan_store<T, MT>(w, cs, smv, smi);
 }
-template <typename T, int MT> constexpr unsigned smem_classify() { return pipe_smem_bytes<T, SubT<T, MT>::v>(4 + 2 * MT, 2, 0); }
+template <typename T, int MT, bool CB> constexpr unsigned smem_classify() {
+    return CB ? pipe_smem_bytes<T, SubT<T, MT>::v>(2 + 2 * MT, 1, 1) : pipe_smem_bytes<T, SubT<T, MT>::v>(4 + 2 * MT, 2, 0);
+}
 
 template <typename T, int MT>
 __global__ void __launch_bounds__(LB_TMA_THREADS, 1) k_formk_gram(Wk<T> w) {
@@ -337,7 +364,7 @@
 }
 template <typename T, int MT> constexpr unsigned smem_cmprlb() { return pipe_smem_bytes<T, SubT<T, MT>::v>(3 + 2 * MT, 0, 1); }
 
-template <typename T, int MT>
+template <typename T, int MT, bool CB>
 __global__ void __launch_bounds__(LB_TMA_THREADS, 1) k_subsm_step(Wk<T> w) {
     constexpr int VEC = Real<T>::VEC;
     constexpr int SUBT = SubT<T, MT>::v;
@@ -352,22 +379,27 @@
     const i64 n = w.n;
     const int col = s->col, head0 = s->head - 1;
     const T theta = s->theta, rtheta = (T)1 / theta;
+    LB_BTAB(T, CB);
+    btab_load<T, CB>(btab, s);
     constexpr unsigned OZ = 0, OX = G::REAL_SLOT, OG = 2 * G::REAL_SLOT, OR = 3 * G::REAL_SLOT, OL = 4 * G::REAL_SLOT,
-                       OU = 5 * G::REAL_SLOT, OW = 6 * G::REAL_SLOT;
+                       OU = 5 * G::REAL_SLOT, OW = (CB ? 4 : 6) * G::REAL_SLOT;
     if (threadIdx.x == 0) {
         pipe_begin(&ps);
         pipe_add(&ps, w.z, sizeof(T), G::REAL_SLOT);
         pipe_add(&ps, w.x, sizeof(T), G::REAL_SLOT);
         pipe_add(&ps, w.g, sizeof(T), G::REAL_SLOT);
         pipe_add(&ps, w.r, sizeof(T), G::REAL_SLOT);
-        pipe_add(&ps, w.l, sizeof(T), G::REAL_SLOT);
-        pipe_add(&ps, w.u, sizeof(T), G::REAL_SLOT);
+        if (!CB) {
+            pipe_add(&ps, w.l, sizeof(T), G::REAL_SLOT);
+            pipe_add(&ps, w.u, sizeof(T), G::REAL_SLOT);
+        }
         pipe_add_w<T>(&ps, w, head0, col, G::REAL_SLOT);
-        pipe_add(&ps, w.nbd, 4, G::INT_SLOT);
+        if (CB) pipe_add(&ps, w.bcls, 1, G::BYTE_SLOT);
+        else pipe_add(&ps, w.nbd, 4, G::INT_SLOT);
         pipe_add(&ps, w.state, 1, G::BYTE_SLOT);
         pipe_end(&ps);
     }
-    const unsigned onb = OW + 2u * (unsigned)col * G::REAL_SLOT, ost = onb + G::INT_SLOT;
+    const unsigned onb = OW + 2u * (unsigned)col * G::REAL_SLOT, ost = onb + (CB ? G::BYTE_SLOT : G::INT_SLOT);
     T wv1[MT], wv2[MT];
 #pragma unroll
     for (int j = 0; j < MT; ++j) { wv1[j] = (j < col) ? s->wv[j] : (T)0; wv2[j] = (j < col) ? s->wv[col + j] : (T)0; }
@@ -384,8 +416,8 @@
         stv<T>(w.xp, base, n, z);
         if (any) {
             T dk[VEC], l[VEC], u[VEC]; int nb[VEC];
-            lds_real<T>(sb, OR, lt, dk); lds_real<T>(sb, OL, lt, l); lds_real<T>(sb, OU, lt, u);
-            lds_int<T>(sb, onb, lt, nb);
+            lds_real<T>(sb, OR, lt, dk);
+            lds_bounds<T, CB>(sb, OL, OU, onb, lt, btab, l, u, nb);
 #pragma unroll
             for (int j = 0; j < MT; ++j) {
                 if (j < col) {
@@ -422,11 +454,13 @@
     i64 r0 = block_isum(iwd, smi);
     if (threadIdx.x == 0) LB_SLOT(w.ipart, 0)[blockIdx.x] = r0;
 }
-template <typename T, int MT> constexpr unsigned smem_subsm() { return pipe_smem_bytes<T, SubT<T, MT>::v>(6 + 2 * MT, 1, 1); }
+template <typename T, int MT, bool CB> constexpr unsigned smem_subsm() {
+    return CB ? pipe_smem_bytes<T, SubT<T, MT>::v>(4 + 2 * MT, 0, 2) : pipe_smem_bytes<T, SubT<T, MT>::v>(6 + 2 * MT, 1, 1);
+}
 
 template <typename T, int MT> constexpr bool fused_passes_ok() { return sizeof(T) * MT <= 80; }
 
-template <typename T, int MT>
+template <typename T, int MT, bool CB>
 __global__ void __launch_bounds__(LB_TMA_THREADS, 1) k_update_classify(Wk<T> w) {
     constexpr int VEC = Real<T>::VEC;
     constexpr int SUBT = SubT<T, MT>::v;
@@ -442,17 +476,23 @@
     const i64 n = w.n;
     const int col = s->col, head0 = s->head - 1, itail0 = s->itail - 1;
     const T stp = s->stp;
+    LB_BTAB(T, CB);
+    btab_load<T, CB>(btab, s);
     constexpr unsigned OG = 0, OR = G::REAL_SLOT, OD = 2 * G::REAL_SLOT, OX = 3 * G::REAL_SLOT, OL = 4 * G::REAL_SLOT,
-                       OU = 5 * G::REAL_SLOT, ONB = 6 * G::REAL_SLOT, OIW = ONB + G::INT_SLOT, OW = OIW + G::INT_SLOT;
+                       OU = 5 * G::REAL_SLOT, ONB = (CB ? 4 : 6) * G::REAL_SLOT, OIW = ONB + (CB ? G::BYTE_SLOT : G::INT_SLOT),
+                       OW = OIW + G::INT_SLOT;
     if (threadIdx.x == 0) {
         pipe_begin(&ps);
         pipe_add(&ps, w.g, sizeof(T), G::REAL_SLOT);
         pipe_add(&ps, w.gold, sizeof(T), G::REAL_SLOT);
         pipe_add(&ps, w.d, sizeof(T), G::REAL_SLOT);
         pipe_add(&ps, w.x, sizeof(T), G::REAL_SLOT);
-        pipe_add(&ps, w.l, sizeof(T), G::REAL_SLOT);
-        pipe_add(&ps, w.u, sizeof(T), G::REAL_SLOT);
-        pipe_add(&ps, w.nbd, 4, G::INT_SLOT);
+        if (CB) pipe_add(&ps, w.bcls, 1, G::BYTE_SLOT);
+        else {
+            pipe_add(&ps, w.l, sizeof(T), G::REAL_SLOT);
+            pipe_add(&ps, w.u, sizeof(T), G::REAL_SLOT);
+            pipe_add(&ps, w.nbd, 4, G::INT_SLOT);
+        }
         pipe_add(&ps, w.iwhere, 4, G::INT_SLOT);
         pipe_add_w<T>(&ps, w, head0, col - 1, G::REAL_SLOT);
         pipe_end(&ps);
@@ -480,8 +520,8 @@
         stv<T>(wyn, base, n, y);
         T x[VEC], l[VEC], u[VEC], dc[VEC];
         int nb[VEC], iw[VEC];
-        lds_real<T>(sb, OX, lt, x); lds_real<T>(sb, OL, lt, l); lds_real<T>(sb, OU, lt, u);
-        lds_int<T>(sb, ONB, lt, nb); lds_int<T>(sb, OIW, lt, iw);
+        lds_real<T>(sb, OX, lt, x);
+        lds_bounds<T, CB>(sb, OL, OU, ONB, lt, btab, l, u, nb); lds_int<T>(sb, OIW, lt, iw);
         bool mv[VEC]; T tk[VEC];
 #pragma unroll
         for (int v = 0; v < VEC; ++v) {
@@ -524,7 +564,9 @@
     block_sum_store<T, 2 * MT + 1>(ac, 2 * MT + 1, sm, w.part2);
     cauchy_scan_store<T, MT>(w, cs, smv, smi);
 }
-template <typename T, int MT> constexpr unsigned smem_update_classify() { return pipe_smem_bytes<T, SubT<T, MT>::v>(6 + 2 * (MT - 1), 2, 0); }
+template <typename T, int MT, bool CB> constexpr unsigned smem_update_classify() {
+    return CB ? pipe_smem_bytes<T, SubT<T, MT>::v>(4 + 2 * (MT - 1), 1, 1) : pipe_smem_bytes<T, SubT<T, MT>::v>(6 + 2 * (MT - 1), 2, 0);
+}
 
 template <typename T, int MT, int GF>
 __global__ void __launch_bounds__(LB_TMA_THREADS, 1) k_formk_cmprlb(Wk<T> w) {
@@ -705,7 +747,7 @@
 }
 template <typename T, int MT> constexpr unsigned smem_formk_cmprlb() { return pipe_smem_bytes<T, SubT<T, MT>::v>(3 + 2 * MT, 1, 1); }
 
-template <typename T, int MT, int PASS>
+template <typename T, int MT, int PASS, bool CB>
 __global__ void __launch_bounds__(LB_TMA_THREADS, 1) k_subsm_lsinit(Wk<T> w) {
     constexpr int VEC = Real<T>::VEC;
     constexpr int SUBT = SubT<T, MT>::v;
@@ -727,19 +769,24 @@
     const bool lz = s->lazy_z != 0;
     const T tsum = s->tsum;
     const bool axpy = tsum != (T)0;
-    constexpr unsigned OX = 0, OG = G::REAL_SLOT, OL = 2 * G::REAL_SLOT, OU = 3 * G::REAL_SLOT, OR = 4 * G::REAL_SLOT,
-                       OZ = 5 * G::REAL_SLOT;
-    const unsigned OW = (lz ? 5u : 6u) * G::REAL_SLOT;
+    LB_BTAB(T, CB);
+    btab_load<T, CB>(btab, s);
+    constexpr unsigned OX = 0, OG = G::REAL_SLOT, OL = 2 * G::REAL_SLOT, OU = 3 * G::REAL_SLOT, OR = (CB ? 2 : 4) * G::REAL_SLOT,
+                       OZ = OR + G::REAL_SLOT;
+    const unsigned OW = (lz ? OZ : OZ + G::REAL_SLOT);
     if (threadIdx.x == 0) {
         pipe_begin(&ps);
         pipe_add(&ps, PASS == 1 ? w.t : w.x, sizeof(T), G::REAL_SLOT);
         pipe_add(&ps, w.g, sizeof(T), G::REAL_SLOT);
-        pipe_add(&ps, w.l, sizeof(T), G::REAL_SLOT);
-        pipe_add(&ps, w.u, sizeof(T), G::REAL_SLOT);
+        if (!CB) {
+            pipe_add(&ps, w.l, sizeof(T), G::REAL_SLOT);
+            pipe_add(&ps, w.u, sizeof(T), G::REAL_SLOT);
+        }
         pipe_add(&ps, w.r, sizeof(T), G::REAL_SLOT);
         if (!lz) pipe_add(&ps, w.z, sizeof(T), G::REAL_SLOT);
         pipe_add_w<T>(&ps, w, head0, col, G::REAL_SLOT);
-        pipe_add(&ps, w.nbd, 4, G::INT_SLOT);
+        if (CB) pipe_add(&ps, w.bcls, 1, G::BYTE_SLOT);
+        else pipe_add(&ps, w.nbd, 4, G::INT_SLOT);
         pipe_add(&ps, w.state, 1, G::BYTE_SLOT);
         pipe_end(&ps);
     }
@@ -751,7 +798,7 @@
     i64 iwd = 0;
     auto pass = [&](auto full_c) {
     constexpr bool FULLC = decltype(full_c)::value;
-    const unsigned onb = OW + 2u * (unsigned)(FULLC ? MT : col) * G::REAL_SLOT, ost = onb + G::INT_SLOT;
+    const unsigned onb = OW + 2u * (unsigned)(FULLC ? MT : col) * G::REAL_SLOT, ost = onb + (CB ? G::BYTE_SLOT : G::INT_SLOT);
     tma_pass<T, SUBT>(n, &ps, LB_DYN_STAGES(dyn), full, [&](i64 base, const char* sb, int lt) {
         int st[VEC];
         lds_byte<T>(sb, ost, lt, st);
@@ -787,8 +834,7 @@
             return;
         }
         T l[VEC], u[VEC]; int nb[VEC];
-        lds_real<T>(sb, OL, lt, l); lds_real<T>(sb, OU, lt, u);
-        lds_int<T>(sb, onb, lt, nb);
+        lds_bounds<T, CB>(sb, OL, OU, onb, lt, btab, l, u, nb);
         if (!spec) stv<T>(w.xp, base, n, z);
         if (any) {
 #pragma unroll
```

Result: faster. 99.10, median of 6 (+5.5%).
